# privefl/bigsnpr

Measured on AMD Instinct MI355X. Metric: SNP-cols/sec for bed_randomSVD k=20 (m*passes/wall), higher is better.
Workload: dtype i8 (2-bit codes x 24-bit (early block steps) / 16-bit (late block steps) fixed-point image of the fp64 basis in int8 slices, exact int32 MFMA accumulation; fp64 panel algebra and Rayleigh-Ritz)

## Files before the change

bigsnpr_amd/_lib.py:

```python
import ctypes as C
import os
import threading

import numpy as np

_HERE = os.path.dirname(os.path.abspath(__file__))
LIB_PATH = os.path.join(_HERE, "libbigsnpr_hip.so")

u8p = C.POINTER(C.c_uint8)
i32p = C.POINTER(C.c_int32)
i64p = C.POINTER(C.c_int64)
u64p = C.POINTER(C.c_uint64)
f64p = C.POINTER(C.c_double)
vp = C.c_void_p
i64 = C.c_int64

ALLREDUCE_FN = C.CFUNCTYPE(None, C.c_void_p, C.c_int64, C.c_void_p)


class SvdOptions(C.Structure):
    _fields_ = [("k", C.c_int32), ("tol", C.c_double), ("block", C.c_int32),
                ("slices", C.c_int32), ("max_basis", C.c_int32), ("seed", C.c_uint32),
                ("verbose", C.c_int32), ("m_total", C.c_int64), ("allreduce", ALLREDUCE_FN),
                ("allreduce_ctx", C.c_void_p), ("hook_rank", C.c_int32), ("hook_world", C.c_int32),
                ("comm", C.c_void_p), ("binom_scaling", C.c_int32),
                ("center_out", C.POINTER(C.c_double)), ("scale_out", C.POINTER(C.c_double)),
                ("warm_start", C.c_int32), ("warm_denominator", C.c_int32), ("max_restarts", C.c_int32),
                ("vec_floor", C.c_double), ("exchange_timing", C.c_int32), ("exchange_timeout_ms", C.c_int32)]


class SvdInfo(C.Structure):
    _fields_ = [("niter", C.c_int32), ("nops", C.c_int32), ("basis", C.c_int32),
                ("converged", C.c_int32), ("max_rel_resid", C.c_double), ("gpu_ms", C.c_double),
                ("cprod_ms", C.c_double), ("prod_ms", C.c_double), ("n_cprod", C.c_int32),
                ("n_prod", C.c_int32), ("block", C.c_int32), ("slices", C.c_int32),
                ("n_bad", C.c_int32), ("fused_stats", C.c_int32), ("cprod_stats_ms", C.c_double),
                ("n_cprod_stats", C.c_int32), ("warm_launches", C.c_int32), ("warm_fraction", C.c_double),
                ("warm_ms", C.c_double), ("tiled", C.c_int32), ("segmented_passes", C.c_int32), ("compact_gathers", C.c_int32),
                ("slices_max", C.c_int32), ("wide_steps", C.c_int32), ("wide_cprod_ms", C.c_double),
                ("wide_prod_ms", C.c_double), ("n_wide_cprod", C.c_int32), ("n_wide_prod", C.c_int32),
                ("lead_rel_resid", C.c_double), ("exchange_mode", C.c_int32), ("n_exchange", C.c_int32 * 4),
                ("exchange_ms", C.c_double * 4), ("compacted", C.c_int32), ("compact_ms", C.c_double),
                ("out_of_core", C.c_int32), ("na_free_steps", C.c_double * 2), ("na_skip", C.c_int32),
                ("early_ritz", C.c_int32 * 2)]


class PlrOptions(C.Structure):
    _fields_ = [("family", C.c_int32), ("nlambda", C.c_int32), ("nlam_min", C.c_int32), ("n_abort", C.c_int32),
                ("dfmax", C.c_int32), ("max_iter", C.c_int32), ("eps", C.c_double), ("lambda_min_ratio", C.c_double)]


_PLR_TAIL = [f64p, f64p, i64, f64p, i32p, C.c_int32, f64p, C.c_int32, C.POINTER(PlrOptions), f64p, f64p, f64p, f64p, f64p,
             i32p, i32p, i32p, i32p, i32p]

SIGNATURES = {
    "bsn_last_error": (C.c_char_p, []),
    "bsn_version": (C.c_int, []),
    "bsn_device_count": (C.c_int, [C.POINTER(C.c_int)]),
    "bsn_set_device": (C.c_int, [C.c_int]),
    "bsn_selftest": (C.c_int, []),
    "bsn_comm_unique_id": (C.c_int, [u8p]),
    "bsn_comm_init": (C.c_int, [u8p, C.c_int, C.c_int, C.POINTER(vp)]),
    "bsn_comm_rank": (C.c_int, [vp]),
    "bsn_comm_world": (C.c_int, [vp]),
    "bsn_comm_allreduce": (C.c_int, [vp, vp, i64]),
    "bsn_comm_abort": (C.c_int, [vp]),
    "bsn_comm_destroy": (C.c_int, [vp]),
    "bsn_ld_last_stats": (C.c_int, [f64p]),
    "bsn_robust_scale_tau2": (C.c_int, [vp, i64, i64, C.c_int32, C.c_double, C.c_double, f64p, f64p]),
    "bsn_robust_medians": (C.c_int, [vp, i64, i64, C.c_int32, f64p, f64p]),
    "bsn_robust_pair_scales": (C.c_int, [vp, i64, i64, C.c_int32, C.c_double, C.c_double, f64p, f64p]),
    "bsn_robust_mc_count": (C.c_int, [vp, i64, vp, i64, C.c_double, C.POINTER(C.c_int64)]),
    "bsn_robust_scale_cols": (C.c_int, [vp, i64, i64, C.c_int32, f64p]),
    "bsn_robust_rotate": (C.c_int, [vp, i64, i64, C.c_int32, f64p]),
    "bsn_robust_wdist": (C.c_int, [vp, i64, i64, C.c_int32, f64p, f64p, f64p]),
    "bsn_robust_dist_ogk": (C.c_int, [vp, i64, i64, C.c_int32, C.c_int32, C.c_double, C.c_double, C.c_double, f64p, C.POINTER(C.c_int64)]),
    "bsn_robust_rollmean": (C.c_int, [f64p, i64, f64p, C.c_int32, C.POINTER(C.c_int64), C.c_int32, f64p]),
    "bsn_robust_sort": (C.c_int, [f64p, i64]),
    "bsn_order_decreasing": (C.c_int, [f64p, i64, C.POINTER(C.c_int64), C.c_int32, i32p, i32p]),
    "bsn_robust_mc_window": (C.c_int, [vp, i64, vp, i64, C.c_double, C.c_double, i64, f64p, C.POINTER(C.c_int64)]),
    "bsn_bed_open": (C.c_int, [C.c_char_p, i64, i64, C.POINTER(vp)]),
    "bsn_bed_from_host": (C.c_int, [u8p, i64, i64, i64, C.POINTER(vp)]),
    "bsn_bed_from_fbm": (C.c_int, [u8p, i64, i64, i64, C.POINTER(vp)]),
    "bsn_fbm_open": (C.c_int, [u8p, i64, i64, i64, f64p, C.POINTER(vp)]),
    "bsn_bed_bits": (C.c_int, [vp]),
    "bsn_bed_tile": (C.c_int, [vp, C.POINTER(C.c_int)]),
    "bsn_bed_sample_major": (C.c_int, [vp, C.POINTER(C.c_int)]),
    "bsn_bed_na_known": (i64, [vp]),
    "bsn_bed_synthetic": (C.c_int, [i64, i64, C.c_uint32, C.c_uint32, C.c_uint32, i64, C.POINTER(vp)]),
    "bsn_bed_close": (C.c_int, [vp]),
    "bsn_bed_release_workspace": (C.c_int, [vp]),
    "bsn_bed_nrow": (i64, [vp]),
    "bsn_bed_ncol": (i64, [vp]),
    "bsn_bed_bytes": (i64, [vp]),
    "bsn_bed_download": (C.c_int, [vp, u8p]),
    "bsn_bed_prodvec": (C.c_int, [vp, i64p, i64, i64p, i64, f64p, f64p, f64p, f64p]),
    "bsn_bed_cprodvec": (C.c_int, [vp, i64p, i64, i64p, i64, f64p, f64p, f64p, f64p]),
    "bsn_bed_prodvec_sharded": (C.c_int, [vp, i64p, i64, i64p, i64, f64p, f64p, f64p, vp, f64p]),
    "bsn_bed_col_counts": (C.c_int, [vp, i64p, i64, i64p, i64, i32p]),
    "bsn_bed_row_counts": (C.c_int, [vp, i64p, i64, i64p, i64, i32p]),
    "bsn_bed_colstats": (C.c_int, [vp, i64p, i64, i64p, i64, f64p, f64p, i32p, i32p]),
    "bsn_snp_colstats": (C.c_int, [vp, i64p, i64, i64p, i64, f64p, f64p]),
    "bsn_bed_read": (C.c_int, [vp, i64p, i64, i64p, i64, C.c_int32, i32p]),
    "bsn_bed_read_scaled": (C.c_int, [vp, i64p, i64, i64p, i64, f64p, f64p, f64p]),
    "bsn_bed_cprod_planes": (C.c_int, [vp, i64p, i64, i64p, i64, f64p, i64, f64p, f64p]),
    "bsn_bed_prod_and_rowsumssq": (C.c_int, [vp, i64p, i64, i64p, i64, f64p, f64p, f64p, i64, f64p, f64p]),
    "bsn_snp_prod_and_rowsumssq2": (C.c_int, [vp, i64p, i64, i64p, i64, f64p, f64p, f64p, i64, f64p, f64p]),
    "bsn_mult_lin_reg": (C.c_int, [vp, i64p, i64, i64p, i64, f64p, i64, f64p]),
    "bsn_univ_linreg": (C.c_int, [vp, i64p, i64, i64p, i64, f64p, f64p, i64, f64p, f64p]),
    "bsn_univ_logreg": (C.c_int, [vp, i64p, i64, i64p, i64, f64p, f64p, i64, C.c_double, C.c_int32, f64p, f64p, i32p]),
    "bsn_bed_sp_reg": (C.c_int, [vp, i64p, i64, i64p, i64] + _PLR_TAIL),
    "bsn_dense_sp_reg": (C.c_int, [vp, C.c_int, i64, i64, i64] + _PLR_TAIL),
    "bsn_plr_last_stats": (C.c_int, [f64p]),
    "bsn_impute_simple": (C.c_int, [vp, C.c_int, C.c_uint64, C.POINTER(vp), u8p, i64p]),
    "bsn_impute_last_ms": (C.c_int, [f64p]),
    "bsn_bed_group_counts": (C.c_int, [vp, i64p, i64, i32p, C.c_int32, i64p, i64, i32p]),
    "bsn_fst": (C.c_int, [f64p, f64p, i64, i64, C.c_double, f64p, f64p]),
    "bsn_bed_fst": (C.c_int, [vp, i64p, i64, i32p, C.c_int32, i64p, i64, C.c_double, f64p, f64p]),
    "bsn_snp_max3": (C.c_int, [vp, i64p, i64, i32p, i64p, i64, f64p, C.c_int32, f64p]),
    "bsn_popstat_last_ms": (C.c_int, [f64p]),
    "bsn_bed_to_fbm": (C.c_int, [vp, i64p, i64, i64p, i64, u8p]),
    "bsn_bed_readbina": (C.c_int, [vp, u8p, u8p]),
    "bsn_bed_is_streamed": (C.c_int, [vp]),
    "bsn_bed_streaming_kernels": (C.c_int, [vp, C.c_char_p, i64]),
    "bsn_bed_subset_payload": (C.c_int, [vp, i64p, i64, i64p, i64, u8p]),
    "bsn_op_create": (C.c_int, [vp, i64p, i64, i64p, i64, f64p, f64p, C.POINTER(vp)]),
    "bsn_op_destroy": (C.c_int, [vp]),
    "bsn_op_set_slices": (C.c_int, [vp, C.c_int]),
    "bsn_op_prod": (C.c_int, [vp, vp, i64, C.c_int, vp, i64]),
    "bsn_op_cprod": (C.c_int, [vp, vp, i64, C.c_int, vp, i64]),
    "bsn_op_sync": (C.c_int, [vp]),
    "bsn_op_last_kernel": (C.c_int, [vp, C.c_char_p, i64]),
    "bsn_bed_randomsvd": (C.c_int, [vp, i64p, i64, i64p, i64, f64p, f64p, C.POINTER(SvdOptions),
                                    f64p, f64p, f64p, C.POINTER(SvdInfo)]),
    "bsn_bed_tcrossprod": (C.c_int, [vp, i64p, i64, i64p, i64, f64p, f64p, i64, f64p]),
    "bsn_cormat": (C.c_int, [vp, i64p, i64, i64p, i64, C.c_double, f64p, f64p, C.c_int, i32p,
                             C.POINTER(C.c_int64), C.POINTER(vp)]),
    "bsn_cormat_fetch": (C.c_int, [vp, i32p, f64p]),
    "bsn_cormat_has_nan": (C.c_int, [vp, C.POINTER(C.c_int)]),
    "bsn_cormat_free": (C.c_int, [vp]),
    "bsn_ld_scores": (C.c_int, [vp, i64p, i64, i64p, i64, C.c_double, f64p, f64p]),
    "bsn_clumping_chr": (C.c_int, [vp, i64p, i64, i64p, i64, C.c_int, f64p, f64p, i32p, i32p, f64p,
                                   C.c_double, C.c_double, i32p]),
    "bsn_clumping_chr_cached": (C.c_int, [vp, i64p, i64, i64p, i64, C.c_int, f64p, f64p, i32p, i32p, f64p,
                                          i64, f64p, f64p, i32p]),
    "bsn_snp_grid_prs": (C.c_int, [vp, i64p, i64, i64p, i64, f64p, i32p, C.POINTER(C.c_uint8), i64, i64,
                                   C.c_int, f64p]),
    "bsn_sfbm_from_csc": (C.c_int, [i64p, i32p, f64p, i64, C.c_int, C.POINTER(vp)]),
    "bsn_sfbm_ncol": (C.c_int, [vp, i64p, i64p, i64p]),
    "bsn_sfbm_free": (C.c_int, [vp]),
    "bsn_lassosum2": (C.c_int, [vp, f64p, i64, f64p, f64p, f64p, i64, i64p, C.c_double, C.c_int32, C.c_double,
                                f64p, i32p, f64p]),
    "bsn_ldpred2_gibbs": (C.c_int, [vp, f64p, f64p, i64, i64p, f64p, f64p, i32p, u64p, i64, C.c_int, C.c_int, C.c_uint64,
                                    f64p, f64p]),
    "bsn_ldpred2_gibbs_sampling": (C.c_int, [vp, f64p, f64p, i64, i64p, C.c_double, C.c_double, C.c_int32, C.c_uint64,
                                             C.c_int, C.c_int, C.c_uint64, f64p, f64p]),
    "bsn_ldpred2_auto": (C.c_int, [vp, f64p, f64p, f64p, i64, i64p, f64p, u64p, i64, C.c_double, C.c_int, C.c_int, C.c_int,
                                   C.c_int, C.c_double, C.c_int, C.c_double, C.c_double, C.c_double, C.c_double,
                                   C.c_double, C.c_uint64, f64p, f64p, f64p, f64p, f64p, f64p, f64p, f64p]),
    "bsn_sfbm_prodvec": (C.c_int, [vp, f64p, i64p, i64, f64p]),
    "bsn_sfbm_ld_scores": (C.c_int, [vp, i64p, i64, f64p]),
    "bsn_sfbm_solve_sym": (C.c_int, [vp, f64p, f64p, i64p, i64, C.c_double, C.c_int32, f64p, i32p, f64p]),
    "bsn_sfbm_last_ms": (C.c_int, [vp, f64p]),
    "bsn_sfbm_ldsplit": (C.c_int, [vp, C.c_double, C.c_double, C.c_int32, C.c_int32, C.c_int32, C.c_double, f64p, f64p, i32p,
                                   f64p, f64p, f64p, i32p, i32p, i32p, f64p]),
    "bsn_malloc": (C.c_int, [C.POINTER(vp), i64]),
    "bsn_free": (C.c_int, [vp]),
    "bsn_host_alloc": (C.c_int, [C.POINTER(vp), i64]),
    "bsn_host_free": (C.c_int, [vp]),
    "bsn_memcpy_h2d": (C.c_int, [vp, vp, i64]),
    "bsn_memcpy_d2h": (C.c_int, [vp, vp, i64]),
    "bsn_device_sync": (C.c_int, []),
    "bsn_timer_start": (C.c_int, [vp]),
    "bsn_timer_stop": (C.c_int, [vp, f64p]),
}

_lib = None


class BsnError(RuntimeError):
    pass


def load():
    global _lib
    if _lib is None:
        LIB_PATH = os.environ.get("BSN_LIB_PATH") or globals()["LIB_PATH"]
        if not os.path.exists(LIB_PATH):
            raise ImportError(
                "%s not found: build it with `python -m bigsnpr_amd.build` "
                "(there is no CPU fallback)" % LIB_PATH)
        lib = C.CDLL(LIB_PATH)
        for name, (res, args) in SIGNATURES.items():
            fn = getattr(lib, name)
            fn.restype = res
            fn.argtypes = args
        _lib = lib
    return _lib


def check(rc):
    if rc != 0:
        raise BsnError(load().bsn_last_error().decode("utf-8", "replace"))


def ptr(a, t):
    return None if a is None else a.ctypes.data_as(t)


def as_i64(a):
    return None if a is None else np.ascontiguousarray(a, dtype=np.int64)


def as_f64(a):
    return None if a is None else np.ascontiguousarray(a, dtype=np.float64)


class DeviceArray:

    def __init__(self, rows, cols=1):
        self.rows, self.cols = int(rows), int(cols)
        p = vp()
        check(load().bsn_malloc(C.byref(p), self.rows * self.cols * 8))
        self.ptr = p

    @classmethod
    def from_numpy(cls, a):
        a = np.asarray(a, dtype=np.float64)
        if a.ndim == 1:
            a = a[:, None]
        d = cls(a.shape[0], a.shape[1])
        h = np.asfortranarray(a)
        check(load().bsn_memcpy_h2d(d.ptr, h.ctypes.data_as(vp), h.nbytes))
        return d

    def to_numpy(self):
        h = np.empty((self.rows, self.cols), dtype=np.float64, order="F")
        check(load().bsn_memcpy_d2h(h.ctypes.data_as(vp), self.ptr, h.nbytes))
        return h

    def col_ptr(self, j):
        return vp(self.ptr.value + 8 * self.rows * j)

    def free(self):
        if self.ptr is not None and self.ptr.value:
            load().bsn_free(self.ptr)
            self.ptr = None

    def __del__(self):
        try:
            self.free()
        except Exception:
            pass


class _PinnedBlock:

    def __init__(self, pool, addr, size):
        self.pool, self.addr, self.size = pool, addr, size
        self.__array_interface__ = {"data": (addr, False), "shape": (size,), "typestr": "|u1", "version": 3}

    def __del__(self):
        try:
            self.pool._give_back(self.addr, self.size)
        except Exception:
            pass


class PinnedPool:

    def __init__(self, keep=None):
        self.free = []
        self.keep = int(os.environ.get("BSN_RESULT_POOL_KEEP", 1 << 30)) if keep is None else keep
        self.keep_max = int(os.environ.get("BSN_RESULT_POOL_MAX", 8 << 30))
        self.live = 0
        self.peak_live = 0
        self.lazy = not os.environ.get("BSN_RESULT_POOL_EAGER")
        self.pending = set()
        self.wanted = []
        self.prefetched = 0
        self.lock = threading.RLock()

    def empty(self, shape, dtype=np.float64):
# ... 70 lines not shown
```

bigsnpr_amd/csrc/api.hip:

```cpp
#include <dlfcn.h>
#include <fcntl.h>
#include <pthread.h>
#include <sys/mman.h>
#include <sys/stat.h>
#include <unistd.h>

#include <algorithm>
#include <cerrno>
#include <cmath>
#include <condition_variable>
#include <chrono>
#include <cstring>
#include <limits>
#include <map>
#include <memory>
#include <mutex>
#include <sched.h>
#include <atomic>
#include <thread>

#include <cstdlib>

#include "bsn_internal.hpp"
#include <cxxabi.h>
// ... 972 lines not shown
int bsn_bed_close(bsn_bed *bed) {
  return guarded([&] {
    if (bed) {
      (void)hipSetDevice(bed->device);
      free_bed(bed);
    }
  });
}

int bsn_bed_tile(bsn_bed *bed, int *built) {
  return guarded([&] {
    BSN_HIP(hipSetDevice(bed->device));
    const bool ok = image_tile(bed);
    if (built) *built = ok ? 1 : 0;
  });
}

int bsn_bed_streaming_kernels(bsn_bed *bed, char *buf, int64_t len) {
  return guarded([&] {
    if (!buf || len < 1) fail("bsn_bed_streaming_kernels: no buffer");
    buf[0] = 0;
    if (bed->last_solve_on_sub && bed->sub) bed = bed->sub;
    if (!bed->svd_op) return;
    static const char *kinds[kProfKinds] = {"cprod", "prod", "cprod_stats", "warm", "cprod_wide", "prod_wide"};
    std::string out;
    for (int k = 0; k < kProfKinds; k++) {
      const void *fn = bed->svd_op->prof_kernel[k];
      if (!fn) continue;
      const char *mangled = hipKernelNameRefByPtr(fn, bed->stream);
      if (!mangled) continue;
      int status = 1;
      char *dem = abi::__cxa_demangle(mangled, nullptr, nullptr, &status);
      std::string name = (status == 0 && dem) ? dem : mangled;
      free(dem);
      const size_t par = name.find('(');
      if (par != std::string::npos) name.resize(par);
      out += std::string(kinds[k]) + "=" + name + "\n";
    }
    snprintf(buf, (size_t)len, "%s", out.c_str());
  });
}

int bsn_op_last_kernel(bsn_op *op, char *buf, int64_t len) {
  return guarded([&] {
    if (!buf || len < 1) fail("bsn_op_last_kernel: no buffer");
    buf[0] = 0;
    if (!op->last_kernel) return;
    const char *mangled = hipKernelNameRefByPtr(op->last_kernel, op->bed->stream);
    if (!mangled) return;
    int status = 1;
    char *dem = abi::__cxa_demangle(mangled, nullptr, nullptr, &status);
    std::string name = (status == 0 && dem) ? dem : mangled;
    free(dem);
    const size_t par = name.find('(');
    if (par != std::string::npos) name.resize(par);
    snprintf(buf, (size_t)len, "%s", name.c_str());
  });
}

int bsn_bed_sample_major(bsn_bed *bed, int *built) {
  return guarded([&] {
    BSN_HIP(hipSetDevice(bed->device));
    const bool ok = image_smaj(bed);
    if (built) *built = ok ? 1 : 0;
  });
}

int bsn_bed_release_workspace(bsn_bed *bed) {
  return guarded([&] {
    BSN_HIP(hipSetDevice(bed->device));
    BSN_HIP(hipStreamSynchronize(bed->stream));
    bed->svd_op.reset();
    bed->svd_ws.reset();
    if (bed->d_tiled) {
      BSN_HIP(hipFree(bed->d_tiled));
      bed->d_tiled = nullptr;
    }
    bed->tiled_tried = false;
    image_smaj_wait(bed);
    if (bed->d_smaj) {
      BSN_HIP(hipFree(bed->d_smaj));
      bed->d_smaj = nullptr;
    }
    bed->smaj_tried = false;
    bed->smaj_cap = 0;
    if (bed->sub) {
      bed_free(bed->sub);
      bed->sub = nullptr;
      bed->sub_key = 0;
      bed->sub_cols.clear();
      bed->sub_rows.clear();
      bed->last_solve_on_sub = false;
    }
    bed->stats_cache.release();
    if (bed->slab_img) {
      bed_free(bed->slab_img);
      bed->slab_img = nullptr;
    }
    if (bed->slab_stage) {
      delete (bsn::FileStage *)bed->slab_stage;
      bed->slab_stage = nullptr;
    }
    dev_cache_flush();
  });
}

int64_t bsn_bed_nrow(const bsn_bed *bed) { return bed->n; }
int64_t bsn_bed_ncol(const bsn_bed *bed) { return bed->m; }
int64_t bsn_bed_bytes(const bsn_bed *bed) { return bed->pitch * bed->m; }

int bsn_bed_download(bsn_bed *bed, uint8_t *payload_out) {
  return guarded([&] {
    BSN_HIP(hipSetDevice(bed->device));
    if (bed->streamed()) {
      std::memcpy(payload_out, bed->h_map, (size_t)bed->n_byte * (size_t)bed->m);
      return;
    }
    image_download(bed, payload_out);
  });
}

int bsn_op_create(bsn_bed *bed, const int64_t *ind_row, int64_t n, const int64_t *ind_col,
                  int64_t m, const double *center, const double *scale, bsn_op **out) {
  return guarded([&] {
    std::unique_ptr<bsn_op> op(new bsn_op());
    fill_op(op.get(), bed, ind_row, n, ind_col, m, center, scale);
    *out = op.release();
  });
}

int bsn_op_destroy(bsn_op *op) {
  return guarded([&] {
    if (op) {
      (void)hipSetDevice(op->bed->device);
      delete op;
    }
  });
}

int bsn_op_set_slices(bsn_op *op, int slices) {
  return guarded([&] {
    if (slices < 1 || slices > 7) fail("slices must be in 1..7");
    op->slices = slices;
  });
}

int bsn_op_prod(bsn_op *op, const double *d_X, int64_t ldx, int nvec, double *d_Y, int64_t ldy) {
  return guarded([&] {
    BSN_HIP(hipSetDevice(op->bed->device));
    op_prod(op, d_X, ldx, nvec, d_Y, ldy);
  });
}

int bsn_op_cprod(bsn_op *op, const double *d_X, int64_t ldx, int nvec, double *d_Z, int64_t ldz) {
  return guarded([&] {
    BSN_HIP(hipSetDevice(op->bed->device));
    op_cprod(op, d_X, ldx, nvec, d_Z, ldz);
  });
}

int bsn_op_sync(bsn_op *op) {
  return guarded([&] { BSN_HIP(hipStreamSynchronize(op->bed->stream)); });
}

static void matvec_host(bsn_bed *bed, const int64_t *ind_row, int64_t n, const int64_t *ind_col,
                        int64_t m, const double *center, const double *scale, const double *x,
                        double *out, bool transpose, bsn_comm *comm = nullptr) {
  if (bed->streamed()) {
    if (comm) fail("sharded products are not available for an out-of-core handle");
    SlabWalk W(bed);
    std::vector<double> ce, sc, xs, part;
    if (!transpose) std::fill(out, out + n, 0.0);
    W.run(ind_col, m, [&](bsn_bed *sb, const std::vector<int64_t> &P, const std::vector<int64_t> &local) {
      const int64_t k = (int64_t)P.size();
      if (center) { ce.resize((size_t)k); for (int64_t t = 0; t < k; t++) ce[(size_t)t] = center[P[(size_t)t]]; }
      if (scale) { sc.resize((size_t)k); for (int64_t t = 0; t < k; t++) sc[(size_t)t] = scale[P[(size_t)t]]; }
      if (transpose) {
        part.resize((size_t)k);
        matvec_host(sb, ind_row, n, local.data(), k, center ? ce.data() : nullptr, scale ? sc.data() : nullptr, x,
                    part.data(), true);
        BSN_HIP(hipStreamSynchronize(sb->stream));
        for (int64_t t = 0; t < k; t++) out[P[(size_t)t]] = part[(size_t)t];
      } else {
        xs.resize((size_t)k);
        for (int64_t t = 0; t < k; t++) xs[(size_t)t] = x[P[(size_t)t]];
        part.resize((size_t)n);
        matvec_host(sb, ind_row, n, local.data(), k, center ? ce.data() : nullptr, scale ? sc.data() : nullptr, xs.data(),
                    part.data(), false);
        BSN_HIP(hipStreamSynchronize(sb->stream));
        for (int64_t i = 0; i < n; i++) out[i] += part[(size_t)i];
      }
    });
    return;
  }
  bsn_op op;
  const bool late = transpose && bed->bits == 2 && !bed->generic && (center || scale);
  fill_op(&op, bed, ind_row, n, ind_col, m, center, scale, late);
  if (late) {
    op.late_center = center;
    op.late_scale = scale;
    if (!center) BSN_HIP(hipMemsetAsync(op.d_center.p, 0, (size_t)m * 8, bed->stream));
    if (!scale) {
      hipLaunchKernelGGL(k_fill_f64, dim3((unsigned)((m + 255) / 256)), dim3(256), 0, bed->stream, op.d_scale.p, m, 1.0);
      BSN_HIP(hipGetLastError());
    }
  }
  op.slices = 7;
  int64_t nin = transpose ? n : m, nout = transpose ? m : n;
  DevBuf<double> d_in, d_out;
  copy_h2d(bed, d_in.ensure((size_t)nin), x, (size_t)nin * 8);
  d_out.ensure((size_t)nout);
  if (bed->generic) {
    const int32_t *rows = op.rows_identity ? nullptr : op.d_rows.p, *cols = op.cols_contig ? nullptr : op.d_cols.p;
    if (comm) fail("sharded products are not available for a generic decode table");
    if (transpose)
      lut_cprod(bed, rows, n, cols, op.col0, m, center ? op.d_center.p : nullptr, scale ? op.d_scale.p : nullptr,
                d_in.p, d_out.p);
    else
      lut_prod(bed, rows, n, cols, op.col0, m, center ? op.d_center.p : nullptr, scale ? op.d_scale.p : nullptr,
               d_in.p, d_out.p);
    copy_d2h(bed, out, d_out.p, (size_t)nout * 8);
    return;
  }
  if (transpose)
    op_cprod(&op, d_in.p, nin, 1, d_out.p, nout);
  else
    op_prod(&op, d_in.p, nin, 1, d_out.p, nout);
  if (comm) {
    if (transpose) fail("internal: the crossproduct of a column shard needs no exchange");
    if (comm->device != bed->device) fail("the communicator was created on another device");
    comm_allreduce_sum(comm, d_out.p, nout, bed->stream);
  }
  copy_d2h(bed, out, d_out.p, (size_t)nout * 8);
}

int bsn_bed_prodvec(bsn_bed *bed, const int64_t *ind_row, int64_t n, const int64_t *ind_col,
                    int64_t m, const double *center, const double *scale, const double *x,
                    double *y) {
  return guarded([&] { matvec_host(bed, ind_row, n, ind_col, m, center, scale, x, y, false); });
}

int bsn_bed_prodvec_sharded(bsn_bed *bed, const int64_t *ind_row, int64_t n, const int64_t *ind_col,
                            int64_t m, const double *center, const double *scale, const double *x,
                            bsn_comm *comm, double *y) {
  return guarded([&] { matvec_host(bed, ind_row, n, ind_col, m, center, scale, x, y, false, comm); });
}

int bsn_bed_cprodvec(bsn_bed *bed, const int64_t *ind_row, int64_t n, const int64_t *ind_col,
                     int64_t m, const double *center, const double *scale, const double *x,
                     double *z) {
  return guarded([&] { matvec_host(bed, ind_row, n, ind_col, m, center, scale, x, z, true); });
}

int bsn_bed_col_counts(bsn_bed *bed, const int64_t *ind_row, int64_t n, const int64_t *ind_col,
                       int64_t m, int32_t *res) {
  return guarded([&] { counts_host(bed, ind_row, n, ind_col, m, res); });
}

int bsn_bed_row_counts(bsn_bed *bed, const int64_t *ind_row, int64_t n, const int64_t *ind_col, int64_t m,
                       int32_t *res) {
  return guarded([&] {
    bsn_op op;
    fill_op(&op, bed, ind_row, n, ind_col, m, nullptr, nullptr);
    DevBuf<double> d_c;
    d_c.ensure((size_t)3 * n);
    op_row_counts(&op, d_c.p);
    std::vector<double> c((size_t)3 * n);
    copy_d2h(bed, c.data(), d_c.p, (size_t)3 * n * 8);
    for (int64_t i = 0; i < n; i++) {
      const int64_t n2 = (int64_t)c[(size_t)i], n1 = (int64_t)c[(size_t)(n + i)], na = (int64_t)c[(size_t)(2 * n + i)];
      res[4 * i + 0] = (int32_t)(m - n1 - n2 - na);
      res[4 * i + 1] = (int32_t)n1;
      res[4 * i + 2] = (int32_t)n2;
      res[4 * i + 3] = (int32_t)na;
    }
  });
}

int bsn_bed_colstats(bsn_bed *bed, const int64_t *ind_row, int64_t n, const int64_t *ind_col,
                     int64_t m, double *sumX, double *denoX, int32_t *nb_nona_col,
                     int32_t *n_bad) {
  return guarded([&] {
    std::vector<int32_t> cnt((size_t)4 * m);
    counts_host(bed, ind_row, n, ind_col, m, cnt.data());
    int32_t bad = 0;
    for (int64_t j = 0; j < m; j++) {
      const int32_t *c = &cnt[(size_t)4 * j];
      double xSum = (double)c[1] + 2.0 * c[2], xxSum = (double)c[1] + 4.0 * c[2];
      int32_t nona = (int32_t)(n - c[3]);
      sumX[j] = xSum;
      denoX[j] = xxSum - xSum * xSum / nona;
      nb_nona_col[j] = nona;
      if (2 * (int64_t)nona < n) bad++;
    }
    if (n_bad) *n_bad = bad;
  });
}

int bsn_snp_colstats(bsn_bed *bed, const int64_t *ind_row, int64_t n, const int64_t *ind_col,
                     int64_t m, double *sumX, double *denoX) {
  return guarded([&] {
    const double qnan = std::numeric_limits<double>::quiet_NaN();
    if (bed->generic) {
      bsn_op op;
      fill_op(&op, bed, ind_row, n, ind_col, m, nullptr, nullptr);
      DevBuf<double> d_st;
// ... 364 lines not shown
```

bigsnpr_amd/csrc/bsn_internal.hpp:

```cpp
#pragma once
#include <hip/hip_runtime.h>
#include <stdint.h>

#include <atomic>
#include <cstdarg>
#include <cstdio>
#include <functional>
#include <cstdlib>
#include <memory>
#include <stdexcept>
#include <string>
#include <vector>

#include "bigsnpr_hip.h"

namespace bsn {
inline const char *abl_getenv(const char *name) {
#ifdef BSN_ABLATION
  return getenv(name);
#else
  (void)name;
  return nullptr;
#endif
}

struct Error : std::runtime_error {
  using std::runtime_error::runtime_error;
};
void set_error(const char *msg);
[[noreturn]] void fail(const char *fmt, ...);
void require_gpu();

#define BSN_HIP(expr)                                                             \
  do {                                                                            \
    hipError_t e__ = (expr);                                                      \
    if (e__ != hipSuccess)                                                        \
      ::bsn::fail("HIP error %s at %s:%d (%s)", hipGetErrorString(e__), __FILE__, \
                  __LINE__, #expr);                                               \
  } while (0)

template <class F>
int guarded(F &&f) {
  try {
    f();
    return 0;
  } catch (const std::exception &ex) {
    set_error(ex.what());
    (void)hipGetLastError();
    return 1;
  } catch (...) {
    set_error("unknown C++ exception");
    (void)hipGetLastError();
    return 1;
  }
}

constexpr size_t kDevCacheMaxBlock = (size_t)256 << 20;
constexpr size_t kDevCacheMaxTotal = (size_t)2 << 30;
void *dev_alloc(size_t bytes, size_t *granted, int *device);
void dev_release(void *p, size_t granted, int device);
void dev_cache_flush();
size_t dev_cache_held();

template <class T>
struct DevBuf {
  T *p = nullptr;
  size_t n = 0;
  size_t granted = 0;
  int device = 0;
  DevBuf() = default;
  DevBuf(const DevBuf &) = delete;
  DevBuf &operator=(const DevBuf &) = delete;
  ~DevBuf() { release(); }
  void release() {
    if (p) dev_release(p, granted, device);
    p = nullptr;
    n = 0;
    granted = 0;
  }
  T *ensure(size_t count) {
    if (count > n) {
      release();
      p = (T *)dev_alloc(count * sizeof(T), &granted, &device);
      n = count;
    }
    return p;
  }
};

constexpr int64_t kPitchAlign = 256;

inline int64_t round_up(int64_t a, int64_t b) { return (a + b - 1) / b * b; }

__host__ __device__ inline uint32_t dev_from_plink(uint32_t w) {
  return (~w & 0xAAAAAAAAu) | ((w ^ (w >> 1)) & 0x55555555u);
}
__host__ __device__ inline uint32_t plink_from_dev(uint32_t w) {
  return (~w & 0xAAAAAAAAu) | (~(w ^ (w >> 1)) & 0x55555555u);
}

}

struct bsn_bed;
namespace bsn {
struct SvdWorkspace;
}

constexpr int kCommClasses = 4;
struct bsn_comm {
  void *comm = nullptr;
  int rank = 0, world = 1, device = 0;
  hipStream_t stream = nullptr;
  std::atomic<int> aborted{0};
  bool timing = false;
  struct Timed { hipEvent_t a, b; int cls; };
  std::vector<Timed> timed;
  std::vector<hipEvent_t> ev_pool;
  ~bsn_comm() {
    for (auto &t : timed) { (void)hipEventDestroy(t.a); (void)hipEventDestroy(t.b); }
    for (auto e : ev_pool) (void)hipEventDestroy(e);
  }
};

constexpr int kProfKinds = 6;
struct bsn_op {
  bsn_bed *bed = nullptr;
  int64_t n = 0, m = 0;
  bool rows_identity = true;
  bool cols_contig = true;
  bool no_na = false;
  bool na_skip_c = false, na_skip_p = false;
  bool stats_pending = false;
  bsn::DevBuf<int32_t> d_counts;
  bsn::DevBuf<int32_t> d_na;
  long long *h_na_total = nullptr;
  bool na_poll = false;
  int64_t col0 = 0;
  int slices = 4;
  int64_t passes = 0;
  const double *late_center = nullptr, *late_scale = nullptr;
  const double *preq_X = nullptr;
  int64_t preq_ldx = 0;
  int preq_nvec = 0, preq_S = 0;
  bool profile = false;
  int prof_kind_override = -1;
  std::vector<hipEvent_t> ev_begin, ev_end;
  std::vector<int> ev_kind;
  std::vector<char> ev_more;
  const void *prof_kernel[kProfKinds] = {};
  const void *last_kernel = nullptr;
  ~bsn_op() {
    for (auto e : ev_begin) (void)hipEventDestroy(e);
    for (auto e : ev_end) (void)hipEventDestroy(e);
    if (h_na_total) (void)hipHostFree(h_na_total);
  }
  bsn::DevBuf<int32_t> d_rows;
  bsn::DevBuf<int32_t> d_cols;
  bsn::DevBuf<double> d_center, d_scale;
  bsn::DevBuf<double> d_xfull;
  bsn::DevBuf<int8_t> d_q;
  bsn::DevBuf<int32_t> d_acc;
  bsn::DevBuf<double> d_meta;
  bsn::DevBuf<double> d_yfull;
};

struct bsn_bed {
  int64_t n = 0, m = 0, n_byte = 0, pitch = 0;
  int bits = 2;
  double v_off = 0.0, v_step = 1.0;
  bool generic = false;
  double *d_lut = nullptr;
  uint8_t *d_img = nullptr;
  uint8_t *d_tiled = nullptr;
  bool tiled_tried = false;
  size_t tiled_cap = 0;
  const uint8_t *h_map = nullptr;
  void *map_base = nullptr;
  size_t map_len = 0;
  int64_t slab_cols = 0;
  int fd_file = -1;
  bsn_bed *slab_img = nullptr;
  void *slab_stage = nullptr;
  bool streamed() const { return d_img == nullptr && h_map != nullptr; }
  uint8_t *d_smaj = nullptr;
  int64_t pitch_smaj = 0, rows_smaj = 0;
  bool smaj_tried = false;
  size_t smaj_cap = 0;
  void *smaj_job = nullptr;
  int64_t cap_m = 0;
  bsn_bed *sub = nullptr;
  uint64_t sub_key = 0;
  std::vector<int64_t> sub_cols, sub_rows;
  bool last_solve_on_sub = false;
  int device = 0;
  bool stream_borrowed = false;
  hipStream_t stream = nullptr;
  hipStream_t stream_up = nullptr;
  hipEvent_t ev_up = nullptr;
  hipEvent_t ev0 = nullptr, ev1 = nullptr;
  std::vector<int32_t> na_cnt;
  struct CountsCache {
    std::vector<int64_t> rows;
    std::vector<int32_t> cnt;
    void clear() {
      rows.clear();
      cnt.clear();
    }
  } counts_cache;
  struct StatsCache {
    bsn::DevBuf<int32_t> d_cnt;
    std::vector<uint8_t> known;
    int64_t n_known = 0;
    bsn::DevBuf<int32_t> d_cols;
    uint64_t cols_key = 0;
    void clear() {
      known.clear();
      n_known = 0;
    }
    void release() {
      clear();
      d_cnt.release();
      d_cols.release();
      cols_key = 0;
    }
  } stats_cache;
  void forget_counts() {
    counts_cache.clear();
    stats_cache.clear();
  }
  int na_blocks_state = 0;
  long long *h_na_blocks = nullptr;
  long long *d_na_blocks = nullptr;
  double na_free[2] = {0.0, 0.0};
  std::unique_ptr<bsn_op> svd_op;
  std::shared_ptr<bsn::SvdWorkspace> svd_ws;
  uint8_t *h_stage[2] = {nullptr, nullptr};
  hipEvent_t ev_stage[2] = {nullptr, nullptr};
  bool stage_busy[2] = {false, false};
  unsigned stage_next = 0;
};

struct bsn_sfbm {
  int64_t m2 = 0, nnz = 0;
  bsn::DevBuf<int64_t> p;
  bsn::DevBuf<int32_t> i;
  bsn::DevBuf<double> x;
  std::vector<int32_t> lo, hi;
  int64_t bandwidth = 0;
  std::vector<int64_t> hp;
  double last_ms = 0;
};

namespace bsn {

void image_alloc(bsn_bed *b, int64_t n, int64_t m, int bits = 2);
void stage_init(bsn_bed *b);
void bed_free(bsn_bed *b);
bsn_bed *image_gather(bsn_bed *src, const int64_t *ind_row, int64_t n, const int64_t *ind_col, int64_t m,
                      bsn_bed *reuse = nullptr);
bool image_tile(bsn_bed *b);
bool image_smaj(bsn_bed *b);
bool image_smaj_start(bsn_bed *b);
bool image_smaj_poll(bsn_bed *b);
void image_smaj_wait(bsn_bed *b);
void image_from_host(bsn_bed *b, const uint8_t *payload, int64_t n_byte_src);
struct FileStage {
  uint8_t *pin[2] = {nullptr, nullptr};
  hipEvent_t done[2] = {nullptr, nullptr};
  size_t bytes = 0;
  ~FileStage();
  FileStage() = default;
  FileStage(const FileStage &) = delete;
  FileStage &operator=(const FileStage &) = delete;
};
void image_from_file(bsn_bed *b, int fd, int64_t offset, int64_t n_byte_src, FileStage *stage = nullptr);
void image_from_fbm(bsn_bed *b, const uint8_t *bytes, int64_t ld, const uint8_t *lut);
void stats8(bsn_bed *b, const int32_t *d_rows, int64_t n, const int32_t *d_cols, int64_t col0, int64_t m,
            long long *d_out);
void lut_colstats(bsn_bed *b, const int32_t *d_rows, int64_t n, const int32_t *d_cols, int64_t col0, int64_t m,
                  double *d_out);
void lut_cprod(bsn_bed *b, const int32_t *d_rows, int64_t n, const int32_t *d_cols, int64_t col0, int64_t m,
               const double *d_center, const double *d_scale, const double *d_x, double *d_z);
void lut_prod(bsn_bed *b, const int32_t *d_rows, int64_t n, const int32_t *d_cols, int64_t col0, int64_t m,
              const double *d_center, const double *d_scale, const double *d_x, double *d_y);
void refuse_generic(const bsn_bed *b, const char *what);
void image_generate(bsn_bed *b, uint32_t seed, uint32_t npop, uint32_t na16, int64_t j_begin);
void image_download(bsn_bed *b, uint8_t *payload_out);
void counts_all_rows(bsn_bed *b, const int32_t *d_cols, int64_t col0, int64_t m, int32_t *d_counts);
void counts_host(bsn_bed *bed, const int64_t *ind_row, int64_t n, const int64_t *ind_col, int64_t m,
                 int32_t *res);
void counts_device(bsn_op *op, const int64_t *ind_row, int64_t n, int32_t *d_counts);
struct StatsCols {
  const int64_t *ind_col;
  const int32_t *d_cols;
  int64_t col0, m;
};
bool stats_cache_enabled(const bsn_bed *b);
bool stats_cache_known(const bsn_bed *b, const StatsCols &c);
void stats_cache_store(bsn_bed *b, const StatsCols &c, const int32_t *d_counts, hipStream_t st);
void stats_cache_load(bsn_bed *b, const StatsCols &c, int32_t *d_counts, hipStream_t st);
void read_dense(bsn_bed *b, const int32_t *d_rows, int64_t n, const int32_t *d_cols, int64_t m,
                const double *d_center, const double *d_scale, int32_t na_val, int32_t *d_out_i,
                double *d_out_d);

void to_bytes(bsn_bed *b, const int32_t *d_rows, int64_t n, const int32_t *d_cols, int64_t m,
              uint8_t *d_out);
void readbina_bytes(bsn_bed *b, const uint8_t *d_tab, uint8_t *d_out);
void subset_pack(bsn_bed *b, const int32_t *d_rows, int64_t n, const int32_t *d_cols, int64_t m,
                 uint8_t *d_out);

void copy_h2d(bsn_bed *b, void *d_dst, const void *src, size_t bytes, hipStream_t stream = nullptr);
hipStream_t upload_stream(bsn_bed *b);
void copy_d2h(bsn_bed *b, void *dst, const void *d_src, size_t bytes);
bool host_is_pinned(const void *p);
// ... 57 lines not shown
```

bigsnpr_amd/csrc/matvec.hip:

```cpp
#include <cmath>
#include <cstdlib>

#include "bsn_internal.hpp"
#include "byte_plan.hpp"
#include "prod_plan.hpp"
#include "prodt_sparse.hpp"
#include <type_traits>

namespace bsn {

typedef int v4i __attribute__((ext_vector_type(4)));
typedef int v8i __attribute__((ext_vector_type(8)));

static thread_local const void *g_last_kernel = nullptr;
#define BSN_KLAUNCH(kern, ...)                 \
  do {                                         \
    g_last_kernel = (const void *)(kern);      \
    hipLaunchKernelGGL(kern, __VA_ARGS__);     \
  } while (0)

__device__ __forceinline__ uint32_t lut4(uint32_t lut, uint32_t sel) {
  return __builtin_amdgcn_perm(lut, lut, sel);
}
__device__ __forceinline__ uint32_t perm8(uint32_t hi, uint32_t lo, uint32_t sel) {
// ... 49 lines not shown
      const double b3 = fabs(b - 3.0 * a);
      if (!(fabs(b) <= 1.79e308)) bad++; else mx = fmax(mx, fabs(b));
      if (raw3 && b3 <= 1.79e308) mx = fmax(mx, b3);
    } else if (mode == 2) {
      double b = center ? fabs(center[k + v * ldx]) : 0.0;
      if (!(b <= 1.79e308)) bad++; else mx = fmax(mx, b);
    }
    a = fabs(a);
    if (!(a <= 1.79e308)) bad++; else mx = fmax(mx, a);
  }
  for (int off = 32; off > 0; off >>= 1) {
    mx = fmax(mx, __shfl_down(mx, off));
    bad += __shfl_down(bad, off);
  }
  __shared__ double smx[16];
  __shared__ unsigned long long sbad[16];
  const int wave = threadIdx.x >> 6, nw = blockDim.x >> 6;
  if ((threadIdx.x & 63) == 0) {
    smx[wave] = mx;
    sbad[wave] = bad;
  }
  __syncthreads();
  if (threadIdx.x == 0) {
    for (int w = 1; w < nw; w++) {
      mx = fmax(mx, smx[w]);
      bad += sbad[w];
    }
    double *pp = part + ((int64_t)v * gridDim.x + blockIdx.x) * 2;
    pp[0] = mx;
    pp[1] = (double)bad;
    if (blockIdx.x == 0) meta[v].sum_hi = meta[v].sum_lo = meta[v].sum2_hi = meta[v].sum2_lo = 0;
  }
}

template <int S, int PERM>
__global__ __launch_bounds__(64) void k_quant(const double *__restrict__ X, int64_t ldx, int64_t len,
                                              int64_t len_pad, const double *__restrict__ center,
                                              const double *__restrict__ scale, int mode, int ncol,
                                              VecMeta *meta, int8_t *__restrict__ q, double vstep, double voff,
                                              int raw3, const double *__restrict__ part, int gx) {
  __shared__ double sa[64 * 17], sb[64 * 17];
  const int tid = threadIdx.x, v = blockIdx.y;
  const int64_t kb = (int64_t)blockIdx.x * 64 + tid;
  const int nplanes = mode >= 1 ? 2 : 1;
  double qs = 1.0;
  if (gx > 0) {
    double mx = 0, bad = 0;
    for (int t = tid; t < gx; t += 64) {
      mx = fmax(mx, part[((int64_t)v * gx + t) * 2]);
      bad += part[((int64_t)v * gx + t) * 2 + 1];
    }
    for (int off = 32; off > 0; off >>= 1) {
      mx = fmax(mx, __shfl_xor(mx, off));
      bad += __shfl_xor(bad, off);
    }
    qs = 0.0;
    if (mx > 0) {
      int e;
      frexp(ldexp(0.99, 8 * S - 1) / mx, &e);
      qs = ldexp(1.0, e - 1);
    }
    if (blockIdx.x == 0 && tid == 0) {
      meta[v].absmax_bits = (unsigned long long)__double_as_longlong(mx);
      meta[v].nonfinite = (unsigned long long)bad;
    }
  }
  if (blockIdx.x == 0 && tid == 0) meta[v].qscale = qs;
  double xa[16], xc[16], xs[16];
#pragma unroll
  for (int it = 0; it < 16; it++) {
    const int64_t k = (int64_t)blockIdx.x * 1024 + it * 64 + tid;
    const bool in = k < len;
    xa[it] = in ? X[k + v * ldx] : 0.0;
    xc[it] = 0.0;
    xs[it] = 1.0;
    if (mode == 1) {
      if (in && scale) xs[it] = scale[k];
      if (in && center) xc[it] = center[k];
    } else if (mode == 2) {
      if (in && center) xc[it] = center[k + v * ldx];
    }
  }
#pragma unroll
  for (int it = 0; it < 16; it++) {
    const int t = it * 64 + tid;
    double a = xa[it], b = 0;
    if (mode == 1) {
      a = a / xs[it];
      b = (xc[it] - voff) * a;
      a *= vstep;
    } else if (mode == 2) {
      b = xc[it];
    }
    if (!(fabs(a) <= 1.79e308)) a = 0;
    if (!(fabs(b) <= 1.79e308)) b = 0;
    sa[t + (t >> 4)] = a * qs;
    sb[t + (t >> 4)] = b * qs;
  }
  __syncthreads();
  long long shi = 0, slo = 0, shi2 = 0, slo2 = 0;
  if (kb * 16 < len_pad) {
    uint32_t pk[2][S][4];
#pragma unroll
    for (int p = 0; p < 2; p++)
#pragma unroll
      for (int s = 0; s < S; s++)
#pragma unroll
        for (int w = 0; w < 4; w++) pk[p][s][w] = 0;
#pragma unroll
    for (int e = 0; e < 16; e++) {
      long long A = llrint(sa[tid * 17 + e]), B = llrint(sb[tid * 17 + e]);
      shi += A >> 24; slo += A & 0xFFFFFF;
      shi2 += B >> 24; slo2 += B & 0xFFFFFF;
      if ((raw3 & 1) && PERM != 2) B -= 3 * A;
      const int pos = PERM == 1 ? ((e & 3) * 4 + (e >> 2)) : e;
#pragma unroll
      for (int s = 0; s < S; s++) {
        const int8_t da = (int8_t)(A & 0xFF), db = (int8_t)(B & 0xFF);
        A = (A - da) >> 8;
        B = (B - db) >> 8;
        if constexpr (PERM == 2) {
          const int r = prodt_sparse_row(e), ba = prodt_sparse_byte(e, 0), bb = prodt_sparse_byte(e, 1);
          pk[r][s][ba >> 2] |= (uint32_t)(uint8_t)da << (8 * (ba & 3));
          pk[r][s][bb >> 2] |= (uint32_t)(uint8_t)db << (8 * (bb & 3));
        } else {
          pk[0][s][pos >> 2] |= (uint32_t)(uint8_t)da << (8 * (pos & 3));
          pk[1][s][pos >> 2] |= (uint32_t)(uint8_t)db << (8 * (pos & 3));
        }
      }
    }
    for (int p = 0; p < nplanes; p++)
#pragma unroll
      for (int s = 0; s < S; s++) {
        const int col = v * S + s;
        int8_t *dst = q + ((kb * nplanes + p) * ncol + col) * 16;
        *(uint4 *)dst = p == 0 ? uint4{pk[0][s][0], pk[0][s][1], pk[0][s][2], pk[0][s][3]}
                               : uint4{pk[1][s][0], pk[1][s][1], pk[1][s][2], pk[1][s][3]};
      }
  }
  for (int off = 32; off > 0; off >>= 1) {
    shi += __shfl_down(shi, off); slo += __shfl_down(slo, off);
    shi2 += __shfl_down(shi2, off); slo2 += __shfl_down(slo2, off);
  }
  if (tid == 0) {
    atomicAdd((unsigned long long *)&meta[v].sum_hi, (unsigned long long)shi);
    atomicAdd((unsigned long long *)&meta[v].sum_lo, (unsigned long long)slo);
    if (mode >= 1) {
      atomicAdd((unsigned long long *)&meta[v].sum2_hi, (unsigned long long)shi2);
      atomicAdd((unsigned long long *)&meta[v].sum2_lo, (unsigned long long)slo2);
    }
  }
}

template <int NB, int NPLANE, int KC, bool RAW0, bool STATS, bool CONTIG, int TILES = 2, int WAVES = 8, int MINW = 1,
          int TAG = 0, bool TILED = false, int SGB = 0, bool NASKIP = false>
__global__ __launch_bounds__(64 * WAVES, MINW) void k_cprod(const uint8_t *__restrict__ img, int64_t pitch,
                                               const int32_t *__restrict__ cols, int64_t col0,
                                               int64_t m, const int8_t *__restrict__ xq,
                                               int32_t *__restrict__ acc_out, int64_t m_out,
                                               uint32_t lutA, uint32_t lutB, uint32_t lutC,
                                               int32_t *__restrict__ counts, int32_t n_pad_samples) {
  constexpr int NCOL = 16 * NB;
  constexpr int LD = KC / 256;
  constexpr int XS = KC / 16 * NCOL;
  __shared__ uint4 xs[2][XS];
  const int tid = threadIdx.x, wave = tid >> 6, lane = tid & 63;
  const int c = lane & 15, g = lane >> 4;
  constexpr int NT = 64 * WAVES;
  const int64_t wg_base = (int64_t)blockIdx.x * (WAVES * 16 * TILES);
  const int64_t snp_base = wg_base + wave * (16 * TILES);
  const uint8_t *rowp[TILES];
  uint32_t voff[TILES];
#pragma unroll
  for (int t = 0; t < TILES; t++) {
    int64_t j = snp_base + t * 16 + c;
    if (j > m - 1) j = m - 1;
    int64_t col = CONTIG ? col0 + j : (int64_t)cols[j];
    rowp[t] = img + col * pitch + g * 16;
    voff[t] = TILED ? (uint32_t)((((j - wg_base) >> 6) * (pitch >> 8)) * 16384 + (j & 63) * 256 + g * 16)
                    : (uint32_t)((j - wg_base) * pitch + g * 16);
  }
  static_assert(!TILED || (CONTIG && (WAVES * 16 * TILES) % 64 == 0), "streaming layout: whole 64-variant blocks");
  const __amdgpu_buffer_rsrc_t rs = __builtin_amdgcn_make_buffer_rsrc(
      (void *)(TILED ? img + (((col0 + wg_base) >> 6) * (pitch >> 8)) * 16384
                     : img + (col0 + (CONTIG ? wg_base : 0)) * pitch),
      0, 0x7fffffff, 0x00020000);
  typedef unsigned int v4u __attribute__((ext_vector_type(4)));
  auto gload = [&](const int t, const int off) -> uint4 {
    if constexpr (CONTIG) {
      const int soff = TILED ? ((off >> 8) << 14) + (off & 255) : off;
      const v4u r = __builtin_amdgcn_raw_buffer_load_b128(rs, (int)voff[t], soff, 0);
      return uint4{r.x, r.y, r.z, r.w};
    } else {
      return *(const uint4 *)(rowp[t] + off);
    }
  };
  const int nchunks = (int)(pitch * 4 / KC);
  const uint4 *xq4 = (const uint4 *)xq;

  v4i acc[TILES][NPLANE][NB];
#pragma unroll
  for (int t = 0; t < TILES; t++)
#pragma unroll
    for (int p = 0; p < NPLANE; p++)
#pragma unroll
      for (int nb = 0; nb < NB; nb++) acc[t][p][nb] = v4i{0, 0, 0, 0};
  uint32_t st_lo[TILES], st_hi[TILES], st_na[TILES];
#pragma unroll
  for (int t = 0; t < TILES; t++) st_lo[t] = st_hi[t] = st_na[t] = 0;

  constexpr int NX = (XS + NT - 1) / NT;
  static_assert(NX <= 4, "staging registers");
  constexpr bool XFULL = (XS % NT == 0);
  uint4 ga[2][TILES][LD];
  uint4 xr0 = {0, 0, 0, 0}, xr1 = {0, 0, 0, 0}, xr2 = {0, 0, 0, 0}, xr3 = {0, 0, 0, 0};
#pragma unroll
  for (int t = 0; t < TILES; t++)
#pragma unroll
    for (int it = 0; it < LD; it++) ga[0][t][it] = gload(t, it * 64);
  auto staged = [&](const int x) -> bool { return XFULL || tid + x * NT < XS; };
  if (staged(0)) xs[0][tid] = xq4[tid];
  if constexpr (NX > 1) if (staged(1)) xs[0][tid + NT] = xq4[tid + NT];
  if constexpr (NX > 2) if (staged(2)) xs[0][tid + 2 * NT] = xq4[tid + 2 * NT];
  if constexpr (NX > 3) if (staged(3)) xs[0][tid + 3 * NT] = xq4[tid + 3 * NT];
#pragma unroll
  for (int t = 0; t < TILES; t++)
#pragma unroll
    for (int it = 0; it < LD; it++)
      ga[1][t][it] = gload(t, (nchunks > 1 ? KC / 4 : 0) + it * 64);
  __syncthreads();

  auto chunk = [&](auto SETC, const int ch) {
    constexpr int SET = decltype(SETC)::value;
    const int ch1 = ch + 1 < nchunks ? ch + 1 : nchunks - 1;
    const int ch2 = ch + 2 < nchunks ? ch + 2 : nchunks - 1;
    {
      const uint4 *src = xq4 + (int64_t)ch1 * XS;
      auto at = [&](const int x) -> int { return XFULL ? tid + x * NT : (tid + x * NT < XS ? tid + x * NT : XS - 1); };
      xr0 = src[at(0)];
      if constexpr (NX > 1) xr1 = src[at(1)];
      if constexpr (NX > 2) xr2 = src[at(2)];
      if constexpr (NX > 3) xr3 = src[at(3)];
    }
    __builtin_amdgcn_sched_barrier(0);
    if constexpr (SGB & 2) __builtin_amdgcn_s_setprio(2);
    const int off2 = ch2 * (KC / 4);
    auto kstep = [&](const int t, const uint32_t w, const uint4 (&bv)[NB]) {
      uint32_t s0 = w & 0x03030303u, s1 = (w >> 2) & 0x03030303u,
               s2 = (w >> 4) & 0x03030303u, s3 = (w >> 6) & 0x03030303u;
      if constexpr (STATS) {
        const uint32_t lo = w & 0x55555555u;
        st_lo[t] += __popc(lo);
        st_hi[t] += __popc(w);
        st_na[t] += __popc(lo & (w >> 1));
      }
      static_assert(!NASKIP || (RAW0 && NPLANE == 2 && !STATS), "the skip is for the missing-value plane of the plain pass");
      bool plane1 = true;
      if constexpr (NASKIP) plane1 = __builtin_amdgcn_ballot_w64(((w & (w >> 1)) & 0x55555555u) != 0u) != 0ull;
#pragma unroll
      for (int p = 0; p < NPLANE; p++) {
        if (NASKIP && p == 1 && !plane1) continue;
        const uint32_t lut = p == 0 ? lutA : p == 1 ? lutB : lutC;
        v4i a;
        if (RAW0 && p == 0) {
          a = v4i{(int)s0, (int)s1, (int)s2, (int)s3};
        } else {
          a = v4i{(int)lut4(lut, s0), (int)lut4(lut, s1), (int)lut4(lut, s2), (int)lut4(lut, s3)};
        }
#pragma unroll
        for (int nb = 0; nb < NB; nb++) {
          v4i b = {(int)bv[nb].x, (int)bv[nb].y, (int)bv[nb].z, (int)bv[nb].w};
          acc[t][p][nb] = __builtin_amdgcn_mfma_i32_16x16x64_i8(a, b, acc[t][p][nb], 0, 0, 0);
        }
      }
    };
    constexpr bool PFB = NB <= 2;
    uint4 bv[NB], bn[PFB ? NB : 1];
#pragma unroll
    for (int nb = 0; nb < NB; nb++) bv[nb] = xs[SET][(g * 4) * NCOL + nb * 16 + c];
#pragma unroll
    for (int it = 0; it < LD; it++) {
#pragma unroll
      for (int d = 0; d < 4; d++) {
        if constexpr (!PFB) {
          if (it * 4 + d > 0) {
#pragma unroll
            for (int nb = 0; nb < NB; nb++) bv[nb] = xs[SET][(it * 16 + g * 4 + d) * NCOL + nb * 16 + c];
          }
        } else if (it * 4 + d + 1 < LD * 4) {
          const int itn = (it * 4 + d + 1) / 4, dn = (it * 4 + d + 1) % 4;
#pragma unroll
          for (int nb = 0; nb < NB; nb++) bn[nb] = xs[SET][(itn * 16 + g * 4 + dn) * NCOL + nb * 16 + c];
        }
#pragma unroll
        for (int t = 0; t < TILES; t++) {
          const uint32_t w = d == 0 ? ga[SET][t][it].x : d == 1 ? ga[SET][t][it].y
                             : d == 2 ? ga[SET][t][it].z : ga[SET][t][it].w;
          kstep(t, w, bv);
        }
        if constexpr (PFB) {
#pragma unroll
          for (int nb = 0; nb < NB; nb++) bv[nb] = bn[nb];
        }
      }
    }
#pragma unroll
    for (int t = 0; t < TILES; t++)
#pragma unroll
      for (int it = 0; it < LD; it++) ga[SET][t][it] = gload(t, off2 + it * 64);
    if constexpr (SGB & 1) {
      constexpr int VSTEP = TILES * (7 + (NPLANE - (RAW0 ? 1 : 0)) * 4 + (STATS ? 6 : 0));
      constexpr int MSTEP = TILES * NPLANE * NB;
      __builtin_amdgcn_sched_group_barrier(0x100, NB, 0);
      __builtin_amdgcn_sched_group_barrier(0x002, 7, 0);
      auto slot = [&](auto IC) {
        constexpr int i = decltype(IC)::value;
        constexpr int nv = VSTEP * (i + 1) / MSTEP - VSTEP * i / MSTEP;
        __builtin_amdgcn_sched_group_barrier(0x008, 1, 0);
        if constexpr (nv > 0) __builtin_amdgcn_sched_group_barrier(0x002, nv, 0);
      };
      auto slots = [&](auto self, auto IC) {
        constexpr int i = decltype(IC)::value;
        if constexpr (i < MSTEP) {
          slot(IC);
          self(self, std::integral_constant<int, i + 1>{});
        }
      };
#pragma unroll
      for (int stp = 0; stp < LD * 4; stp++) {
        __builtin_amdgcn_sched_group_barrier(0x100, NB, 0);
        slots(slots, std::integral_constant<int, 0>{});
      }
      __builtin_amdgcn_sched_group_barrier(0x020, TILES * LD, 0);
    }
    __builtin_amdgcn_sched_barrier(0);
    if constexpr (SGB & 2) __builtin_amdgcn_s_setprio(0);
    {
      if (staged(0)) xs[SET ^ 1][tid] = xr0;
      if constexpr (NX > 1) if (staged(1)) xs[SET ^ 1][tid + NT] = xr1;
      if constexpr (NX > 2) if (staged(2)) xs[SET ^ 1][tid + 2 * NT] = xr2;
      if constexpr (NX > 3) if (staged(3)) xs[SET ^ 1][tid + 3 * NT] = xr3;
    }
    __syncthreads();
  };
  for (int ch = 0; ch < nchunks; ch += 2) {
    chunk(std::integral_constant<int, 0>{}, ch);
    if (ch + 1 < nchunks) chunk(std::integral_constant<int, 1>{}, ch + 1);
  }

#pragma unroll
  for (int t = 0; t < TILES; t++)
#pragma unroll
    for (int r = 0; r < 4; r++) {
      int64_t j = snp_base + t * 16 + g * 4 + r;
      if (j < m) {
#pragma unroll
        for (int p = 0; p < NPLANE; p++)
#pragma unroll
          for (int nb = 0; nb < NB; nb++)
            acc_out[((int64_t)p * m_out + j) * NCOL + nb * 16 + c] = acc[t][p][nb][r];
      }
    }
  if constexpr (STATS) {
#pragma unroll
    for (int t = 0; t < TILES; t++) {
      uint32_t lo = st_lo[t], hi = st_hi[t] - st_lo[t], na = st_na[t];
      lo += __shfl_xor(lo, 16); hi += __shfl_xor(hi, 16); na += __shfl_xor(na, 16);
      lo += __shfl_xor(lo, 32); hi += __shfl_xor(hi, 32); na += __shfl_xor(na, 32);
      const int64_t j = snp_base + t * 16 + c;
      if (g == 0 && j < m) {
        const int32_t n1 = (int32_t)(lo - na), n2 = (int32_t)(hi - na);
        *(int4 *)(counts + 4 * j) =
            int4{(int32_t)(pitch * 4) - n1 - n2 - (int32_t)na - n_pad_samples, n1, n2, (int32_t)na};
      }
    }
  }
}

__device__ __forceinline__ double horner(const int32_t *a, int S) {
  double r = 0;
  for (int s = S - 1; s >= 0; s--) r = r * 256.0 + (double)a[s];
  return r;
}
__device__ __forceinline__ double horner_sub(const int32_t *a, const int32_t *q, int k, int S) {
  double r = 0;
  for (int s = S - 1; s >= 0; s--) r = r * 256.0 + (double)((long long)a[s] - (long long)k * q[s]);
  return r;
}

template <int NCOL>
__global__ __launch_bounds__(128) void k_cprod_final(const int32_t *__restrict__ acc, int64_t m, int S, int nv,
                                                     const VecMeta *__restrict__ meta,
                                                     const double *__restrict__ center,
                                                     const double *__restrict__ scale, double *Z, int64_t ldz,
                                                     int has_q) {
  constexpr int ROW = 2 * NCOL + 1;
  __shared__ int32_t srow[128 * ROW];
  const int64_t j = (int64_t)blockIdx.x * 128 + threadIdx.x;
  if (j >= m) return;
  int32_t *my = srow + threadIdx.x * ROW;
  {
    const int4 *pa = (const int4 *)(acc + j * NCOL), *pq = (const int4 *)(acc + (m + j) * NCOL);
#pragma unroll
    for (int t = 0; t < NCOL / 4; t++) {
      const int4 x = pa[t];
      my[4 * t] = x.x; my[4 * t + 1] = x.y; my[4 * t + 2] = x.z; my[4 * t + 3] = x.w;
    }
    if (has_q) {
#pragma unroll
      for (int t = 0; t < NCOL / 4; t++) {
        const int4 x = pq[t];
        my[NCOL + 4 * t] = x.x; my[NCOL + 4 * t + 1] = x.y; my[NCOL + 4 * t + 2] = x.z; my[NCOL + 4 * t + 3] = x.w;
      }
    }
  }
  const double c = center ? center[j] : 0.0, s = scale ? scale[j] : 1.0;
  for (int v = 0; v < nv; v++) {
    const double P = has_q ? horner_sub(my + v * S, my + NCOL + v * S, 3, S) : horner(my + v * S, S);
    const double Q = has_q ? horner(my + NCOL + v * S, S) : 0.0;
    const double Sx = (double)meta[v].sum_hi * 16777216.0 + (double)meta[v].sum_lo;
    const double qs = meta[v].qscale;
    double z = qs > 0 ? (P - c * (Sx - Q)) / (s * qs) : 0.0 / s;
    if (P == 0.0 && Sx - Q == 0.0 && qs > 0) z = 0.0;
    if (meta[v].nonfinite) z = __longlong_as_double(0x7ff8000000000000LL);
    Z[j + v * ldz] = z;
  }
}

template <int NB, bool CONTIG, bool RAWP, bool HASQ = true, int TAG = 0, bool TILED = false>
__global__ __launch_bounds__(256) void k_prod(const uint8_t *__restrict__ img, int64_t pitch,
                                              const int32_t *__restrict__ cols, int64_t col0,
                                              int64_t m_pad, int64_t mc,
                                              const int8_t *__restrict__ wq,
                                              int32_t *__restrict__ acc_out, int64_t n_pad,
                                              uint32_t lutP, uint32_t lutQ) {
  constexpr int NCOL = 16 * NB, WAVES = 4;
  const int tid = threadIdx.x, wave = tid >> 6, lane = tid & 63;
  const int sg = lane & 15, g = lane >> 4;
  const unsigned bx = blockIdx.x, by = blockIdx.y;
  static_assert(!TILED || CONTIG, "streaming layout: contiguous variants");
  const int64_t wbase = ((int64_t)bx * WAVES + wave) * 256;
  const int64_t wbyte = wbase / 4 + sg * 4;
  const uint32_t lane_off = (uint32_t)(g * 16 * pitch + wbyte);
  const int64_t j0 = (int64_t)by * mc;
  int64_t j1 = j0 + mc;
  if (j1 > m_pad) j1 = m_pad;
  const uint4 *wq4 = (const uint4 *)wq;

  v4i acc[16][NB];
#pragma unroll
  for (int u = 0; u < 16; u++)
#pragma unroll
    for (int nb = 0; nb < NB; nb++) acc[u][nb] = v4i{0, 0, 0, 0};

  constexpr int WS = 8 * NCOL;
  __shared__ uint4 ws[2][WS];
  static_assert((WS & (WS - 1)) == 0 && WS <= 64 * WAVES, "digit staging");
  uint32_t X[2][16];
  uint4 wreg = {0, 0, 0, 0};
  const int wtid = tid & (WS - 1);
  auto load = [&](int64_t jb, uint32_t *dst) {
    if (CONTIG) {
      if constexpr (TILED) {
        const int64_t sbw = (int64_t)bx;
        const __amdgpu_buffer_rsrc_t rs = __builtin_amdgcn_make_buffer_rsrc(
            (void *)(img + (((col0 + jb) >> 6) * (pitch >> 8) + sbw) * 16384), 0, 0x7fffffff, 0x00020000);
        const int toff = g * 4096 + wave * 64 + sg * 4;
#pragma unroll
        for (int r = 0; r < 16; r++) dst[r] = (uint32_t)__builtin_amdgcn_raw_buffer_load_b32(rs, toff, r * 256, 0);
      } else {
        const __amdgpu_buffer_rsrc_t rs = __builtin_amdgcn_make_buffer_rsrc(
            (void *)(img + (col0 + jb) * pitch), 0, 0x7fffffff, 0x00020000);
#pragma unroll
        for (int r = 0; r < 16; r++) dst[r] = (uint32_t)__builtin_amdgcn_raw_buffer_load_b32(rs, (int)lane_off, r * (int)pitch, 0);
      }
    } else {
      const int4 *ip = (const int4 *)(cols + jb + g * 16);
#pragma unroll
      for (int r4 = 0; r4 < 4; r4++) {
        int4 id = ip[r4];
        dst[r4 * 4 + 0] = *(const uint32_t *)(img + (int64_t)id.x * pitch + wbyte);
        dst[r4 * 4 + 1] = *(const uint32_t *)(img + (int64_t)id.y * pitch + wbyte);
        dst[r4 * 4 + 2] = *(const uint32_t *)(img + (int64_t)id.z * pitch + wbyte);
        dst[r4 * 4 + 3] = *(const uint32_t *)(img + (int64_t)id.w * pitch + wbyte);
      }
    }
  };
  if (j0 >= j1) return;
  const int64_t jlast = j1 - 64;
  ws[0][wtid] = wq4[(j0 / 16) * 2 * NCOL + wtid];
  load(j0, X[0]);
  load(j0 + 64 < j1 ? j0 + 64 : jlast, X[1]);
  __syncthreads();

  auto step = [&](auto SETC, const int64_t jb) {
    constexpr int SET = decltype(SETC)::value;
    const int64_t jn1 = jb + 64 < j1 ? jb + 64 : jlast, jn2 = jb + 128 < j1 ? jb + 128 : jlast;
    wreg = wq4[(jn1 / 16) * 2 * NCOL + wtid];
    __builtin_amdgcn_sched_barrier(0);
    v4i aw[NB], awc[NB];
#pragma unroll
    for (int nb = 0; nb < NB; nb++) {
      uint4 t0 = ws[SET][(g * 2 + 0) * NCOL + nb * 16 + sg];
      uint4 t1 = ws[SET][(g * 2 + 1) * NCOL + nb * 16 + sg];
      aw[nb] = v4i{(int)t0.x, (int)t0.y, (int)t0.z, (int)t0.w};
      awc[nb] = v4i{(int)t1.x, (int)t1.y, (int)t1.z, (int)t1.w};
    }
    uint32_t T[4][4];
#pragma unroll
    for (int r4 = 0; r4 < 4; r4++) {
      const uint32_t x0 = X[SET][4 * r4], x1 = X[SET][4 * r4 + 1], x2 = X[SET][4 * r4 + 2], x3 = X[SET][4 * r4 + 3];
      const uint32_t lo01 = perm8(x1, x0, 0x05010400u);
      const uint32_t hi01 = perm8(x1, x0, 0x07030602u);
      const uint32_t lo23 = perm8(x3, x2, 0x05010400u);
      const uint32_t hi23 = perm8(x3, x2, 0x07030602u);
      T[0][r4] = perm8(lo23, lo01, 0x05040100u);
      T[1][r4] = perm8(lo23, lo01, 0x07060302u);
      T[2][r4] = perm8(hi23, hi01, 0x05040100u);
      T[3][r4] = perm8(hi23, hi01, 0x07060302u);
    }
    __builtin_amdgcn_sched_barrier(0);
    load(jn2, X[SET]);
    __builtin_amdgcn_sched_barrier(0);
#pragma unroll
    for (int q = 0; q < 4; q++)
#pragma unroll
      for (int u0 = 0; u0 < 4; u0++) {
        v4i g0, na;
#pragma unroll
        for (int r4 = 0; r4 < 4; r4++) {
          const uint32_t sel = (T[q][r4] >> (2 * u0)) & 0x03030303u;
          g0[r4] = RAWP ? (int)sel : (int)lut4(lutP, sel);
          if (HASQ) na[r4] = (int)lut4(lutQ, sel);
        }
#pragma unroll
        for (int nb = 0; nb < NB; nb++) {
          acc[q * 4 + u0][nb] = __builtin_amdgcn_mfma_i32_16x16x64_i8(aw[nb], g0, acc[q * 4 + u0][nb], 0, 0, 0);
          if (HASQ)
            acc[q * 4 + u0][nb] = __builtin_amdgcn_mfma_i32_16x16x64_i8(awc[nb], na, acc[q * 4 + u0][nb], 0, 0, 0);
        }
      }
    ws[SET ^ 1][wtid] = wreg;
    __syncthreads();
  };
  for (int64_t jb = j0; jb < j1; jb += 128) {
    step(std::integral_constant<int, 0>{}, jb);
    if (jb + 64 < j1) step(std::integral_constant<int, 1>{}, jb + 64);
  }
#pragma unroll
  for (int u = 0; u < 16; u++) {
    const int64_t i = wbase + sg * 16 + u;
#pragma unroll
    for (int nb = 0; nb < NB; nb++)
      *(v4i *)(acc_out + (((int64_t)by * n_pad + i) * NCOL + nb * 16 + 4 * g)) = acc[u][nb];
  }
}

template <int NB, bool HASQ, int TILES = 2, int WAVES = 16, int TAG = 0, int SGB = 3, bool NASKIP = false, bool SPARSE = false>
__global__ __launch_bounds__(64 * WAVES) void k_prodT(const uint8_t *__restrict__ simg, int64_t rows_t, int64_t chunk0,
                                                      int nchunks, int cps,
                                                      const int8_t *__restrict__ wq, int32_t *__restrict__ acc_out,
                                                      int64_t n_pad, uint32_t lutQ, int seg_bs, int seg_stride, int seg_off) {
  constexpr int KC = 512, NCOL = 16 * NB, LD = KC / 256;
  constexpr int XS = KC / 16 * 2 * NCOL;
  constexpr int NT = 64 * WAVES, NX = XS / NT;
  static_assert(XS % NT == 0 && NX >= 1 && NX <= 4, "digit staging");
  __shared__ uint4 xs[2][XS];
  const int tid = threadIdx.x, wave = tid >> 6, lane = tid & 63;
  const int c = lane & 15, g = lane >> 4;
  const unsigned bx = seg_bs > 0 ? (blockIdx.x / (unsigned)seg_bs) * (unsigned)seg_stride + (unsigned)seg_off + blockIdx.x % (unsigned)seg_bs
                                 : blockIdx.x;
  const int64_t wg_base = (int64_t)bx * (WAVES * 16 * TILES);
  const int64_t row_base = wg_base + wave * (16 * TILES);
  uint32_t voff[TILES];
#pragma unroll
  for (int t = 0; t < TILES; t++) {
    int64_t i = row_base + t * 16 + c;
    if (i > rows_t - 1) i = rows_t - 1;
    voff[t] = (uint32_t)((i - wg_base) * (KC / 4) + g * 16);
  }
  const int ch_begin = (int)blockIdx.y * cps;
  int ch_end = ch_begin + cps;
  if (ch_end > nchunks) ch_end = nchunks;
  if (ch_begin >= ch_end) return;
  if (wg_base >= rows_t) return;
  const int64_t chunk_stride = rows_t * (KC / 4);
  const uint8_t *const base0 = simg + ((chunk0 + ch_begin) * rows_t + wg_base) * (KC / 4);
  typedef unsigned int v4u __attribute__((ext_vector_type(4)));
  auto gload = [&](const int t, const int ch, const int off) -> uint4 {
    const __amdgpu_buffer_rsrc_t rs =
        __builtin_amdgcn_make_buffer_rsrc((void *)(base0 + (int64_t)ch * chunk_stride), 0, 0x7fffffff, 0x00020000);
    const v4u r = __builtin_amdgcn_raw_buffer_load_b128(rs, (int)voff[t], off, 0);
    return uint4{r.x, r.y, r.z, r.w};
  };
  const int nch = ch_end - ch_begin;
  const uint4 *xq4 = (const uint4 *)wq + (int64_t)ch_begin * XS;

  v4i acc[TILES][NB];
#pragma unroll
  for (int t = 0; t < TILES; t++)
#pragma unroll
    for (int nb = 0; nb < NB; nb++) acc[t][nb] = v4i{0, 0, 0, 0};
  uint4 ga[2][TILES][LD];
  uint4 xr0 = {0, 0, 0, 0}, xr1 = {0, 0, 0, 0}, xr2 = {0, 0, 0, 0}, xr3 = {0, 0, 0, 0};
#pragma unroll
  for (int t = 0; t < TILES; t++)
#pragma unroll
    for (int it = 0; it < LD; it++) ga[0][t][it] = gload(t, 0, it * 64);
#pragma unroll
  for (int x = 0; x < NX; x++) xs[0][tid + x * NT] = xq4[tid + x * NT];
#pragma unroll
  for (int t = 0; t < TILES; t++)
#pragma unroll
    for (int it = 0; it < LD; it++) ga[1][t][it] = gload(t, nch > 1 ? 1 : 0, it * 64);
  __syncthreads();

  auto chunk = [&](auto SETC, const int ch) {
    constexpr int SET = decltype(SETC)::value;
    const int ch1 = ch + 1 < nch ? ch + 1 : nch - 1;
    const int ch2 = ch + 2 < nch ? ch + 2 : nch - 1;
    xr0 = xq4[(int64_t)ch1 * XS + tid];
    if constexpr (NX > 1) xr1 = xq4[(int64_t)ch1 * XS + tid + NT];
    if constexpr (NX > 2) xr2 = xq4[(int64_t)ch1 * XS + tid + 2 * NT];
    if constexpr (NX > 3) xr3 = xq4[(int64_t)ch1 * XS + tid + 3 * NT];
    __builtin_amdgcn_sched_barrier(0);
    if constexpr (SGB & 2) __builtin_amdgcn_s_setprio(2);
    constexpr int NP = HASQ ? 2 : 1;
    static_assert(!SPARSE || (HASQ && !NASKIP), "the sparse form replaces the two planes of the plain pass");
    constexpr bool PFB = NB <= 2;
    uint4 bv[NP][NB], bn[PFB ? NP : 1][PFB ? NB : 1];
    auto xrow = [&](const int kb, const int p) -> int {
      return SPARSE ? (kb + (2 * p + (g >> 1)) * 4) * 2 + (g & 1) : (kb + g * 4) * 2 + p;
    };
#pragma unroll
    for (int p = 0; p < NP; p++)
#pragma unroll
      for (int nb = 0; nb < NB; nb++) {
        bv[p][nb] = xs[SET][xrow(0, p) * NCOL + nb * 16 + c];
        if constexpr (PFB) bn[p][nb] = bv[p][nb];
      }
#pragma unroll
    for (int it = 0; it < LD; it++) {
#pragma unroll
      for (int d = 0; d < 4; d++) {
        if constexpr (!PFB) {
          if (it * 4 + d > 0) {
#pragma unroll
            for (int p = 0; p < NP; p++)
#pragma unroll
              for (int nb = 0; nb < NB; nb++) bv[p][nb] = xs[SET][xrow(it * 16 + d, p) * NCOL + nb * 16 + c];
          }
        } else if (it * 4 + d + 1 < LD * 4) {
          const int itn = (it * 4 + d + 1) / 4, dn = (it * 4 + d + 1) % 4;
#pragma unroll
          for (int p = 0; p < NP; p++)
#pragma unroll
            for (int nb = 0; nb < NB; nb++) bn[p][nb] = xs[SET][xrow(itn * 16 + dn, p) * NCOL + nb * 16 + c];
        }
#pragma unroll
        for (int t = 0; t < TILES; t++) {
          const uint32_t w = d == 0 ? ga[SET][t][it].x : d == 1 ? ga[SET][t][it].y
                             : d == 2 ? ga[SET][t][it].z : ga[SET][t][it].w;
          if constexpr (SPARSE) {
            uint32_t av[4], idx;
            prodt_sparse_decode(w, av, idx);
            const v4i a = {(int)av[0], (int)av[1], (int)av[2], (int)av[3]};
#pragma unroll
            for (int nb = 0; nb < NB; nb++) {
              const v8i b = {(int)bv[0][nb].x, (int)bv[0][nb].y, (int)bv[0][nb].z, (int)bv[0][nb].w,
                             (int)bv[1][nb].x, (int)bv[1][nb].y, (int)bv[1][nb].z, (int)bv[1][nb].w};
              acc[t][nb] = __builtin_amdgcn_smfmac_i32_16x16x128_i8(a, b, acc[t][nb], (int)idx, 0, 0);
            }
            continue;
          }
          const uint32_t s0 = w & 0x03030303u, s1 = (w >> 2) & 0x03030303u, s2 = (w >> 4) & 0x03030303u,
                         s3 = (w >> 6) & 0x03030303u;
          const v4i a0 = {(int)s0, (int)s1, (int)s2, (int)s3};
#pragma unroll
          for (int nb = 0; nb < NB; nb++) {
            const v4i b = {(int)bv[0][nb].x, (int)bv[0][nb].y, (int)bv[0][nb].z, (int)bv[0][nb].w};
            acc[t][nb] = __builtin_amdgcn_mfma_i32_16x16x64_i8(a0, b, acc[t][nb], 0, 0, 0);
          }
          if constexpr (HASQ) {
            static_assert(!NASKIP || HASQ, "the skip is for the missing-value plane");
            bool plane1 = true;
            if constexpr (NASKIP) plane1 = __builtin_amdgcn_ballot_w64(((w & (w >> 1)) & 0x55555555u) != 0u) != 0ull;
            if (plane1) {
              const v4i a1 = {(int)lut4(lutQ, s0), (int)lut4(lutQ, s1), (int)lut4(lutQ, s2), (int)lut4(lutQ, s3)};
#pragma unroll
              for (int nb = 0; nb < NB; nb++) {
                const v4i b = {(int)bv[1][nb].x, (int)bv[1][nb].y, (int)bv[1][nb].z, (int)bv[1][nb].w};
                acc[t][nb] = __builtin_amdgcn_mfma_i32_16x16x64_i8(a1, b, acc[t][nb], 0, 0, 0);
              }
            }
          }
        }
        if constexpr (PFB) {
#pragma unroll
          for (int p = 0; p < NP; p++)
#pragma unroll
            for (int nb = 0; nb < NB; nb++) bv[p][nb] = bn[p][nb];
        }
      }
    }
#pragma unroll
    for (int t = 0; t < TILES; t++)
#pragma unroll
      for (int it = 0; it < LD; it++) ga[SET][t][it] = gload(t, ch2, it * 64);
    if constexpr (SGB & 1) {
      constexpr int VSTEP = TILES * (SPARSE ? 18 : 7 + (HASQ ? 4 : 0)), MSTEP = TILES * (SPARSE ? NB : NP * NB);
      __builtin_amdgcn_sched_group_barrier(0x100, NP * NB, 0);
      __builtin_amdgcn_sched_group_barrier(0x002, SPARSE ? 9 : 7, 0);
      auto slots = [&](auto self, auto IC) {
        constexpr int i = decltype(IC)::value;
        if constexpr (i < MSTEP) {
          constexpr int nv = VSTEP * (i + 1) / MSTEP - VSTEP * i / MSTEP;
          __builtin_amdgcn_sched_group_barrier(0x008, 1, 0);
          if constexpr (nv > 0) __builtin_amdgcn_sched_group_barrier(0x002, nv, 0);
          self(self, std::integral_constant<int, i + 1>{});
        }
      };
#pragma unroll
      for (int stp = 0; stp < LD * 4; stp++) {
        __builtin_amdgcn_sched_group_barrier(0x100, NP * NB, 0);
        slots(slots, std::integral_constant<int, 0>{});
      }
      __builtin_amdgcn_sched_group_barrier(0x020, TILES * LD, 0);
    }
    __builtin_amdgcn_sched_barrier(0);
    if constexpr (SGB & 2) __builtin_amdgcn_s_setprio(0);
    xs[SET ^ 1][tid] = xr0;
    if constexpr (NX > 1) xs[SET ^ 1][tid + NT] = xr1;
    if constexpr (NX > 2) xs[SET ^ 1][tid + 2 * NT] = xr2;
    if constexpr (NX > 3) xs[SET ^ 1][tid + 3 * NT] = xr3;
    __syncthreads();
  };
  for (int ch = 0; ch < nch; ch += 2) {
    chunk(std::integral_constant<int, 0>{}, ch);
    if (ch + 1 < nch) chunk(std::integral_constant<int, 1>{}, ch + 1);
  }
#pragma unroll
  for (int t = 0; t < TILES; t++)
#pragma unroll
    for (int r = 0; r < 4; r++) {
      const int64_t i = row_base + t * 16 + g * 4 + r;
      if (i < n_pad) {
#pragma unroll
        for (int nb = 0; nb < NB; nb++)
          acc_out[((int64_t)blockIdx.y * n_pad + i) * NCOL + nb * 16 + c] = acc[t][nb][r];
      }
    }
}

template <int NCOL>
__global__ __launch_bounds__(256) void k_prod_final(const int32_t *__restrict__ acc, int64_t n_pad, int ky, int S, int nv,
                             const VecMeta *meta, const int32_t *rows, int64_t n, double *Y,
                             int64_t ldy, int sub_const, double beta, int64_t blk_rows = 0) {
  int64_t i = (int64_t)blockIdx.x * blockDim.x + threadIdx.x;
  if (i >= n) return;
  int64_t i2 = rows ? (int64_t)rows[i] : i;
  if (i2 < 0) {
    for (int v = 0; v < nv; v++) Y[(i / blk_rows * nv + v) * blk_rows + i % blk_rows] = 0.0;
    return;
  }
  long long d[NCOL];
#pragma unroll
  for (int c = 0; c < NCOL; c++) d[c] = 0;
  for (int k = 0; k < ky; k++) {
    const int4 *a = (const int4 *)(acc + ((int64_t)k * n_pad + i2) * NCOL);
#pragma unroll
    for (int c4 = 0; c4 < NCOL / 4; c4++) {
      int4 t = a[c4];
      d[4 * c4 + 0] += t.x;
      d[4 * c4 + 1] += t.y;
      d[4 * c4 + 2] += t.z;
      d[4 * c4 + 3] += t.w;
    }
  }
  for (int v = 0; v < nv; v++) {
    double r = 0;
    for (int s = S - 1; s >= 0; s--) {
      long long dv = 0;
#pragma unroll
      for (int c = 0; c < NCOL; c++) dv = (c == v * S + s) ? d[c] : dv;
      r = r * 256.0 + (double)dv;
    }
    double C = sub_const ? (double)meta[v].sum2_hi * 16777216.0 + (double)meta[v].sum2_lo : 0.0;
    double qs = meta[v].qscale;
    double y = qs > 0 ? (r - C) / qs : 0.0;
    if (meta[v].nonfinite) y = __longlong_as_double(0x7ff8000000000000LL);
    if (blk_rows > 0)
      Y[(i / blk_rows * nv + v) * blk_rows + i % blk_rows] = y;
    else
      Y[i + v * ldy] = beta != 0.0 ? beta * Y[i + v * ldy] + y : y;
  }
}

__device__ __forceinline__ uint32_t val8m(uint32_t w, uint32_t &na) {
  const uint32_t t = w ^ 0x80808080u;
  const uint32_t y = (t & 0x7F7F7F7Fu) + 0x7F7F7F7Fu;
  const uint32_t z = ~(y | t | 0x7F7F7F7Fu);
  na = z >> 7;
  return w & ~(z | (z - na));
}

template <int NB, bool HASNA, bool CONTIG>
__global__ __launch_bounds__(512) void k_cprod8(const uint8_t *__restrict__ img, int64_t pitch,
                                                const int32_t *__restrict__ cols, int64_t col0, int64_t m,
                                                const int8_t *__restrict__ xq, int32_t *__restrict__ acc_out,
                                                int64_t m_out, int slice_chunks) {
  constexpr int KC = 256, LD = KC / 64, NCOL = 16 * NB, XS = KC / 16 * NCOL, WAVES = 8, NT = 64 * WAVES;
  constexpr int NPL = HASNA ? 2 : 1;
  __shared__ uint4 xs[2][XS];
  const int tid = threadIdx.x, wave = tid >> 6, lane = tid & 63, c = lane & 15, g = lane >> 4;
  const int64_t snp_base = ((int64_t)blockIdx.x * WAVES + wave) * 16;
  int64_t j = snp_base + c;
  if (j > m - 1) j = m - 1;
  const int64_t col = CONTIG ? col0 + j : (int64_t)cols[j];
  const int ch0 = (int)blockIdx.y * slice_chunks;
  const int nchunks = min((int)(pitch / KC) - ch0, slice_chunks);
  const uint8_t *rowp = img + col * pitch + (int64_t)ch0 * KC + g * 16;
  const uint4 *xq4 = (const uint4 *)xq + (int64_t)ch0 * XS;
  acc_out += (int64_t)blockIdx.y * NPL * m_out * NCOL;
  v4i acc[NPL][NB];
#pragma unroll
  for (int p = 0; p < NPL; p++)
#pragma unroll
    for (int nb = 0; nb < NB; nb++) acc[p][nb] = v4i{0, 0, 0, 0};
  static_assert(XS <= NT, "digit staging");
  uint4 ga[2][LD], xr = {0, 0, 0, 0};
#pragma unroll
  for (int it = 0; it < LD; it++) ga[0][it] = *(const uint4 *)(rowp + it * 64);
  if (tid < XS) xs[0][tid] = xq4[tid];
#pragma unroll
  for (int it = 0; it < LD; it++) ga[1][it] = *(const uint4 *)(rowp + (nchunks > 1 ? KC : 0) + it * 64);
  __syncthreads();
  auto chunk = [&](auto SETC, const int ch) {
    constexpr int SET = decltype(SETC)::value;
    const int ch1 = ch + 1 < nchunks ? ch + 1 : nchunks - 1, ch2 = ch + 2 < nchunks ? ch + 2 : nchunks - 1;
    if (tid < XS) xr = xq4[(int64_t)ch1 * XS + tid];
    __builtin_amdgcn_sched_barrier(0);
#pragma unroll
    for (int it = 0; it < LD; it++) {
      const uint4 w = ga[SET][it];
      v4i val, na;
      if constexpr (HASNA) {
        uint32_t n0, n1, n2, n3;
        val = v4i{(int)val8m(w.x, n0), (int)val8m(w.y, n1), (int)val8m(w.z, n2), (int)val8m(w.w, n3)};
        na = v4i{(int)n0, (int)n1, (int)n2, (int)n3};
      } else {
        val = v4i{(int)w.x, (int)w.y, (int)w.z, (int)w.w};
      }
#pragma unroll
      for (int nb = 0; nb < NB; nb++) {
        const uint4 bv = xs[SET][(it * 4 + g) * NCOL + nb * 16 + c];
        const v4i b = {(int)bv.x, (int)bv.y, (int)bv.z, (int)bv.w};
        acc[0][nb] = __builtin_amdgcn_mfma_i32_16x16x64_i8(val, b, acc[0][nb], 0, 0, 0);
        if constexpr (HASNA) acc[1][nb] = __builtin_amdgcn_mfma_i32_16x16x64_i8(na, b, acc[1][nb], 0, 0, 0);
      }
    }
#pragma unroll
    for (int it = 0; it < LD; it++) ga[SET][it] = *(const uint4 *)(rowp + (int64_t)ch2 * KC + it * 64);
    __builtin_amdgcn_sched_barrier(0);
    if (tid < XS) xs[SET ^ 1][tid] = xr;
    __syncthreads();
  };
  for (int ch = 0; ch < nchunks; ch += 2) {
    chunk(std::integral_constant<int, 0>{}, ch);
    if (ch + 1 < nchunks) chunk(std::integral_constant<int, 1>{}, ch + 1);
  }
#pragma unroll
  for (int r = 0; r < 4; r++) {
    const int64_t jo = snp_base + g * 4 + r;
    if (jo < m) {
#pragma unroll
      for (int p = 0; p < NPL; p++)
#pragma unroll
        for (int nb = 0; nb < NB; nb++) acc_out[((int64_t)p * m_out + jo) * NCOL + nb * 16 + c] = acc[p][nb][r];
    }
  }
}

__device__ __forceinline__ double horner_slices(const int32_t *a, int S, int nslice, int64_t stride) {
  double r = 0;
  for (int s = S - 1; s >= 0; s--) {
    long long d = 0;
    for (int t = 0; t < nslice; t++) d += a[t * stride + s];
    r = r * 256.0 + (double)d;
  }
  return r;
}
__global__ void k_cprod_final8(const int32_t *acc, int64_t m, int ncol, int S, const VecMeta *meta,
                               const double *center, const double *scale, double *Z, int64_t ldz, int has_q,
                               double vstep, double voff, int nslice) {
  int64_t j = (int64_t)blockIdx.x * blockDim.x + threadIdx.x;
  int v = blockIdx.y;
  if (j >= m) return;
  const int64_t stride = (has_q ? 2 : 1) * m * ncol;
  const double P = horner_slices(acc + j * ncol + v * S, S, nslice, stride);
  const double Q = has_q ? horner_slices(acc + (m + j) * ncol + v * S, S, nslice, stride) : 0.0;
  const double Sx = (double)meta[v].sum_hi * 16777216.0 + (double)meta[v].sum_lo;
  const double c = center ? center[j] : 0.0, s = scale ? scale[j] : 1.0, qs = meta[v].qscale;
  double z = qs > 0 ? (vstep * P + (voff - c) * (Sx - Q)) / (s * qs) : 0.0 / s;
  if (meta[v].nonfinite) z = __longlong_as_double(0x7ff8000000000000LL);
  Z[j + v * ldz] = z;
}

template <int NB, bool HASNA, bool CONTIG>
__global__ __launch_bounds__(256) void k_prod8(const uint8_t *__restrict__ img, int64_t pitch,
                                               const int32_t *__restrict__ cols, int64_t col0, int64_t m_pad,
                                               int64_t mc, const int8_t *__restrict__ wq,
                                               int32_t *__restrict__ acc_out, int64_t n_pad) {
  constexpr int NCOL = 16 * NB, WS = 8 * NCOL;
  const int tid = threadIdx.x, wave = tid >> 6, lane = tid & 63, sg = lane & 15, g = lane >> 4;
  const int64_t wbase = ((int64_t)blockIdx.x * 4 + wave) * 64;
  const int64_t wbyte = wbase + sg * 4;
  const int64_t j0 = (int64_t)blockIdx.y * mc;
  int64_t j1 = j0 + mc;
  if (j1 > m_pad) j1 = m_pad;
  if (j0 >= j1) return;
  const uint4 *wq4 = (const uint4 *)wq;
  v4i acc[4][NB];
#pragma unroll
  for (int u = 0; u < 4; u++)
#pragma unroll
    for (int nb = 0; nb < NB; nb++) acc[u][nb] = v4i{0, 0, 0, 0};
  __shared__ uint4 ws[2][WS];
  static_assert(WS <= 256, "digit staging");
  const int wtid = tid & (WS - 1);
  uint32_t X[2][16];
  auto load = [&](int64_t jb, uint32_t *dst) {
#pragma unroll
    for (int r = 0; r < 16; r++) {
      const int64_t jj = jb + g * 16 + r;
      const int64_t col = CONTIG ? col0 + jj : (int64_t)cols[jj];
      dst[r] = *(const uint32_t *)(img + col * pitch + wbyte);
    }
  };
  const int64_t jlast = j1 - 64;
  uint4 wreg = {0, 0, 0, 0};
  ws[0][wtid] = wq4[(j0 / 16) * 2 * NCOL + wtid];
  load(j0, X[0]);
  load(j0 + 64 < j1 ? j0 + 64 : jlast, X[1]);
  __syncthreads();
  auto step = [&](auto SETC, const int64_t jb) {
    constexpr int SET = decltype(SETC)::value;
    const int64_t jn1 = jb + 64 < j1 ? jb + 64 : jlast, jn2 = jb + 128 < j1 ? jb + 128 : jlast;
// ... 50 lines not shown
    }
  }
}

void require_bits(const bsn_bed *b, int bits, const char *what) {
  if (b->bits != bits)
    fail("%s is not available for this handle: it needs %s", what,
         bits == 2 ? "a 2-bit genotype image (.bed, or an FBM.code256 whose codes decode to 0 / 1 / 2 / NA)"
                   : "a byte (dosage) image");
}

void prof_begin(bsn_op *op, int kind, bool more) {
  if (!op->profile) return;
  if (op->prof_kind_override >= 0) kind = op->prof_kind_override;
  op->ev_more.push_back(more);
  hipEvent_t a, b;
  BSN_HIP(hipEventCreate(&a));
  BSN_HIP(hipEventCreate(&b));
  op->ev_begin.push_back(a);
  op->ev_end.push_back(b);
  op->ev_kind.push_back(kind);
  BSN_HIP(hipEventRecord(a, op->bed->stream));
}
void prof_end(bsn_op *op) {
  if (!op->profile) return;
  BSN_HIP(hipEventRecord(op->ev_end.back(), op->bed->stream));
  op->prof_kernel[op->ev_kind.back() % kProfKinds] = g_last_kernel;
}
void prof_collect(bsn_op *op, double ms[kProfKinds], int count[kProfKinds]) {
  for (int k = 0; k < kProfKinds; k++) ms[k] = 0, count[k] = 0;
  for (size_t i = 0; i < op->ev_begin.size(); i++) {
    float t = 0;
    if (hipEventSynchronize(op->ev_end[i]) == hipSuccess &&
        hipEventElapsedTime(&t, op->ev_begin[i], op->ev_end[i]) == hipSuccess) {
      ms[op->ev_kind[i]] += t;
      if (!op->ev_more[i]) count[op->ev_kind[i]]++;
    }
    (void)hipEventDestroy(op->ev_begin[i]);
    (void)hipEventDestroy(op->ev_end[i]);
  }
  (void)hipGetLastError();
  op->ev_begin.clear();
  op->ev_end.clear();
  op->ev_kind.clear();
  op->ev_more.clear();
}

static VecMeta *meta_buffer(bsn_op *op) {
  return (VecMeta *)op->d_meta.ensure((size_t)kMetaVecs * 8 + (size_t)kMetaVecs * 256 * 2);
}
static inline int64_t n_padded(const bsn_bed *b) { return b->bits == 8 ? b->pitch : b->pitch * 4; }

static void quantise(bsn_op *op, const double *d_X, int64_t ldx, int64_t len, int64_t len_pad,
                     int nvec, int mode, int S, int ncol, int permute, int exact_int,
                     VecMeta *meta, int8_t *q, const double *d_W2 = nullptr) {
  hipStream_t st = op->bed->stream;
  const bool bytes = op->bed->bits == 8;
  const double vstep = bytes ? op->bed->v_step : 1.0, voff = bytes ? op->bed->v_off : 0.0;
  const int raw3 = (!bytes && mode == 1) ? 1 : 0;
  if (bytes) permute = 0;
  if (permute == 2 && !(mode == 1 && (raw3 & 1))) fail("internal: the interleaved digit rows are the scaled product's");
  double *part = (double *)(meta + kMetaVecs);
  int gx = 0;
  if (exact_int) {
    hipLaunchKernelGGL(k_meta_clear, dim3(1), dim3(64), 0, st, meta, nvec);
  } else {
    gx = (int)((len + 1023) / 1024);
    if (gx > 256) gx = 256;
    hipLaunchKernelGGL(k_absmax, dim3(gx, nvec), dim3(1024), 0, st, d_X, ldx, len,
                       mode == 1 ? op->d_center.p : mode == 2 ? d_W2 : nullptr,
                       mode == 1 ? op->d_scale.p : nullptr, mode, meta, part, vstep, voff, raw3);
  }
  int64_t nblk = len_pad / 16;
  const double *qc = mode == 1 ? op->d_center.p : mode == 2 ? d_W2 : nullptr;
  const double *qsc = mode == 1 ? op->d_scale.p : nullptr;
  const dim3 qgrid((unsigned)((nblk + 63) / 64), nvec);
#define BSN_QUANT(SV)                                                                                  \
  case SV:                                                                                             \
    if (permute == 2)                                                                                  \
      hipLaunchKernelGGL((k_quant<SV, 2>), qgrid, dim3(64), 0, st, d_X, ldx, len, len_pad, qc, qsc, mode, \
                         ncol, meta, q, vstep, voff, raw3, part, gx);                                  \
    else if (permute)                                                                                  \
      hipLaunchKernelGGL((k_quant<SV, 1>), qgrid, dim3(64), 0, st, d_X, ldx, len, len_pad, qc, qsc, mode, \
                         ncol, meta, q, vstep, voff, raw3, part, gx);                                  \
    else                                                                                               \
      hipLaunchKernelGGL((k_quant<SV, 0>), qgrid, dim3(64), 0, st, d_X, ldx, len, len_pad, qc, qsc, mode, \
                         ncol, meta, q, vstep, voff, raw3, part, gx);                                  \
    break;
  switch (S) {
    BSN_QUANT(1) BSN_QUANT(2) BSN_QUANT(3) BSN_QUANT(4) BSN_QUANT(5) BSN_QUANT(6) BSN_QUANT(7) BSN_QUANT(8)
    default: fail("slices must be in 1..8");
  }
#undef BSN_QUANT
  BSN_HIP(hipGetLastError());
}

static const double *scatter_rows_if_needed(bsn_op *op, const double *d_X, int64_t *ldx,
                                            int nvec) {
  if (op->rows_identity) return d_X;
  bsn_bed *b = op->bed;
  double *xf = op->d_xfull.ensure((size_t)b->n * nvec);
  BSN_HIP(hipMemsetAsync(xf, 0, (size_t)b->n * nvec * sizeof(double), b->stream));
  hipLaunchKernelGGL(k_scatter_rows, dim3((unsigned)((op->n + 255) / 256), nvec), dim3(256), 0,
                     b->stream, d_X, *ldx, op->d_rows.p, op->n, xf, b->n);
  BSN_HIP(hipGetLastError());
  *ldx = b->n;
  return xf;
}

#pragma clang fp contract(off)
__global__ void k_binom_scale(const int32_t *counts, int64_t m, double *center, double *scale) {
  int64_t j = (int64_t)blockIdx.x * blockDim.x + threadIdx.x;
  if (j >= m) return;
  const int4 c = *(const int4 *)(counts + 4 * j);
  const double sumX = (double)(c.y + 2 * c.z);
  const double nona = (double)(c.x + c.y + c.z);
  const double af = sumX / (2.0 * nona);
  center[j] = 2.0 * af;
  scale[j] = sqrt(2.0 * af * (1.0 - af));
}
#pragma clang fp contract(on)

__global__ __launch_bounds__(256) void k_stats_summary(const int32_t *counts, int64_t m, int64_t n, int32_t *na,
                                                       unsigned long long *out) {
  long long s = 0, bad = 0;
  for (int64_t j = (int64_t)blockIdx.x * 256 + threadIdx.x; j < m; j += (int64_t)gridDim.x * 256) {
    const int4 c = *(const int4 *)(counts + 4 * j);
    s += c.w;
    na[j] = c.w;
    if (2 * ((int64_t)c.x + c.y + c.z) < n) bad++;
  }
  for (int off = 32; off > 0; off >>= 1) {
    s += __shfl_down(s, off);
    bad += __shfl_down(bad, off);
  }
  __shared__ long long sw[4], sb[4];
  if ((threadIdx.x & 63) == 0) {
    sw[threadIdx.x >> 6] = s;
    sb[threadIdx.x >> 6] = bad;
  }
  __syncthreads();
  if (threadIdx.x == 0) {
    s = sw[0] + sw[1] + sw[2] + sw[3];
    bad = sb[0] + sb[1] + sb[2] + sb[3];
    if (s) atomicAdd(&out[0], (unsigned long long)s);
    if (bad) atomicAdd(&out[1], (unsigned long long)bad);
  }
}

static bool use_tiled(const bsn_op *op) {
  return op->bed->d_tiled != nullptr && op->cols_contig && (op->col0 & 63) == 0;
}

template <int NPLANE, bool RAW0, bool STATS>
static void launch_cprod(bsn_op *op, int NB, const int8_t *q, int32_t *acc, uint32_t l0,
                         uint32_t l1, uint32_t l2, int32_t *counts = nullptr) {
  bsn_bed *b = op->bed;
  constexpr int KC = 512, TT = STATS ? 2 : 4;
  constexpr bool PLAIN = NPLANE == 2 && RAW0 && !STATS;
  if (b->pitch * 4 > 4000000) fail("more than 4e6 samples are not supported by the crossproduct kernel");
  const int32_t *cols = op->cols_contig ? nullptr : op->d_cols.p;
  const int32_t npad = (int32_t)(b->pitch * 4 - b->n);
  CprodFacts f;
  f.NB = NB, f.plain = PLAIN, f.stats = STATS, f.cols_contig = op->cols_contig, f.tiled = use_tiled(op);
  f.warm = op->prof_kind_override == 3, f.na_skip = op->na_skip_c;
  const CprodKernel k = choose_cprod(f);
  const uint8_t *image = k.tiled ? b->d_tiled : b->d_img;
  const int per_wg = 16 * k.tiles * k.waves;
  const dim3 grid((unsigned)((op->m + per_wg - 1) / per_wg)), block(64 * k.waves);
#define BSN_CPROD(NBV, CONTIGV, TV, WV, TAGV, TILEDV, SGBV, NASKIPV)                                                   \
  if (k == CprodKernel{NBV, CONTIGV, TV, WV, TAGV, TILEDV, SGBV, NASKIPV}) {                                           \
    BSN_KLAUNCH((k_cprod<NBV, NPLANE, KC, RAW0, STATS, CONTIGV, TV, WV, 1, TAGV, TILEDV, SGBV, NASKIPV>), grid, block, \
                0, b->stream, image, b->pitch, cols, op->col0, op->m, q, acc, op->m, l0, l1, l2, counts, npad);        \
    BSN_HIP(hipGetLastError());                                                                                        \
    return;                                                                                                            \
  }
  BSN_CPROD(1, false, 2, 8, 0, false, 0, false)
  BSN_CPROD(1, true, 2, 8, 0, false, 0, false)
  BSN_CPROD(1, true, 2, 8, 1, false, 0, false)
  BSN_CPROD(1, true, TT, 8, 0, true, 0, false)
  BSN_CPROD(1, true, TT, 8, 1, true, 0, false)
  BSN_CPROD(2, false, 2, 16, 0, false, 0, false)
  BSN_CPROD(2, true, 2, 16, 0, false, 3, false)
  BSN_CPROD(2, true, 2, 16, 0, true, 3, false)
  if constexpr (!STATS && NPLANE < 3) {
    BSN_CPROD(3, false, 2, 16, 0, false, 0, false)
    BSN_CPROD(3, true, 2, 16, 0, false, 3, false)
  }
  if constexpr (PLAIN) {
    BSN_CPROD(2, false, 2, 16, 0, false, 0, true)
    BSN_CPROD(2, true, 2, 16, 0, false, 0, true)
    BSN_CPROD(3, false, 2, 16, 0, false, 0, true)
    BSN_CPROD(3, true, 2, 16, 0, false, 0, true)
  }
#undef BSN_CPROD
  fail("internal: no crossproduct kernel with %d column blocks for this pass", NB);
}

static void launch_cprod_final(bsn_op *op, int NB, const int32_t *acc, int S, int nv, const VecMeta *meta, double *Z,
                               int64_t ldz, bool has_q) {
  auto go = [&](auto kern) {
    hipLaunchKernelGGL(kern, dim3((unsigned)((op->m + 127) / 128)), dim3(128), 0, op->bed->stream, acc, op->m, S, nv, meta,
                       op->d_center.p, op->d_scale.p, Z, ldz, has_q ? 1 : 0);
  };
  if (NB == 1) go(k_cprod_final<16>);
  else if (NB == 2) go(k_cprod_final<32>);
  else go(k_cprod_final<48>);
  BSN_HIP(hipGetLastError());
}

static void finish_fused_stats(bsn_op *op) {
  bsn_bed *b = op->bed;
  hipLaunchKernelGGL(k_binom_scale, dim3((unsigned)((op->m + 255) / 256)), dim3(256), 0, b->stream,
                     op->d_counts.p, op->m, op->d_center.p, op->d_scale.p);
  BSN_HIP(hipGetLastError());
  op->stats_pending = false;
  if (!op->h_na_total) BSN_HIP(hipHostMalloc((void **)&op->h_na_total, 2 * sizeof(long long), hipHostMallocDefault));
  op->h_na_total[0] = -1;
  op->h_na_total[1] = -1;
  unsigned long long *d_tot = (unsigned long long *)(op->d_counts.p + 4 * op->m);
  BSN_HIP(hipMemsetAsync(d_tot, 0, 16, b->stream));
  int gx = (int)((op->m + 1023) / 1024);
  if (gx > 1024) gx = 1024;
  hipLaunchKernelGGL(k_stats_summary, dim3(gx), dim3(256), 0, b->stream, op->d_counts.p, op->m, op->n,
                     op->d_na.ensure((size_t)op->m), d_tot);
  BSN_HIP(hipGetLastError());
  BSN_HIP(hipMemcpyAsync(op->h_na_total, d_tot, 16, hipMemcpyDeviceToHost, b->stream));
  op->na_poll = true;
}

void op_poll_stats(bsn_op *op) {
  if (!op->na_poll || !op->h_na_total) return;
  const long long t = *(volatile long long *)op->h_na_total;
  if (t < 0) return;
  op->na_poll = false;
  if (t == 0 && !getenv("BSN_FORCE_NA_PLANE")) op->no_na = true;
}

__device__ __forceinline__ uint32_t hash32(uint32_t x) {
  x ^= x >> 16; x *= 0x7feb352dU; x ^= x >> 15; x *= 0x846ca68bU; x ^= x >> 16;
  return x;
}
__global__ __launch_bounds__(64) void k_na_blocks(const uint8_t *__restrict__ img, int64_t pitch, int64_t m,
                                                  unsigned long long *out) {
  const int lane = threadIdx.x, c = lane & 15, g = lane >> 4;
  const uint32_t h = hash32((uint32_t)blockIdx.x * 0x9E3779B1u + 0x7F4A7C15u), h2 = hash32(h ^ 0x85EBCA6Bu);
  const int64_t nseg = pitch / 64, ngrp = m / 16, nhalf = m / 256, ndw = pitch / 4;
  int free_c = 0, free_p = 0, tot_c = 0, tot_p = 0;
  if (ngrp > 0 && nseg > 0) {
    const int64_t grp = (int64_t)(((uint64_t)h * (uint64_t)ngrp) >> 32), seg = (int64_t)(((uint64_t)h2 * (uint64_t)nseg) >> 32);
    const uint4 w = *(const uint4 *)(img + (grp * 16 + c) * pitch + seg * 64 + g * 16);
    const uint32_t ws[4] = {w.x, w.y, w.z, w.w};
#pragma unroll
    for (int d = 0; d < 4; d++)
      free_c += __builtin_amdgcn_ballot_w64(((ws[d] & (ws[d] >> 1)) & 0x55555555u) != 0u) == 0ull;
    tot_c = 4;
  }
  if (nhalf > 0 && ndw > 0) {
    const int64_t hc = (int64_t)(((uint64_t)h2 * (uint64_t)nhalf) >> 32), dw = (int64_t)(((uint64_t)h * (uint64_t)ndw) >> 32);
#pragma unroll
    for (int d = 0; d < 4; d++) {
      const uint32_t w = *(const uint32_t *)(img + (hc * 256 + 64 * g + 16 * d + c) * pitch + dw * 4);
      free_p += __builtin_amdgcn_ballot_w64(((w & (w >> 1)) & 0x55555555u) != 0u) == 0ull;
    }
    tot_p = 4;
  }
  if (lane == 0) {
    atomicAdd(&out[0], (unsigned long long)free_c);
    atomicAdd(&out[1], (unsigned long long)tot_c);
    atomicAdd(&out[2], (unsigned long long)free_p);
    atomicAdd(&out[3], (unsigned long long)tot_p);
  }
}

void op_na_blocks(bsn_op *op, int digit_cols) {
  bsn_bed *b = op->bed;
  op->na_skip_c = op->na_skip_p = false;
  if (b->bits != 2 || b->generic || op->no_na || !b->d_img || digit_cols <= 16) return;
  const char *fe = getenv("BSN_NA_SKIP");
  const int force = fe ? atoi(fe) : -1;
  if (force == 0) return;
  if (force == 1) {
    op->na_skip_c = op->na_skip_p = true;
    return;
  }
  const char *me = getenv("BSN_NA_SKIP_MIN");
  const double min_free = me ? atof(me) : 0.30;
  if (b->na_blocks_state == 0) {
    if (!b->h_na_blocks) BSN_HIP(hipHostMalloc((void **)&b->h_na_blocks, 5 * sizeof(long long), hipHostMallocDefault));
    if (!b->d_na_blocks) BSN_HIP(hipMalloc((void **)&b->d_na_blocks, 5 * sizeof(long long)));
    for (int i = 0; i < 5; i++) b->h_na_blocks[i] = -1;
    BSN_HIP(hipMemsetAsync(b->d_na_blocks, 0, 5 * sizeof(long long), b->stream));
    constexpr int kSamples = 8192;
    hipLaunchKernelGGL(k_na_blocks, dim3(kSamples), dim3(64), 0, b->stream, b->d_img, b->pitch, b->m,
                       (unsigned long long *)b->d_na_blocks);
    BSN_HIP(hipGetLastError());
    BSN_HIP(hipMemsetAsync((uint8_t *)b->d_na_blocks + 4 * sizeof(long long), 1, 1, b->stream));
    BSN_HIP(hipMemcpyAsync(b->h_na_blocks, b->d_na_blocks, 4 * sizeof(long long), hipMemcpyDeviceToHost, b->stream));
    BSN_HIP(hipMemcpyAsync(b->h_na_blocks + 4, b->d_na_blocks + 4, sizeof(long long), hipMemcpyDeviceToHost, b->stream));
    b->na_blocks_state = 1;
    return;
  }
  if (b->na_blocks_state == 1) {
    if (*(volatile long long *)(b->h_na_blocks + 4) != 1) return;
    const long long *v = b->h_na_blocks;
    b->na_free[0] = v[1] > 0 ? (double)v[0] / (double)v[1] : 0.0;
    b->na_free[1] = v[3] > 0 ? (double)v[2] / (double)v[3] : 0.0;
    b->na_blocks_state = 2;
  }
  op->na_skip_c = b->na_free[0] >= min_free;
  op->na_skip_p = b->na_free[1] >= min_free;
}

static int cprod_vmax(const bsn_op *op, int S) { return cprod_vmax(op->bed->bits, op->stats_pending, S); }

void op_cprod_prequant(bsn_op *op, const double *d_X, int64_t ldx, int nvec) {
  bsn_bed *b = op->bed;
  const int S = op->slices;
  op->preq_X = nullptr;
  if (nvec <= 0 || nvec > cprod_vmax(op, S) || !op->rows_identity) return;
  const int64_t npad = n_padded(b);
  quantise(op, d_X, ldx, b->n, npad, nvec, 0, S, 16 * pick_nb(nvec * S), 1, 0, meta_buffer(op),
           op->d_q.ensure((size_t)npad * kMaxCols * 2));
  op->preq_X = d_X;
  op->preq_ldx = ldx;
  op->preq_nvec = nvec;
  op->preq_S = S;
}

void op_cprod(bsn_op *op, const double *d_X, int64_t ldx, int nvec, double *d_Z, int64_t ldz) {
  bsn_bed *b = op->bed;
  refuse_generic(b, "this function (it needs the streaming products)");
  const int S = op->slices;
  if (nvec <= 0) return;
  if (b->bits == 8 && byte_slices(b->pitch) > kByteMaxSlices)
    fail("the crossproduct on a dosage FBM supports at most %lld samples", (long long)(kByteMaxSlices * kSliceBytes));
  op_na_blocks(op, nvec * S);
  const bool have_digits = op->preq_X == d_X && op->preq_ldx == ldx && op->preq_nvec == nvec && d_X != nullptr &&
                           op->preq_S == S && nvec <= cprod_vmax(op, S);
  op->preq_X = nullptr;
  const double *xsrc = scatter_rows_if_needed(op, d_X, &ldx, nvec);
  const int64_t npad = n_padded(b);
  VecMeta *meta = meta_buffer(op);
  for (int v0 = 0, vmax = 0; v0 < nvec; v0 += vmax) {
    vmax = cprod_vmax(op, S);
    int nv = nvec - v0 < vmax ? nvec - v0 : vmax;
    int NB = pick_nb(nv * S), ncol = 16 * NB;
    int8_t *q = op->d_q.ensure((size_t)npad * kMaxCols * 2);
    const int nslice = b->bits == 8 ? byte_slices(b->pitch) : 1;
    int32_t *acc = op->d_acc.ensure(std::max((size_t)2 * op->m * kMaxCols, (size_t)nslice * 2 * op->m * ncol));
    if (!have_digits) quantise(op, xsrc + (int64_t)v0 * ldx, ldx, b->n, npad, nv, 0, S, ncol, 1, 0, meta, q);
    prof_begin(op, op->stats_pending ? 2 : NB == 3 ? 4 : 0);
    if (b->bits == 8) {
      const dim3 grid8((unsigned)((op->m + 127) / 128), (unsigned)nslice);
      const int32_t *cols8 = op->cols_contig ? nullptr : op->d_cols.p;
#define BSN_CPROD8(NBV, NAV, CV)                                                                          \
  BSN_KLAUNCH((k_cprod8<NBV, NAV, CV>), grid8, dim3(512), 0, b->stream, b->d_img, b->pitch, cols8, \
                     op->col0, op->m, q, acc, op->m, (int)(kSliceBytes / 256))
      if (NB == 1) {
        if (op->no_na) { if (op->cols_contig) BSN_CPROD8(1, false, true); else BSN_CPROD8(1, false, false); }
        else { if (op->cols_contig) BSN_CPROD8(1, true, true); else BSN_CPROD8(1, true, false); }
      } else {
        if (op->no_na) { if (op->cols_contig) BSN_CPROD8(2, false, true); else BSN_CPROD8(2, false, false); }
        else { if (op->cols_contig) BSN_CPROD8(2, true, true); else BSN_CPROD8(2, true, false); }
      }
#undef BSN_CPROD8
      BSN_HIP(hipGetLastError());
      prof_end(op);
      op->passes++;
      hipLaunchKernelGGL(k_cprod_final8, dim3((unsigned)((op->m + 255) / 256), nv), dim3(256), 0, b->stream, acc,
                         op->m, ncol, S, meta, op->d_center.p, op->d_scale.p, d_Z + (int64_t)v0 * ldz, ldz,
                         op->no_na ? 0 : 1, b->v_step, b->v_off, nslice);
      BSN_HIP(hipGetLastError());
      continue;
    }
    if (op->stats_pending) {
      if (!op->rows_identity) fail("internal: fused scaling statistics need all samples");
      launch_cprod<2, true, true>(op, NB, q, acc, kLutRaw, kLutNA, 0, op->d_counts.ensure((size_t)4 * op->m + 8));
    } else if (op->no_na) {
      launch_cprod<1, true, false>(op, NB, q, acc, kLutRaw, 0, 0);
    } else {
      launch_cprod<2, true, false>(op, NB, q, acc, kLutRaw, kLutNA, 0);
    }
    prof_end(op);
    op->passes++;
    if (op->late_center || op->late_scale) {
      hipStream_t up = upload_stream(b);
      if (op->late_center) copy_h2d(b, op->d_center.p, op->late_center, (size_t)op->m * 8, up);
      if (op->late_scale) copy_h2d(b, op->d_scale.p, op->late_scale, (size_t)op->m * 8, up);
      BSN_HIP(hipEventRecord(b->ev_up, up));
      BSN_HIP(hipStreamWaitEvent(b->stream, b->ev_up, 0));
      op->late_center = op->late_scale = nullptr;
    }
    const bool has_q = op->stats_pending || !op->no_na;
    if (op->stats_pending) finish_fused_stats(op);
    launch_cprod_final(op, NB, acc, S, nv, meta, d_Z + (int64_t)v0 * ldz, ldz, has_q);
  }
}

static void launch_prod(bsn_op *op, int NB, dim3 grid, int64_t m_pad, int64_t mc, const int8_t *q, int32_t *acc,
                        int64_t npad, uint32_t lutP, uint32_t lutQ, bool has_q) {
  bsn_bed *b = op->bed;
  const int32_t *cols = op->d_cols.p;
  const ProdKernel k = choose_prod(NB, op->cols_contig, use_tiled(op), lutP == kLutRaw, has_q, op->prof_kind_override == 3);
  const uint8_t *image = k.tiled ? b->d_tiled : b->d_img;
#define BSN_PROD(NBV, CV, RAWP, HASQ, TAGV, TILEDV)                                                                  \
  if (k == ProdKernel{NBV, CV, RAWP, HASQ, TAGV, TILEDV}) {                                                          \
    BSN_KLAUNCH((k_prod<NBV, CV, RAWP, HASQ, TAGV, TILEDV>), grid, dim3(256), 0, b->stream, image, b->pitch, cols,   \
                op->col0, m_pad, mc, q, acc, npad, lutP, lutQ);                                                      \
    BSN_HIP(hipGetLastError());                                                                                      \
    return;                                                                                                          \
  }
#define BSN_PROD6(NBV, CV, TILEDV)                                                                \
  BSN_PROD(NBV, CV, true, true, 0, TILEDV) BSN_PROD(NBV, CV, true, true, 1, TILEDV)               \
  BSN_PROD(NBV, CV, true, false, 0, TILEDV) BSN_PROD(NBV, CV, true, false, 1, TILEDV)             \
  BSN_PROD(NBV, CV, false, true, 0, TILEDV) BSN_PROD(NBV, CV, false, false, 0, TILEDV)
  BSN_PROD6(1, true, false) BSN_PROD6(1, true, true) BSN_PROD6(1, false, false)
  BSN_PROD6(2, true, false) BSN_PROD6(2, true, true) BSN_PROD6(2, false, false)
#undef BSN_PROD6
#undef BSN_PROD
  fail("internal: no product kernel with %d column blocks", NB);
}

static void launch_prodT(bsn_op *op, const ProdTKernel &k, dim3 grid, int nchunks, int cps, const int8_t *q, int32_t *acc,
                         int64_t npad, uint32_t lutQ, int seg_bs, int seg_stride, int seg_off) {
  bsn_bed *b = op->bed;
#define BSN_PRODT(NBV, HASQV, TAGV, SGBV, NASKIPV, SPARSEV)                                                           \
  if (k == ProdTKernel{NBV, HASQV, TAGV, SGBV, NASKIPV, SPARSEV}) {                                                   \
    BSN_KLAUNCH((k_prodT<NBV, HASQV, 2, 16, TAGV, SGBV, NASKIPV, SPARSEV>), grid, dim3(1024), 0, b->stream, b->d_smaj, \
                b->rows_smaj, op->col0 / 512, nchunks, cps, q, acc, npad, lutQ, seg_bs, seg_stride, seg_off);         \
    BSN_HIP(hipGetLastError());                                                                                       \
    return;                                                                                                           \
  }
  BSN_PRODT(2, true, 0, 3, false, false) BSN_PRODT(2, true, 1, 3, false, false)
  BSN_PRODT(2, false, 0, 3, false, false) BSN_PRODT(2, false, 1, 3, false, false)
  BSN_PRODT(3, true, 0, 3, false, false) BSN_PRODT(3, false, 0, 3, false, false)
  BSN_PRODT(2, true, 0, 0, true, false) BSN_PRODT(3, true, 0, 0, true, false)
  BSN_PRODT(3, true, 0, 3, false, true) BSN_PRODT(3, true, 1, 3, false, true)
#undef BSN_PRODT
  fail("internal: no sample-major product kernel with %d column blocks", k.NB);
}

static void launch_prod_final(bsn_bed *b, int NB, const int32_t *acc, int64_t npad, int ky, int S, int nv, const VecMeta *meta,
                              const int32_t *d_rows, int64_t rows, double *Y, int64_t ldy, int sub_const, double beta,
                              int64_t blk_rows) {
  auto go = [&](auto kern) {
    hipLaunchKernelGGL(kern, dim3((unsigned)((rows + 255) / 256)), dim3(256), 0, b->stream, acc, npad, ky, S, nv, meta, d_rows,
                       rows, Y, ldy, sub_const, beta, blk_rows);
  };
  if (NB == 1) go(k_prod_final<16>);
  else if (NB == 2) go(k_prod_final<32>);
  else go(k_prod_final<48>);
  BSN_HIP(hipGetLastError());
}

static int device_cus() {
  static const int ncu = [] {
    hipDeviceProp_t pr;
    int dev = 0;
    return (hipGetDevice(&dev) == hipSuccess && hipGetDeviceProperties(&pr, dev) == hipSuccess && pr.multiProcessorCount > 0)
               ? pr.multiProcessorCount : 256;
  }();
  return ncu;
}

struct ProdSegments {
  int pieces, stride, nseg;
  const ProdSegment *segs;
  const std::function<void(int)> *after;
  bool done = false;
};
static void prod_planes(bsn_op *op, const double *d_X, const double *d_W2, int64_t ldx, int nvec,
                        double *d_Y, int64_t ldy, int mode, uint32_t lutP, uint32_t lutQ, int sub_const,
                        double beta, int S, ProdSegments *sg = nullptr) {
  bsn_bed *b = op->bed;
  refuse_generic(b, "this function (it needs the streaming products)");
  if (nvec <= 0) return;
  op->preq_X = nullptr;
  op_na_blocks(op, nvec * S);
  if (b->smaj_job) (void)image_smaj_poll(b);
  const bool has_q = lutQ != 0u && !(op->no_na && lutQ == kLutNA);
  ProdFacts f;
  f.bits = b->bits, f.n = b->n, f.m = op->m, f.pitch = b->pitch, f.col0 = op->col0, f.cols_contig = op->cols_contig;
  f.have_smaj = b->d_smaj != nullptr && !getenv("BSN_NO_SMAJ");
  f.mode = mode, f.raw_na = lutP == kLutRaw && lutQ == kLutNA, f.has_q = has_q;
  f.no_sparse = getenv("BSN_NO_SPARSE_PROD") != nullptr;
  f.nvec = nvec, f.S = S, f.segmented = sg != nullptr;
  if (f.have_smaj) f.ncu = device_cus();
#ifdef BSN_ABLATION
  if (const char *e = getenv("BSN_KY")) f.ky = std::max(1, atoi(e));
  if (const char *e = getenv("BSN_KY_T")) f.ky_t = std::max(1, atoi(e));
#endif
  const ProdPlan pl = plan_prod(f);
  if (pl.refuse == ProdRefusal::pitch_limit) fail("more than 6.7e7 samples are not supported by the product kernel");
  if (pl.refuse == ProdRefusal::nothing_queued) return;
  const bool smaj = pl.smaj;
  const int vmax = pl.vmax, ky = pl.ky, smaj_cps = pl.smaj_cps;
  const int64_t npad = n_padded(b), m_pad = pl.m_pad, mc = pl.mc;
  if (smaj && (int64_t)ky * smaj_cps < m_pad / 512) fail("internal: the slabs of k_prodT do not cover the variants");
  VecMeta *meta = meta_buffer(op);
  const bool warm = op->prof_kind_override == 3;
  for (int v0 = 0; v0 < nvec; v0 += vmax) {
    int nv = nvec - v0 < vmax ? nvec - v0 : vmax;
    int NB = pick_nb(nv * S), ncol = 16 * NB;
    const ProdTKernel kt = choose_prodT(NB, has_q, warm, op->na_skip_p, pl.sparse_ok);
    int8_t *q = op->d_q.ensure((size_t)(npad > m_pad ? npad : m_pad) * kMaxCols * 2);
    size_t acc_need = (size_t)ky * npad * ncol;
    if (acc_need < (size_t)2 * op->m * kMaxCols) acc_need = (size_t)2 * op->m * kMaxCols;
    int32_t *acc = op->d_acc.ensure(acc_need);
    quantise(op, d_X + (int64_t)v0 * ldx, ldx, op->m, m_pad, nv, mode, S, ncol, smaj && NB >= 2 ? (kt.sparse ? 2 : 1) : 0, 0, meta, q,
             d_W2 ? d_W2 + (int64_t)v0 * ldx : nullptr);
    dim3 grid((unsigned)pl.wgx, (unsigned)ky);
    prof_begin(op, NB == 3 ? 5 : 1);
    if (smaj && NB >= 2) {
      const int nchunks = (int)(m_pad / 512);
      if (sg) {
        for (int sidx = 0; sidx < sg->nseg; sidx++) {
          const ProdSegment &sgm = sg->segs[sidx];
          const dim3 gs((unsigned)(sg->pieces * sgm.bs), (unsigned)ky);
          if (sidx > 0) prof_begin(op, NB == 3 ? 5 : 1, true);
          launch_prodT(op, kt, gs, nchunks, smaj_cps, q, acc, npad, lutQ, sgm.bs, sg->stride, sgm.off);
          prof_end(op);
          const int64_t rows_s = (int64_t)sgm.bs * 512, tot = rows_s * sg->pieces;
          launch_prod_final(b, NB, acc, npad, ky, S, nv, meta, sgm.d_rows, tot, sgm.d_out, 0, sub_const, 0.0, rows_s);
          (*sg->after)(sidx);
        }
        op->passes++;
        sg->done = true;
        continue;
      }
      launch_prodT(op, kt, grid, nchunks, smaj_cps, q, acc, npad, lutQ, 0, 0, 0);
    } else if (NB > 2) {
      fail("internal: three column blocks without the sample-major copy");
    } else if (b->bits == 8) {
      if (mode != 1) fail("internal: plane products are not defined on a byte image");
      const int32_t *cols8 = op->d_cols.p;
#define BSN_PROD8(NBV, NAV, CV)                                                                          \
  BSN_KLAUNCH((k_prod8<NBV, NAV, CV>), grid, dim3(256), 0, b->stream, b->d_img, b->pitch, cols8, \
                     op->col0, m_pad, mc, q, acc, npad)
      if (NB == 1) {
        if (op->no_na) { if (op->cols_contig) BSN_PROD8(1, false, true); else BSN_PROD8(1, false, false); }
        else { if (op->cols_contig) BSN_PROD8(1, true, true); else BSN_PROD8(1, true, false); }
      } else {
        if (op->no_na) { if (op->cols_contig) BSN_PROD8(2, false, true); else BSN_PROD8(2, false, false); }
        else { if (op->cols_contig) BSN_PROD8(2, true, true); else BSN_PROD8(2, true, false); }
      }
#undef BSN_PROD8
      BSN_HIP(hipGetLastError());
    } else {
      launch_prod(op, NB, grid, m_pad, mc, q, acc, npad, lutP, lutQ, has_q);
    }
    prof_end(op);
    op->last_kernel = g_last_kernel;
    op->passes++;
    launch_prod_final(b, NB, acc, npad, ky, S, nv, meta, op->rows_identity ? nullptr : op->d_rows.p, op->n,
                      d_Y + (int64_t)v0 * ldy, ldy, sub_const, beta, 0);
  }
}

__global__ void k_cprod_raw_final(const int32_t *acc, int64_t m, int ncol, int S, const VecMeta *meta,
                                  double *P, double *Q, int64_t ld) {
  int64_t j = (int64_t)blockIdx.x * blockDim.x + threadIdx.x;
  int v = blockIdx.y;
  if (j >= m) return;
  const double qs = meta[v].qscale;
  const double inv = qs > 0 ? 1.0 / qs : 0.0;
  double p = horner_sub(acc + j * ncol + v * S, acc + (m + j) * ncol + v * S, 3, S) * inv,
         q = horner(acc + (m + j) * ncol + v * S, S) * inv;
  if (meta[v].nonfinite) p = q = __longlong_as_double(0x7ff8000000000000LL);
  P[j + v * ld] = p;
  Q[j + v * ld] = q;
}

void op_cprod_raw(bsn_op *op, const double *d_X, int64_t ldx, int nvec, double *d_P, double *d_Q,
                  int64_t ld) {
  require_bits(op->bed, 2, "the plane sums of multLinReg");
  op->preq_X = nullptr;
  bsn_bed *b = op->bed;
  const int S = op->slices;
  const int vmax = 32 / S;
  if (nvec <= 0) return;
  const double *xsrc = scatter_rows_if_needed(op, d_X, &ldx, nvec);
  const int64_t npad = n_padded(b);
  VecMeta *meta = meta_buffer(op);
  for (int v0 = 0; v0 < nvec; v0 += vmax) {
    int nv = nvec - v0 < vmax ? nvec - v0 : vmax;
    int NB = pick_nb(nv * S), ncol = 16 * NB;
    int8_t *q = op->d_q.ensure((size_t)npad * kMaxCols * 2);
    int32_t *acc = op->d_acc.ensure((size_t)2 * op->m * kMaxCols);
    quantise(op, xsrc + (int64_t)v0 * ldx, ldx, b->n, npad, nv, 0, S, ncol, 1, 0, meta, q);
    launch_cprod<2, true, false>(op, NB, q, acc, kLutRaw, kLutNA, 0);
    op->passes++;
    hipLaunchKernelGGL(k_cprod_raw_final, dim3((unsigned)((op->m + 255) / 256), nv), dim3(256), 0,
                       b->stream, acc, op->m, ncol, S, meta, d_P + (int64_t)v0 * ld,
                       d_Q + (int64_t)v0 * ld, ld);
    BSN_HIP(hipGetLastError());
  }
}

void op_prod(bsn_op *op, const double *d_X, int64_t ldx, int nvec, double *d_Y, int64_t ldy) {
  prod_planes(op, d_X, nullptr, ldx, nvec, d_Y, ldy, 1, kLutRaw, kLutNA, 1, 0.0, op->slices);
}

void op_prod_acc(bsn_op *op, const double *d_X, int64_t ldx, int nvec, double *d_Y, int64_t ldy, double beta) {
  prod_planes(op, d_X, nullptr, ldx, nvec, d_Y, ldy, 1, kLutRaw, kLutNA, 1, beta, op->slices);
}

bool op_prod_segments(bsn_op *op, const double *d_X, int64_t ldx, int nvec, int pieces, int stride, int nseg,
                      const ProdSegment *segs, const std::function<void(int)> &after) {
  if (!op->rows_identity || op->prof_kind_override == 3) return false;
  ProdSegments sg{pieces, stride, nseg, segs, &after};
  prod_planes(op, d_X, nullptr, ldx, nvec, nullptr, 0, 1, kLutRaw, kLutNA, 1, 0.0, op->slices, &sg);
  return sg.done;
}

__global__ void k_rowsq_weights(const double *center, const double *scale, int64_t m, double *a,
                                double *b, double *d) {
  int64_t j = (int64_t)blockIdx.x * blockDim.x + threadIdx.x;
  if (j >= m) return;
  const double c = center[j], s = scale[j];
  a[j] = 1.0 / (s * s);
  b[j] = -2.0 * c / (s * s);
  d[j] = c * c / (s * s);
}

void op_row_sums_sq(bsn_op *op, double *d_out) {
  require_bits(op->bed, 2, "prod_and_rowSumsSq");
  bsn_bed *bed = op->bed;
  DevBuf<double> w;
  double *a = w.ensure((size_t)3 * op->m), *b2 = a + op->m, *d = b2 + op->m;
  hipLaunchKernelGGL(k_rowsq_weights, dim3((unsigned)((op->m + 255) / 256)), dim3(256), 0, bed->stream,
                     op->d_center.p, op->d_scale.p, op->m, a, b2, d);
  BSN_HIP(hipGetLastError());
  constexpr uint32_t kLutX2 = 0x00040100u;
  constexpr uint32_t kLutM = 0x00010101u;
  prod_planes(op, a, b2, op->m, 1, d_out, op->n, 2, kLutX2, kLutG0, 0, 0.0, 7);
  prod_planes(op, d, nullptr, op->m, 1, d_out, op->n, 2, kLutM, 0u, 0, 1.0, 7);
  BSN_HIP(hipStreamSynchronize(bed->stream));
}

void op_row_counts(bsn_op *op, double *d_out) {
  require_bits(op->bed, 2, "bed_counts(byrow = TRUE)");
  bsn_bed *bed = op->bed;
  std::vector<double> ones((size_t)op->m, 1.0);
  DevBuf<double> w;
  copy_h2d(bed, w.ensure((size_t)op->m), ones.data(), (size_t)op->m * 8);
  prod_planes(op, w.p, nullptr, op->m, 1, d_out, op->n, 2, kLutHom2, 0u, 0, 0.0, 7);
  prod_planes(op, w.p, nullptr, op->m, 1, d_out + op->n, op->n, 2, kLutHet, 0u, 0, 0.0, 7);
  prod_planes(op, w.p, nullptr, op->m, 1, d_out + 2 * op->n, op->n, 2, kLutNA, 0u, 0, 0.0, 7);
  BSN_HIP(hipStreamSynchronize(bed->stream));
}

__global__ void k_counts_final(const int32_t *acc, int64_t m, int ncol, int S, int64_t n_sub,
                               int32_t *counts) {
  int64_t j = (int64_t)blockIdx.x * blockDim.x + threadIdx.x;
  if (j >= m) return;
  long long n2 = (long long)horner(acc + j * ncol, S);
  long long n1 = (long long)horner(acc + (m + j) * ncol, S);
  long long na = (long long)horner(acc + (2 * m + j) * ncol, S);
  counts[4 * j + 0] = (int32_t)(n_sub - n1 - n2 - na);
  counts[4 * j + 1] = (int32_t)n1;
  counts[4 * j + 2] = (int32_t)n2;
  counts[4 * j + 3] = (int32_t)na;
}

void counts_weighted(bsn_op *op, const double *d_w, int64_t n_sub, int32_t *d_counts) {
  require_bits(op->bed, 2, "bed_counts");
  op->preq_X = nullptr;
  bsn_bed *b = op->bed;
  const int S = 4;
  const int64_t npad = n_padded(b);
  VecMeta *meta = meta_buffer(op);
  int8_t *q = op->d_q.ensure((size_t)npad * 64);
  int32_t *acc = op->d_acc.ensure((size_t)3 * op->m * 16);
  quantise(op, d_w, b->n, b->n, npad, 1, 0, S, 16, 1, 1, meta, q);
  launch_cprod<3, false, false>(op, 1, q, acc, kLutHom2, kLutHet, kLutNA);
  hipLaunchKernelGGL(k_counts_final, dim3((unsigned)((op->m + 255) / 256)), dim3(256), 0, b->stream,
                     acc, op->m, 16, S, n_sub, d_counts);
  BSN_HIP(hipGetLastError());
}

__global__ void k_group_scatter(const int32_t *__restrict__ rows, const int32_t *__restrict__ group, int64_t n, int g0, int gb,
                                int64_t n_file, int32_t *mult) {
  const int64_t i = (int64_t)blockIdx.x * blockDim.x + threadIdx.x;
  if (i >= n) return;
  const int v = group[i] - g0;
  if (v < 0 || v >= gb) return;
  const int64_t k = rows ? (int64_t)rows[i] : i;
  if (k < 0 || k >= n_file) return;
  atomicAdd(&mult[(int64_t)v * n_file + k], 1);
}

template <int S>
__global__ __launch_bounds__(256) void k_group_digits(const int32_t *__restrict__ mult, int64_t n_file, int64_t nblk, int gb,
                                                      int ncol, int8_t *__restrict__ q) {
  const int64_t kb = (int64_t)blockIdx.x * blockDim.x + threadIdx.x;
  const int v = blockIdx.y;
  if (kb >= nblk || v >= gb) return;
  uint32_t pk[S][4];
#pragma unroll
  for (int s = 0; s < S; s++)
#pragma unroll
    for (int w = 0; w < 4; w++) pk[s][w] = 0;
#pragma unroll
  for (int e = 0; e < 16; e++) {
    const int64_t k = kb * 16 + e;
    long long A = k < n_file ? (long long)mult[(int64_t)v * n_file + k] : 0;
// ... 130 lines not shown
```

bigsnpr_amd/csrc/prod_plan.hpp:

```cpp
#pragma once
#include <algorithm>
#include <cstdint>

#include "byte_plan.hpp"

namespace bsn {
constexpr int kMaxCols = 48;
constexpr int kMetaVecs = 32;
inline int pick_nb(int ncols_needed) { return ncols_needed <= 16 ? 1 : ncols_needed <= 32 ? 2 : 3; }

inline int cprod_vmax(int bits, bool stats_pending, int S) {
  const int nbmax = (bits == 2 && !stats_pending) ? 3 : 2;
  int v = 16 * nbmax / S;
  if (v > kMetaVecs) v = kMetaVecs;
  return v < 1 ? 1 : v;
}

struct ProdFacts {
  int bits = 2;
  int64_t n = 0, m = 0;
  int64_t pitch = 0;
  int64_t col0 = 0;
  bool cols_contig = false;
  bool have_smaj = false;
  int mode = 1;
  bool raw_na = false;
  bool has_q = true;
  bool no_sparse = false;
  int nvec = 1, S = 1;
  int ncu = 256;
  bool segmented = false;
  int ky = 0, ky_t = 0;
};

enum class ProdRefusal { none, pitch_limit, nothing_queued };

struct ProdPlan {
  ProdRefusal refuse = ProdRefusal::none;
  bool smaj = false;
  int vmax = 1;
  int64_t m_pad = 0;
  int64_t wgx = 0;
  int ky = 1;
  int smaj_cps = 0;
  int64_t mc = 0;
  bool sparse_ok = false;
};

inline ProdPlan plan_prod(const ProdFacts &f) {
  ProdPlan p;
  if (f.pitch >= ((int64_t)1 << 24)) {
    p.refuse = ProdRefusal::pitch_limit;
    return p;
  }
  const int nvec = f.nvec, S = f.S;
  const int64_t npad = f.bits == 8 ? f.pitch : f.pitch * 4;
  const bool smaj_ok = f.bits == 2 && f.have_smaj && f.cols_contig && (f.col0 & 511) == 0 && f.mode == 1 && f.raw_na;
  const int vmax_smaj = std::min(kMetaVecs, (smaj_ok && nvec * S > 32 ? kMaxCols : 32) / S);
  const bool smaj = smaj_ok && nvec <= vmax_smaj && pick_nb(nvec * S) >= 2;
  const int vmax = smaj ? vmax_smaj : std::max(1, std::min(kMetaVecs, 32 / S));
  p.smaj = smaj;
  p.vmax = vmax;
  if (f.segmented && !smaj) {
    p.refuse = ProdRefusal::nothing_queued;
    return p;
  }
  const int64_t unit = smaj ? 512 : 64;
  const int64_t m_pad = (f.m + unit - 1) / unit * unit;
  int64_t wgx = f.bits == 8 ? npad / 256 : npad / 1024;
  int ky = (int)((4096 + wgx - 1) / wgx);
  const int64_t steps = m_pad / 64;
  int smaj_cps = 0;
  const int nb_max = pick_nb((nvec < vmax ? nvec : vmax) * S);
  if (smaj) {
    const int ncu = f.ncu;
    wgx = (f.n + 511) / 512;
    const int64_t nchunks = m_pad / 512;
    const double slab_cost = 0.3 * 2.0 * (double)npad * 16.0 * nb_max * 4.0 / ((double)m_pad * (double)(f.pitch));
    int best = 1;
    double best_score = -1e300;
    for (int c = 1; c <= 24 && c <= nchunks; c++) {
      if (c < 6 && c < nchunks && nchunks >= 6) continue;
      const int64_t W = wgx * c;
      const double fill = (double)W / ((double)ncu * (double)((W + ncu - 1) / ncu));
      const double score = fill - slab_cost * c;
      if (score > best_score + 1e-9) best_score = score, best = c;
    }
    ky = best;
    if (f.ky_t > 0) ky = std::max(1, std::min(f.ky_t, (int)nchunks));
    const int64_t ky_min2 = (m_pad + 2499999) / 2500000;
    if (ky < ky_min2) ky = (int)ky_min2;
    smaj_cps = (int)((nchunks + ky - 1) / ky);
    ky = (int)((nchunks + smaj_cps - 1) / smaj_cps);
  }
  if (!smaj) {
    if (ky > steps) ky = (int)steps;
    if (ky > 64) ky = 64;
  }
  if (ky < 1) ky = 1;
  if (f.bits == 2 && nb_max == 1) {
    const int ncol_max = 16 * nb_max;
    int64_t cap = (int64_t)(0.04 * (double)m_pad / (32.0 * ncol_max));
    if (cap < 1) cap = 1;
    if (ky > cap) ky = (int)cap;
    int best = ky;
    double best_fill = 0.0;
    for (int c = ky; c >= 1 && 2 * c >= ky; c--) {
      const int64_t W = wgx * c;
      const double fill = (double)W / (512.0 * (double)((W + 511) / 512));
      if (fill > best_fill + 1e-9) best_fill = fill, best = c;
    }
    ky = best;
  }
  if (!smaj && f.ky > 0) {
    ky = f.ky;
    if (ky > steps) ky = (int)steps;
    if (ky < 1) ky = 1;
  }
  const int64_t ky_min = f.bits == 8 ? byte_min_slabs(m_pad) : (m_pad + 2499999) / 2500000;
  if (ky < ky_min && !smaj) ky = (int)ky_min;
  const int64_t mc = slab_variants(steps, ky);
  if (!smaj) ky = (int)((m_pad + mc - 1) / mc);
  p.sparse_ok = smaj && f.has_q && !f.no_sparse &&
                3.0 * (double)m_pad * (double)((uint64_t)1 << (8 * S - 1)) < 9007199254740992.0;
  p.m_pad = m_pad;
  p.wgx = wgx;
  p.ky = ky;
  p.smaj_cps = smaj_cps;
  p.mc = mc;
  return p;
}

struct CprodKernel {
  int NB;
  bool contig;
  int tiles, waves, tag;
  bool tiled;
  int sgb;
  bool naskip;
};
inline bool operator==(const CprodKernel &a, const CprodKernel &b) {
  return a.NB == b.NB && a.contig == b.contig && a.tiles == b.tiles && a.waves == b.waves && a.tag == b.tag &&
         a.tiled == b.tiled && a.sgb == b.sgb && a.naskip == b.naskip;
}
struct CprodFacts {
  int NB = 1;
  bool plain = true;
  bool stats = false;
  bool cols_contig = false;
  bool tiled = false;
  bool warm = false;
  bool na_skip = false;
};
inline CprodKernel choose_cprod(const CprodFacts &f) {
  if (f.plain && f.na_skip && f.NB >= 2) return {f.NB, f.cols_contig, 2, 16, 0, false, 0, true};
  if (f.NB == 3) return {3, f.cols_contig, 2, 16, 0, false, f.cols_contig ? 3 : 0, false};
  if (f.tiled) return f.NB == 1 ? CprodKernel{1, true, f.stats ? 2 : 4, 8, f.warm ? 1 : 0, true, 0, false}
                                : CprodKernel{2, true, 2, 16, 0, true, 3, false};
  if (f.NB == 1) return {1, f.cols_contig, 2, 8, f.cols_contig && f.warm ? 1 : 0, false, 0, false};
  return {2, f.cols_contig, 2, 16, 0, false, f.cols_contig ? 3 : 0, false};
}

struct ProdKernel {
  int NB;
  bool contig, rawp, hasq;
  int tag;
  bool tiled;
};
inline bool operator==(const ProdKernel &a, const ProdKernel &b) {
  return a.NB == b.NB && a.contig == b.contig && a.rawp == b.rawp && a.hasq == b.hasq && a.tag == b.tag && a.tiled == b.tiled;
}
inline ProdKernel choose_prod(int NB, bool cols_contig, bool tiled, bool rawp, bool has_q, bool warm) {
  return {NB, cols_contig, rawp, has_q, rawp && warm ? 1 : 0, cols_contig && tiled};
}

struct ProdTKernel {
  int NB;
  bool hasq;
  int tag, sgb;
  bool naskip, sparse;
};
inline bool operator==(const ProdTKernel &a, const ProdTKernel &b) {
  return a.NB == b.NB && a.hasq == b.hasq && a.tag == b.tag && a.sgb == b.sgb && a.naskip == b.naskip && a.sparse == b.sparse;
}
inline ProdTKernel choose_prodT(int NB, bool has_q, bool warm, bool na_skip, bool sparse_ok) {
  if (has_q && sparse_ok && NB == 3 && !na_skip) return {3, true, warm ? 1 : 0, 3, false, true};
  if (has_q && na_skip) return {NB, true, 0, 0, true, false};
  return {NB, has_q, NB == 2 && warm ? 1 : 0, 3, false, false};
}

}
```

include/bigsnpr_hip.h:

```cpp
#ifndef BIGSNPR_HIP_H
#define BIGSNPR_HIP_H

#include <stdint.h>

#ifdef __cplusplus
extern "C" {
#endif

typedef struct bsn_bed bsn_bed;
typedef struct bsn_op bsn_op;

const char *bsn_last_error(void);
int bsn_version(void);
int bsn_device_count(int *count);
int bsn_set_device(int device);
int bsn_selftest(void);

int bsn_bed_open(const char *path, int64_t n, int64_t m, bsn_bed **out);
int bsn_bed_is_streamed(const bsn_bed *bed);
int bsn_bed_from_host(const uint8_t *payload, int64_t n, int64_t m, int64_t n_byte, bsn_bed **out);
int bsn_bed_from_fbm(const uint8_t *bytes, int64_t n, int64_t m, int64_t ld, bsn_bed **out);
int bsn_fbm_open(const uint8_t *bytes, int64_t n, int64_t m, int64_t ld, const double *code256, bsn_bed **out);
int bsn_bed_bits(const bsn_bed *bed);
int64_t bsn_bed_na_known(const bsn_bed *bed);
int bsn_bed_synthetic(int64_t n, int64_t m, uint32_t seed, uint32_t npop, uint32_t na16,
                      int64_t j_begin, bsn_bed **out);
int bsn_bed_close(bsn_bed *bed);
int64_t bsn_bed_nrow(const bsn_bed *bed);
int64_t bsn_bed_ncol(const bsn_bed *bed);
int64_t bsn_bed_bytes(const bsn_bed *bed);
int bsn_bed_download(bsn_bed *bed, uint8_t *payload_out);

int bsn_bed_prodvec(bsn_bed *bed, const int64_t *ind_row, int64_t n, const int64_t *ind_col,
                    int64_t m, const double *center, const double *scale, const double *x,
                    double *y);
int bsn_bed_cprodvec(bsn_bed *bed, const int64_t *ind_row, int64_t n, const int64_t *ind_col,
                     int64_t m, const double *center, const double *scale, const double *x,
                     double *z);

struct bsn_comm;
int bsn_bed_prodvec_sharded(bsn_bed *bed, const int64_t *ind_row, int64_t n, const int64_t *ind_col,
                            int64_t m, const double *center, const double *scale, const double *x,
                            struct bsn_comm *comm, double *y);
int bsn_bed_col_counts(bsn_bed *bed, const int64_t *ind_row, int64_t n, const int64_t *ind_col,
                       int64_t m, int32_t *res);
int bsn_bed_row_counts(bsn_bed *bed, const int64_t *ind_row, int64_t n, const int64_t *ind_col, int64_t m,
                       int32_t *res);
int bsn_bed_colstats(bsn_bed *bed, const int64_t *ind_row, int64_t n, const int64_t *ind_col,
                     int64_t m, double *sumX, double *denoX, int32_t *nb_nona_col, int32_t *n_bad);
int bsn_snp_colstats(bsn_bed *bed, const int64_t *ind_row, int64_t n, const int64_t *ind_col,
                     int64_t m, double *sumX, double *denoX);
int bsn_bed_read(bsn_bed *bed, const int64_t *ind_row, int64_t n, const int64_t *ind_col,
                 int64_t m, int32_t na_val, int32_t *out);
int bsn_bed_read_scaled(bsn_bed *bed, const int64_t *ind_row, int64_t n, const int64_t *ind_col,
                        int64_t m, const double *center, const double *scale, double *out);

int bsn_bed_cprod_planes(bsn_bed *bed, const int64_t *ind_row, int64_t n, const int64_t *ind_col,
                         int64_t m, const double *X, int64_t K, double *P, double *Q);

int bsn_mult_lin_reg(bsn_bed *bed, const int64_t *ind_row, int64_t n, const int64_t *ind_col, int64_t m,
                     const double *U, int64_t K, double *res);

int bsn_univ_linreg(bsn_bed *bed, const int64_t *ind_row, int64_t n, const int64_t *ind_col, int64_t m, const double *y,
                    const double *U, int64_t K, double *estim, double *std_err);
int bsn_univ_logreg(bsn_bed *bed, const int64_t *ind_row, int64_t n, const int64_t *ind_col, int64_t m, const double *y01,
                    const double *covar, int64_t q, double tol, int32_t maxiter, double *estim, double *std_err,
                    int32_t *niter);

typedef struct bsn_plr_options {
  int32_t family;
  int32_t nlambda;
  int32_t nlam_min;
  int32_t n_abort;
  int32_t dfmax;
  int32_t max_iter;
  double eps;
  double lambda_min_ratio;
} bsn_plr_options;
int bsn_bed_sp_reg(bsn_bed *bed, const int64_t *ind_row, int64_t n, const int64_t *ind_col, int64_t m, const double *y,
                   const double *covar, int64_t q, const double *pf, const int32_t *fold, int32_t K, const double *alphas,
                   int32_t n_alpha, const bsn_plr_options *opt, double *intercept, double *beta, double *lambda,
                   double *loss, double *loss_val, int32_t *iter, int32_t *nb_active, int32_t *n_done, int32_t *best,
                   int32_t *status);
int bsn_dense_sp_reg(const void *X, int type, int64_t ld, int64_t n, int64_t m, const double *y, const double *covar,
                     int64_t q, const double *pf, const int32_t *fold, int32_t K, const double *alphas, int32_t n_alpha,
                     const bsn_plr_options *opt, double *intercept, double *beta, double *lambda, double *loss,
                     double *loss_val, int32_t *iter, int32_t *nb_active, int32_t *n_done, int32_t *best, int32_t *status);
int bsn_plr_last_stats(double *out );

int bsn_impute_simple(bsn_bed *src, int method, uint64_t seed, bsn_bed **out, uint8_t *fbm_bytes_out ,
                      int64_t *n_all_missing );
int bsn_impute_last_ms(double *ms_out);

int bsn_bed_group_counts(bsn_bed *bed, const int64_t *ind_row, int64_t n, const int32_t *group , int32_t G,
                         const int64_t *ind_col, int64_t m, int32_t *res );
int bsn_fst(const double *af, const double *N, int64_t r, int64_t m, double min_maf, double *fst ,
            double *overall );
int bsn_bed_fst(bsn_bed *bed, const int64_t *ind_row, int64_t n, const int32_t *group , int32_t G,
                const int64_t *ind_col, int64_t m, double min_maf, double *fst , double *overall );
int bsn_snp_max3(bsn_bed *bed, const int64_t *ind_row, int64_t n, const int32_t *y01 , const int64_t *ind_col,
                 int64_t m, const double *val, int32_t L, double *score );
int bsn_popstat_last_ms(double *ms_out );

int bsn_bed_prod_and_rowsumssq(bsn_bed *bed, const int64_t *ind_row, int64_t n, const int64_t *ind_col,
                               int64_t m, const double *center, const double *scale, const double *V,
                               int64_t K, double *XV, double *rowSumsSq);

int bsn_snp_prod_and_rowsumssq2(bsn_bed *bed, const int64_t *ind_row, int64_t n, const int64_t *ind_col,
                                int64_t m, const double *center, const double *scale, const double *V,
                                int64_t K, double *XV, double *rowSumsSq);

int bsn_snp_grid_prs(bsn_bed *bed, const int64_t *ind_row, int64_t n, const int64_t *ind_col, int64_t m,
                     const double *betas, const int32_t *bin, const uint8_t *member, int64_t C, int64_t T,
                     int slices, double *out);

int bsn_bed_to_fbm(bsn_bed *bed, const int64_t *ind_row, int64_t n, const int64_t *ind_col, int64_t m,
                   uint8_t *out);
int bsn_bed_readbina(bsn_bed *bed, const uint8_t *tab, uint8_t *out);
int bsn_bed_subset_payload(bsn_bed *bed, const int64_t *ind_row, int64_t n, const int64_t *ind_col,
                           int64_t m, uint8_t *payload_out);

int bsn_op_create(bsn_bed *bed, const int64_t *ind_row, int64_t n, const int64_t *ind_col,
                  int64_t m, const double *center, const double *scale, bsn_op **out);
int bsn_op_destroy(bsn_op *op);
int bsn_op_set_slices(bsn_op *op, int slices);
int bsn_op_prod(bsn_op *op, const double *d_X, int64_t ldx, int nvec, double *d_Y, int64_t ldy);
int bsn_op_cprod(bsn_op *op, const double *d_X, int64_t ldx, int nvec, double *d_Z, int64_t ldz);
int bsn_op_sync(bsn_op *op);

typedef void (*bsn_allreduce_fn)(void *d_buf, int64_t count, void *ctx);

#define BSN_COMM_ID_BYTES 128
typedef struct bsn_comm bsn_comm;
int bsn_comm_unique_id(uint8_t *id_out );
int bsn_comm_init(const uint8_t *id, int rank, int world, bsn_comm **out);
int bsn_comm_rank(const bsn_comm *comm);
int bsn_comm_world(const bsn_comm *comm);
int bsn_comm_allreduce(bsn_comm *comm, double *d_buf, int64_t count);
int bsn_comm_abort(bsn_comm *comm);
int bsn_comm_destroy(bsn_comm *comm);
typedef struct bsn_svd_options {
  int32_t k;
  double tol;
  int32_t block;
  int32_t slices;
  int32_t max_basis;
  uint32_t seed;
  int32_t verbose;
  int64_t m_total;
  bsn_allreduce_fn allreduce;
  void *allreduce_ctx;
  int32_t hook_rank, hook_world;
  struct bsn_comm *comm;
  int32_t binom_scaling;
  double *center_out, *scale_out;
  int32_t warm_start;
  int32_t warm_denominator;
  int32_t max_restarts;
  double vec_floor;
  int32_t exchange_timing;
  int32_t exchange_timeout_ms;
} bsn_svd_options;
typedef struct bsn_svd_info {
  int32_t niter;
  int32_t nops;
  int32_t basis;
  int32_t converged;
  double max_rel_resid;
  double gpu_ms;
  double cprod_ms;
  double prod_ms;
  int32_t n_cprod, n_prod;
  int32_t block, slices;
  int32_t n_bad;
  int32_t fused_stats;
  double cprod_stats_ms;
  int32_t n_cprod_stats;
  int32_t warm_launches;
  double warm_fraction;
  double warm_ms;
  int32_t tiled;
  int32_t segmented_passes;
  int32_t compact_gathers;
  int32_t slices_max, wide_steps;
  double wide_cprod_ms, wide_prod_ms;
  int32_t n_wide_cprod, n_wide_prod;
  double lead_rel_resid;
  int32_t exchange_mode;
  int32_t n_exchange[4];
  double exchange_ms[4];
  int32_t compacted;
  double compact_ms;
  int32_t out_of_core;
  double na_free_steps[2];
  int32_t na_skip;
  int32_t early_ritz[2];
} bsn_svd_info;
int bsn_bed_randomsvd(bsn_bed *bed, const int64_t *ind_row, int64_t n, const int64_t *ind_col,
                      int64_t m, const double *center, const double *scale,
                      const bsn_svd_options *options, double *d, double *u, double *v,
                      bsn_svd_info *info);
int bsn_bed_streaming_kernels(bsn_bed *bed, char *buf, int64_t len);
int bsn_op_last_kernel(bsn_op *op, char *buf, int64_t len);
int bsn_bed_tile(bsn_bed *bed, int *built);
int bsn_bed_sample_major(bsn_bed *bed, int *built);

int bsn_bed_release_workspace(bsn_bed *bed);

int bsn_bed_tcrossprod(bsn_bed *bed, const int64_t *ind_row, int64_t n, const int64_t *ind_col,
                       int64_t m, const double *center, const double *scale, int64_t block_size,
                       double *K);

typedef struct bsn_cor bsn_cor;
int bsn_cormat(bsn_bed *bed, const int64_t *ind_row, int64_t n, const int64_t *ind_col, int64_t m,
               double size, const double *thr, const double *pos, int fill_diag, int32_t *p_out,
               int64_t *nnz_out, bsn_cor **out);
int bsn_cormat_fetch(bsn_cor *cor, int32_t *i_out, double *x_out);
int bsn_cormat_has_nan(const bsn_cor *cor, int *out);
int bsn_cormat_free(bsn_cor *cor);
int bsn_ld_last_stats(double *out );
int bsn_ld_scores(bsn_bed *bed, const int64_t *ind_row, int64_t n, const int64_t *ind_col, int64_t m,
                  double size, const double *pos, double *out);
int bsn_clumping_chr(bsn_bed *bed, const int64_t *ind_row, int64_t n, const int64_t *ind_col,
                     int64_t m, int mode, const double *aux1, const double *aux2,
                     const int32_t *ordInd, const int32_t *rankInd, const double *pos, double size,
                     double thr, int32_t *keep);
int bsn_clumping_chr_cached(bsn_bed *bed, const int64_t *ind_row, int64_t n, const int64_t *ind_col,
                            int64_t m, int mode, const double *aux1, const double *aux2,
                            const int32_t *ordInd, const int32_t *rankInd, const double *pos,
                            int64_t n_grid, const double *sizes, const double *thrs, int32_t *keep);

int bsn_robust_scale_tau2(const double *d_X, int64_t m, int64_t ld, int32_t ncol, double c1, double c2, double *mu_out, double *s_out);
int bsn_robust_medians(const double *d_X, int64_t m, int64_t ld, int32_t ncol, const double *centre, double *med_out);
int bsn_robust_pair_scales(const double *d_Z, int64_t m, int64_t ld, int32_t p, double c1, double c2, double *s_sum_out, double *s_diff_out);
int bsn_robust_mc_count(const double *d_up, int64_t nu, const double *d_lo, int64_t nl, double t, int64_t *count_out);
int bsn_robust_scale_cols(double *d_Z, int64_t m, int64_t ld, int32_t p, const double *div );
int bsn_robust_rotate(double *d_Z, int64_t m, int64_t ld, int32_t p, const double *E );
int bsn_robust_wdist(const double *d_Z, int64_t m, int64_t ld, int32_t p, const double *mu, const double *sig, double *out);
int bsn_robust_dist_ogk(const double *d_U, int64_t m, int64_t ld, int32_t p, int32_t niter, double cut_ratio, double c1, double c2,
                        double *dist_out, int64_t *n_kept_out);
int bsn_robust_rollmean(const double *x, int64_t m, const double *w, int32_t len, const int64_t *group_off, int32_t ngroups, double *out);
int bsn_robust_sort(double *x, int64_t m);
int bsn_robust_mc_window(const double *d_up, int64_t nu, const double *d_lo, int64_t nl, double a, double b, int64_t cap, double *out,
                         int64_t *count_out);

int bsn_order_decreasing(const double *S, int64_t m, const int64_t *group_off, int32_t ngroups, int32_t *ord, int32_t *rank);

typedef struct bsn_sfbm bsn_sfbm;
int bsn_sfbm_from_csc(const int64_t *p, const int32_t *i, const double *x, int64_t m2, int upper, bsn_sfbm **out);
int bsn_sfbm_ncol(const bsn_sfbm *s, int64_t *m2_out, int64_t *nnz_out, int64_t *bandwidth_out);
int bsn_sfbm_free(bsn_sfbm *s);
int bsn_lassosum2(const bsn_sfbm *s, const double *beta_hat, int64_t m, const double *pf, const double *lambda,
                  const double *delta, int64_t G, const int64_t *ind_sub, double dfmax, int32_t maxiter, double tol,
                  double *beta_out, int32_t *num_iter_out, double *time_out);
int bsn_ldpred2_gibbs(const bsn_sfbm *s, const double *beta_hat, const double *n_vec, int64_t m, const int64_t *ind_sub,
                      const double *h2, const double *p, const int32_t *sparse, const uint64_t *stream, int64_t G, int burn_in,
                      int num_iter, uint64_t seed, double *beta_out, double *seconds_out);
int bsn_ldpred2_gibbs_sampling(const bsn_sfbm *s, const double *beta_hat, const double *n_vec, int64_t m, const int64_t *ind_sub,
                               double h2, double p, int32_t sparse, uint64_t stream, int burn_in, int num_iter, uint64_t seed,
                               double *sample_out, double *seconds_out);
int bsn_ldpred2_auto(const bsn_sfbm *s, const double *beta_hat, const double *n_vec, const double *log_var, int64_t m,
                     const int64_t *ind_sub, const double *p_init, const uint64_t *stream, int64_t G, double h2_init,
                     int burn_in, int num_iter, int report_step, int no_jump_sign, double shrink_corr, int use_mle,
                     double p_lo, double p_hi, double alpha_lo, double alpha_hi, double mean_ld, uint64_t seed,
                     double *beta_est, double *postp_est, double *corr_est, double *sample_beta,
                     double *path_p, double *path_h2, double *path_alpha, double *seconds_out);

int bsn_sfbm_prodvec(bsn_sfbm *s, const double *x, const int64_t *ind_sub, int64_t m, double *y_out);
int bsn_sfbm_ld_scores(bsn_sfbm *s, const int64_t *ind_sub, int64_t m, double *out);
int bsn_sfbm_solve_sym(bsn_sfbm *s, const double *b, const double *add_to_diag, const int64_t *ind_sub, int64_t m, double tol,
                       int32_t maxiter, double *x_out, int32_t *iters_out, double *relres_out);
int bsn_sfbm_last_ms(const bsn_sfbm *s, double *ms_out);

int bsn_sfbm_ldsplit(const bsn_sfbm *s, double thr_r2, double max_r2, int32_t min_size, int32_t max_size, int32_t max_K,
                     double max_cost, const double *pos_scaled, double *C_out, int32_t *best_ind_out, double *cost_out,
                     double *cost2_out, double *perc_kept_out, int32_t *n_block_ok_out, int32_t *all_last_out,
                     int32_t *levels_run_out, double *seconds_out);

int bsn_malloc(void **d_ptr, int64_t bytes);
int bsn_free(void *d_ptr);
// ... 13 lines not shown
```

Measured before the change: 38.57 million.

## Fuse finalisation epilogues into cprod/prodT kernels and split tail workgroups

Folds the fixed-point-to-fp64 finalisation of the transposed product into the k_cprod kernel epilogue through LDS staging, so the separate k_cprod_final pass and its int32 accumulator round trip are skipped. The last k_prodT workgroup per row block reduces the cross-y partial sums and writes Y directly, using an atomic counter. The remainder tail of the cprod grid is also split along K into several parts so the last wave of workgroups fills the device better, with a small tail-final kernel that sums the parts. In exchange it adds atomics, a memset, extra LDS and new launch-bound constraints, and exposes a prod_acc API.

```diff
diff --git a/bigsnpr_amd/_lib.py b/bigsnpr_amd/_lib.py
--- a/bigsnpr_amd/_lib.py
+++ b/bigsnpr_amd/_lib.py
@@ -129,6 +129,7 @@
     "bsn_op_set_slices": (C.c_int, [vp, C.c_int]),
     "bsn_op_prod": (C.c_int, [vp, vp, i64, C.c_int, vp, i64]),
     "bsn_op_cprod": (C.c_int, [vp, vp, i64, C.c_int, vp, i64]),
+    "bsn_op_prod_acc": (C.c_int, [vp, vp, i64, C.c_int, vp, i64, C.c_double]),
     "bsn_op_sync": (C.c_int, [vp]),
     "bsn_op_last_kernel": (C.c_int, [vp, C.c_char_p, i64]),
     "bsn_bed_randomsvd": (C.c_int, [vp, i64p, i64, i64p, i64, f64p, f64p, C.POINTER(SvdOptions),
diff --git a/bigsnpr_amd/csrc/api.hip b/bigsnpr_amd/csrc/api.hip
--- a/bigsnpr_amd/csrc/api.hip
+++ b/bigsnpr_amd/csrc/api.hip
@@ -1148,6 +1148,13 @@
   });
 }
 
+int bsn_op_prod_acc(bsn_op *op, const double *d_X, int64_t ldx, int nvec, double *d_Y, int64_t ldy, double beta) {
+  return guarded([&] {
+    BSN_HIP(hipSetDevice(op->bed->device));
+    op_prod_acc(op, d_X, ldx, nvec, d_Y, ldy, beta);
+  });
+}
+
 int bsn_op_cprod(bsn_op *op, const double *d_X, int64_t ldx, int nvec, double *d_Z, int64_t ldz) {
   return guarded([&] {
     BSN_HIP(hipSetDevice(op->bed->device));
diff --git a/bigsnpr_amd/csrc/bsn_internal.hpp b/bigsnpr_amd/csrc/bsn_internal.hpp
--- a/bigsnpr_amd/csrc/bsn_internal.hpp
+++ b/bigsnpr_amd/csrc/bsn_internal.hpp
@@ -160,6 +160,7 @@
   bsn::DevBuf<double> d_xfull;
   bsn::DevBuf<int8_t> d_q;
   bsn::DevBuf<int32_t> d_acc;
+  bsn::DevBuf<unsigned> d_blkcnt;
   bsn::DevBuf<double> d_meta;
   bsn::DevBuf<double> d_yfull;
 };
diff --git a/bigsnpr_amd/csrc/matvec.hip b/bigsnpr_amd/csrc/matvec.hip
--- a/bigsnpr_amd/csrc/matvec.hip
+++ b/bigsnpr_amd/csrc/matvec.hip
@@ -225,22 +225,87 @@
   }
 }
 
+__device__ __forceinline__ double horner(const int32_t *a, int S) {
+  double r = 0;
+  for (int s = S - 1; s >= 0; s--) r = r * 256.0 + (double)a[s];
+  return r;
+}
+__device__ __forceinline__ double horner_sub(const int32_t *a, const int32_t *q, int k, int S) {
+  double r = 0;
+  for (int s = S - 1; s >= 0; s--) r = r * 256.0 + (double)((long long)a[s] - (long long)k * q[s]);
+  return r;
+}
+
+template <class FA, class FQ>
+__device__ __forceinline__ double cprod_finish(FA a, FQ q, int S, bool has_q, double c, double s, const VecMeta &mv) {
+  double P = 0, Q = 0;
+#pragma unroll 1
+  for (int sl = S - 1; sl >= 0; sl--) {
+    if (has_q) {
+      const long long qv = q(sl);
+      P = P * 256.0 + (double)((long long)a(sl) - 3LL * qv);
+      Q = Q * 256.0 + (double)qv;
+    } else {
+      P = P * 256.0 + (double)(long long)a(sl);
+    }
+  }
+  const double Sx = (double)mv.sum_hi * 16777216.0 + (double)mv.sum_lo;
+  const double qs = mv.qscale;
+  double z = qs > 0 ? (P - c * (Sx - Q)) / (s * qs) : 0.0 / s;
+  if (P == 0.0 && Sx - Q == 0.0 && qs > 0) z = 0.0;
+  if (mv.nonfinite) z = __longlong_as_double(0x7ff8000000000000LL);
+  return z;
+}
+
+struct CprodEpi {
+  double *Z = nullptr;
+  int64_t ldz = 0;
+  const double *center = nullptr, *scale = nullptr;
+  const VecMeta *meta = nullptr;
+  int S = 1, nv = 0;
+  unsigned whole = 0xffffffffu;
+  int parts = 1;
+  int32_t *acc_tail = nullptr;
+  int64_t m_tail = 0;
+};
+
+constexpr int cprod_min_waves(bool epi, int NPLANE, int TILES, int WAVES, int MINW) {
+  return MINW > 1 || !epi || WAVES != 8 ? MINW : TILES == 4 ? 4 : NPLANE == 1 ? 6 : 4;
+}
 template <int NB, int NPLANE, int KC, bool RAW0, bool STATS, bool CONTIG, int TILES = 2, int WAVES = 8, int MINW = 1,
           int TAG = 0, bool TILED = false, int SGB = 0, bool NASKIP = false>
-__global__ __launch_bounds__(64 * WAVES, MINW) void k_cprod(const uint8_t *__restrict__ img, int64_t pitch,
+__global__ __launch_bounds__(64 * WAVES, cprod_min_waves(CONTIG && RAW0 && !STATS && !NASKIP && NPLANE <= 2 && KC == 512, NPLANE,
+                                                         TILES, WAVES, MINW)) void k_cprod(const uint8_t *__restrict__ img, int64_t pitch,
                                                const int32_t *__restrict__ cols, int64_t col0,
                                                int64_t m, const int8_t *__restrict__ xq,
                                                int32_t *__restrict__ acc_out, int64_t m_out,
                                                uint32_t lutA, uint32_t lutB, uint32_t lutC,
-                                               int32_t *__restrict__ counts, int32_t n_pad_samples) {
+                                               int32_t *__restrict__ counts, int32_t n_pad_samples, const CprodEpi epi) {
   constexpr int NCOL = 16 * NB;
   constexpr int LD = KC / 256;
   constexpr int XS = KC / 16 * NCOL;
-  __shared__ uint4 xs[2][XS];
+  constexpr bool EPI = CONTIG && RAW0 && !STATS && !NASKIP && NPLANE <= 2 && KC == 512;
+  constexpr int EROW = NPLANE * NCOL + 1, ETS = WAVES == 8 ? TILES : 1;
+  constexpr int EWORDS = WAVES * ETS * 16 * EROW;
+  constexpr int LDS_U4 = EPI && (EWORDS + 3) / 4 > 2 * XS ? (EWORDS + 3) / 4 : 2 * XS;
+  __shared__ uint4 lds[LDS_U4];
+  uint4 (*const xs)[XS] = (uint4 (*)[XS])lds;
   const int tid = threadIdx.x, wave = tid >> 6, lane = tid & 63;
   const int c = lane & 15, g = lane >> 4;
   constexpr int NT = 64 * WAVES;
-  const int64_t wg_base = (int64_t)blockIdx.x * (WAVES * 16 * TILES);
+  unsigned vb = blockIdx.x;
+  int part = -1, cb = 0, nchunks = (int)(pitch * 4 / KC);
+  if constexpr (EPI) {
+    if (blockIdx.x >= epi.whole) {
+      const unsigned t = blockIdx.x - epi.whole;
+      vb = epi.whole + t / (unsigned)epi.parts;
+      part = (int)(t % (unsigned)epi.parts);
+      int ce;
+      cprod_part_chunks(nchunks, epi.parts, part, cb, ce);
+      nchunks = ce - cb;
+    }
+  }
+  const int64_t wg_base = (int64_t)vb * (WAVES * 16 * TILES);
   const int64_t snp_base = wg_base + wave * (16 * TILES);
   const uint8_t *rowp[TILES];
   uint32_t voff[TILES];
@@ -255,8 +320,8 @@
   }
   static_assert(!TILED || (CONTIG && (WAVES * 16 * TILES) % 64 == 0), "streaming layout: whole 64-variant blocks");
   const __amdgpu_buffer_rsrc_t rs = __builtin_amdgcn_make_buffer_rsrc(
-      (void *)(TILED ? img + (((col0 + wg_base) >> 6) * (pitch >> 8)) * 16384
-                     : img + (col0 + (CONTIG ? wg_base : 0)) * pitch),
+      (void *)(TILED ? img + (((col0 + wg_base) >> 6) * (pitch >> 8) + (((int64_t)cb * (KC / 4)) >> 8)) * 16384
+                     : img + (col0 + (CONTIG ? wg_base : 0)) * pitch + (int64_t)cb * (KC / 4)),
       0, 0x7fffffff, 0x00020000);
   typedef unsigned int v4u __attribute__((ext_vector_type(4)));
   auto gload = [&](const int t, const int off) -> uint4 {
@@ -268,8 +333,7 @@
       return *(const uint4 *)(rowp[t] + off);
     }
   };
-  const int nchunks = (int)(pitch * 4 / KC);
-  const uint4 *xq4 = (const uint4 *)xq;
+  const uint4 *xq4 = (const uint4 *)xq + (int64_t)cb * XS;
 
   v4i acc[TILES][NPLANE][NB];
 #pragma unroll
@@ -421,6 +485,46 @@
     if (ch + 1 < nchunks) chunk(std::integral_constant<int, 1>{}, ch + 1);
   }
 
+  int64_t j_out0 = 0;
+  if constexpr (EPI) {
+    if (part < 0 && epi.Z != nullptr) {
+      int32_t *const stage = (int32_t *)lds + wave * (ETS * 16 * EROW);
+#pragma unroll
+      for (int t0 = 0; t0 < TILES; t0 += ETS) {
+        __syncthreads();
+#pragma unroll
+        for (int t = t0; t < t0 + ETS; t++)
+#pragma unroll
+          for (int r = 0; r < 4; r++)
+#pragma unroll
+            for (int p = 0; p < NPLANE; p++)
+#pragma unroll
+              for (int nb = 0; nb < NB; nb++)
+                stage[((t - t0) * 16 + g * 4 + r) * EROW + p * NCOL + nb * 16 + c] = acc[t][p][nb][r];
+        __syncthreads();
+#pragma unroll 1
+        for (int t = t0; t < t0 + ETS; t++) {
+          const int64_t j = snp_base + t * 16 + c;
+          if (j >= m) continue;
+          const int32_t *const my = stage + ((t - t0) * 16 + c) * EROW;
+          const double cen = epi.center ? epi.center[j] : 0.0, sc = epi.scale ? epi.scale[j] : 1.0;
+#pragma unroll 1
+          for (int v = g; v < epi.nv; v += 4) {
+            const int32_t *const a = my + v * epi.S;
+            epi.Z[j + v * epi.ldz] =
+                cprod_finish([&](int sl) { return (long long)a[sl]; }, [&](int sl) { return (long long)a[NCOL + sl]; },
+                             epi.S, NPLANE == 2, cen, sc, epi.meta[v]);
+          }
+        }
+      }
+      return;
+    }
+    if (part >= 0) {
+      j_out0 = (int64_t)epi.whole * (WAVES * 16 * TILES);
+      acc_out = epi.acc_tail + (int64_t)part * NPLANE * epi.m_tail * NCOL;
+      m_out = epi.m_tail;
+    }
+  }
 #pragma unroll
   for (int t = 0; t < TILES; t++)
 #pragma unroll
@@ -431,7 +535,7 @@
         for (int p = 0; p < NPLANE; p++)
 #pragma unroll
           for (int nb = 0; nb < NB; nb++)
-            acc_out[((int64_t)p * m_out + j) * NCOL + nb * 16 + c] = acc[t][p][nb][r];
+            acc_out[((int64_t)p * m_out + j - j_out0) * NCOL + nb * 16 + c] = acc[t][p][nb][r];
       }
     }
   if constexpr (STATS) {
@@ -450,53 +554,50 @@
   }
 }
 
-__device__ __forceinline__ double horner(const int32_t *a, int S) {
-  double r = 0;
-  for (int s = S - 1; s >= 0; s--) r = r * 256.0 + (double)a[s];
-  return r;
-}
-__device__ __forceinline__ double horner_sub(const int32_t *a, const int32_t *q, int k, int S) {
-  double r = 0;
-  for (int s = S - 1; s >= 0; s--) r = r * 256.0 + (double)((long long)a[s] - (long long)k * q[s]);
-  return r;
-}
-
-template <int NCOL>
-__global__ __launch_bounds__(128) void k_cprod_final(const int32_t *__restrict__ acc, int64_t m, int S, int nv,
+template <int NCOL, bool PIECES = false>
+__global__ __launch_bounds__(PIECES ? 64 : 128) void k_cprod_final(const int32_t *__restrict__ acc, int64_t m, int S, int nv,
                                                      const VecMeta *__restrict__ meta,
                                                      const double *__restrict__ center,
                                                      const double *__restrict__ scale, double *Z, int64_t ldz,
-                                                     int has_q) {
-  constexpr int ROW = 2 * NCOL + 1;
-  __shared__ int32_t srow[128 * ROW];
-  const int64_t j = (int64_t)blockIdx.x * 128 + threadIdx.x;
+                                                     int has_q, int parts, int64_t j0) {
+  constexpr int ROW = 2 * NCOL + 1, TPB = PIECES ? 64 : 128;
+  typedef typename std::conditional<PIECES, long long, int32_t>::type sum_t;
+  __shared__ sum_t srow[TPB * ROW];
+  const int64_t j = (int64_t)blockIdx.x * TPB + threadIdx.x;
   if (j >= m) return;
-  int32_t *my = srow + threadIdx.x * ROW;
-  {
-    const int4 *pa = (const int4 *)(acc + j * NCOL), *pq = (const int4 *)(acc + (m + j) * NCOL);
+  sum_t *my = srow + threadIdx.x * ROW;
+  const int np = has_q ? 2 : 1;
+  if constexpr (PIECES) {
+    for (int t = 0; t < np * NCOL; t++) my[t] = 0;
+  }
+  for (int pc = 0; pc < (PIECES ? parts : 1); pc++) {
+    const int4 *pa = (const int4 *)(acc + ((int64_t)pc * np * m + j) * NCOL), *pq = (const int4 *)(acc + (((int64_t)pc * np + 1) * m + j) * NCOL);
 #pragma unroll
     for (int t = 0; t < NCOL / 4; t++) {
       const int4 x = pa[t];
-      my[4 * t] = x.x; my[4 * t + 1] = x.y; my[4 * t + 2] = x.z; my[4 * t + 3] = x.w;
+      if constexpr (PIECES) {
+        my[4 * t] += x.x; my[4 * t + 1] += x.y; my[4 * t + 2] += x.z; my[4 * t + 3] += x.w;
+      } else {
+        my[4 * t] = x.x; my[4 * t + 1] = x.y; my[4 * t + 2] = x.z; my[4 * t + 3] = x.w;
+      }
     }
     if (has_q) {
 #pragma unroll
       for (int t = 0; t < NCOL / 4; t++) {
         const int4 x = pq[t];
-        my[NCOL + 4 * t] = x.x; my[NCOL + 4 * t + 1] = x.y; my[NCOL + 4 * t + 2] = x.z; my[NCOL + 4 * t + 3] = x.w;
-      }
-    }
-  }
-  const double c = center ? center[j] : 0.0, s = scale ? scale[j] : 1.0;
+        if constexpr (PIECES) {
+          my[NCOL + 4 * t] += x.x; my[NCOL + 4 * t + 1] += x.y; my[NCOL + 4 * t + 2] += x.z; my[NCOL + 4 * t + 3] += x.w;
+        } else {
+          my[NCOL + 4 * t] = x.x; my[NCOL + 4 * t + 1] = x.y; my[NCOL + 4 * t + 2] = x.z; my[NCOL + 4 * t + 3] = x.w;
+        }
+      }
+    }
+  }
+  const double c = center ? center[j0 + j] : 0.0, s = scale ? scale[j0 + j] : 1.0;
   for (int v = 0; v < nv; v++) {
-    const double P = has_q ? horner_sub(my + v * S, my + NCOL + v * S, 3, S) : horner(my + v * S, S);
-    const double Q = has_q ? horner(my + NCOL + v * S, S) : 0.0;
-    const double Sx = (double)meta[v].sum_hi * 16777216.0 + (double)meta[v].sum_lo;
-    const double qs = meta[v].qscale;
-    double z = qs > 0 ? (P - c * (Sx - Q)) / (s * qs) : 0.0 / s;
-    if (P == 0.0 && Sx - Q == 0.0 && qs > 0) z = 0.0;
-    if (meta[v].nonfinite) z = __longlong_as_double(0x7ff8000000000000LL);
-    Z[j + v * ldz] = z;
+    const sum_t *const a = my + v * S;
+    Z[j0 + j + v * ldz] = cprod_finish([&](int sl) { return (long long)a[sl]; }, [&](int sl) { return (long long)a[NCOL + sl]; },
+                                       S, has_q != 0, c, s, meta[v]);
   }
 }
 
@@ -629,11 +730,33 @@
   }
 }
 
+template <class FD>
+__device__ __forceinline__ double prod_finish(FD d, int S, const VecMeta &mv, int sub_const) {
+  double r = 0;
+  for (int s = S - 1; s >= 0; s--) r = r * 256.0 + (double)(long long)d(s);
+  const double C = sub_const ? (double)mv.sum2_hi * 16777216.0 + (double)mv.sum2_lo : 0.0;
+  const double qs = mv.qscale;
+  double y = qs > 0 ? (r - C) / qs : 0.0;
+  if (mv.nonfinite) y = __longlong_as_double(0x7ff8000000000000LL);
+  return y;
+}
+__device__ __forceinline__ void prod_store(double *y_out, double y, double beta) { *y_out = beta != 0.0 ? beta * *y_out + y : y; }
+
+struct ProdFin {
+  double *Y = nullptr;
+  int64_t ldy = 0, n = 0;
+  const VecMeta *meta = nullptr;
+  int S = 1, nv = 0, sub_const = 0;
+  double beta = 0.0;
+  unsigned *count = nullptr;
+};
+
 template <int NB, bool HASQ, int TILES = 2, int WAVES = 16, int TAG = 0, int SGB = 3, bool NASKIP = false, bool SPARSE = false>
 __global__ __launch_bounds__(64 * WAVES) void k_prodT(const uint8_t *__restrict__ simg, int64_t rows_t, int64_t chunk0,
                                                       int nchunks, int cps,
                                                       const int8_t *__restrict__ wq, int32_t *__restrict__ acc_out,
-                                                      int64_t n_pad, uint32_t lutQ, int seg_bs, int seg_stride, int seg_off) {
+                                                      int64_t n_pad, uint32_t lutQ, int seg_bs, int seg_stride, int seg_off,
+                                                      const ProdFin fin) {
   constexpr int KC = 512, NCOL = 16 * NB, LD = KC / 256;
   constexpr int XS = KC / 16 * 2 * NCOL;
   constexpr int NT = 64 * WAVES, NX = XS / NT;
@@ -823,6 +946,54 @@
           acc_out[((int64_t)blockIdx.y * n_pad + i) * NCOL + nb * 16 + c] = acc[t][nb][r];
       }
     }
+  if (fin.Y == nullptr) return;
+  __shared__ int s_last;
+  __threadfence();
+  __syncthreads();
+  if (tid == 0) s_last = atomicAdd(&fin.count[bx], 1u) == gridDim.y - 1u ? 1 : 0;
+  __syncthreads();
+  if (!s_last) return;
+  __threadfence();
+  static_assert(2 * XS * sizeof(uint4) == 256 * NCOL * sizeof(long long), "the panels hold half a block of sums");
+  long long *const sums = (long long *)&xs[0][0];
+  constexpr int PC = NCOL / 16;
+  const int ky = (int)gridDim.y;
+#pragma unroll 1
+  for (int half = 0; half < 2; half++) {
+    const int r = tid >> 2, qd = tid & 3;
+    const int64_t i = wg_base + half * 256 + r;
+    long long d[PC * 4];
+#pragma unroll
+    for (int e = 0; e < PC * 4; e++) d[e] = 0;
+    if (i < n_pad) {
+      for (int k = 0; k < ky; k++) {
+        const int4 *a = (const int4 *)(acc_out + ((int64_t)k * n_pad + i) * NCOL);
+#pragma unroll
+        for (int u = 0; u < PC; u++) {
+          const int4 t = a[u * 4 + qd];
+          d[4 * u + 0] += t.x;
+          d[4 * u + 1] += t.y;
+          d[4 * u + 2] += t.z;
+          d[4 * u + 3] += t.w;
+        }
+      }
+    }
+    __syncthreads();
+#pragma unroll
+    for (int u = 0; u < PC; u++)
+#pragma unroll
+      for (int e = 0; e < 4; e++) sums[r * NCOL + ((u * 4 + qd) * 4 + e + r) % NCOL] = d[4 * u + e];
+    __syncthreads();
+    const int rr = tid & 255;
+    const int64_t io = wg_base + half * 256 + rr;
+    if (io < fin.n) {
+      for (int v = tid >> 8; v < fin.nv; v += 4) {
+        const double y = prod_finish([&](int sl) { return sums[rr * NCOL + (v * fin.S + sl + rr) % NCOL]; }, fin.S, fin.meta[v],
+                                     fin.sub_const);
+        prod_store(fin.Y + io + v * fin.ldy, y, fin.beta);
+      }
+    }
+  }
 }
 
 template <int NCOL>
@@ -851,21 +1022,18 @@
     }
   }
   for (int v = 0; v < nv; v++) {
-    double r = 0;
-    for (int s = S - 1; s >= 0; s--) {
-      long long dv = 0;
-#pragma unroll
-      for (int c = 0; c < NCOL; c++) dv = (c == v * S + s) ? d[c] : dv;
-      r = r * 256.0 + (double)dv;
-    }
-    double C = sub_const ? (double)meta[v].sum2_hi * 16777216.0 + (double)meta[v].sum2_lo : 0.0;
-    double qs = meta[v].qscale;
-    double y = qs > 0 ? (r - C) / qs : 0.0;
-    if (meta[v].nonfinite) y = __longlong_as_double(0x7ff8000000000000LL);
+    const double y = prod_finish(
+        [&](int s) {
+          long long dv = 0;
+#pragma unroll
+          for (int c = 0; c < NCOL; c++) dv = (c == v * S + s) ? d[c] : dv;
+          return dv;
+        },
+        S, meta[v], sub_const);
     if (blk_rows > 0)
       Y[(i / blk_rows * nv + v) * blk_rows + i % blk_rows] = y;
     else
-      Y[i + v * ldy] = beta != 0.0 ? beta * Y[i + v * ldy] + y : y;
+      prod_store(Y + i + v * ldy, y, beta);
   }
 }
 
@@ -1222,9 +1390,34 @@
   return op->bed->d_tiled != nullptr && op->cols_contig && (op->col0 & 63) == 0;
 }
 
+static int device_cus() {
+  static const int ncu = [] {
+    hipDeviceProp_t pr;
+    int dev = 0;
+    return (hipGetDevice(&dev) == hipSuccess && hipGetDeviceProperties(&pr, dev) == hipSuccess && pr.multiProcessorCount > 0)
+               ? pr.multiProcessorCount : 256;
+  }();
+  return ncu;
+}
+
+static bool pass_epilogue() {
+  const char *e = getenv("BSN_PASS_EPILOGUE");
+  return !(e && atoi(e) == 0);
+}
+
+template <class K>
+static int cprod_resident(K kern, int threads) {
+  int nb = 0;
+  if (hipOccupancyMaxActiveBlocksPerMultiprocessor(&nb, kern, threads, 0) != hipSuccess || nb < 1) {
+    (void)hipGetLastError();
+    nb = 1;
+  }
+  return nb * device_cus();
+}
+
 template <int NPLANE, bool RAW0, bool STATS>
 static void launch_cprod(bsn_op *op, int NB, const int8_t *q, int32_t *acc, uint32_t l0,
-                         uint32_t l1, uint32_t l2, int32_t *counts = nullptr) {
+                         uint32_t l1, uint32_t l2, int32_t *counts = nullptr, CprodEpi *epi = nullptr) {
   bsn_bed *b = op->bed;
   constexpr int KC = 512, TT = STATS ? 2 : 4;
   constexpr bool PLAIN = NPLANE == 2 && RAW0 && !STATS;
@@ -1237,11 +1430,35 @@
   const CprodKernel k = choose_cprod(f);
   const uint8_t *image = k.tiled ? b->d_tiled : b->d_img;
   const int per_wg = 16 * k.tiles * k.waves;
-  const dim3 grid((unsigned)((op->m + per_wg - 1) / per_wg)), block(64 * k.waves);
+  dim3 grid((unsigned)((op->m + per_wg - 1) / per_wg)), block(64 * k.waves);
+  constexpr bool EPI_OK = RAW0 && !STATS && NPLANE <= 2;
+  const bool fuse = EPI_OK && epi && epi->Z && k.contig && !k.naskip;
+  if (epi && !fuse) *epi = CprodEpi{};
+  CprodEpi ke;
+  auto plan_grid = [&](int resident) {
+    const char *re = getenv("BSN_CPROD_ROUND");
+    const int R = re && atoi(re) > 0 ? atoi(re) : resident;
+    const CprodGrid cg = plan_cprod_grid((int64_t)grid.x, R, (int)(b->pitch * 4 / KC));
+    if (cg.parts > 1) {
+      epi->whole = (unsigned)cg.whole, epi->parts = cg.parts;
+      epi->m_tail = op->m - cg.whole * per_wg;
+      const size_t need = (size_t)cg.parts * NPLANE * epi->m_tail * 16 * NB;
+      epi->acc_tail = acc = op->d_acc.ensure(need > op->d_acc.n ? need : op->d_acc.n);
+      grid.x = (unsigned)cg.grid();
+    }
+    ke = *epi;
+  };
 #define BSN_CPROD(NBV, CONTIGV, TV, WV, TAGV, TILEDV, SGBV, NASKIPV)                                                   \
   if (k == CprodKernel{NBV, CONTIGV, TV, WV, TAGV, TILEDV, SGBV, NASKIPV}) {                                           \
-    BSN_KLAUNCH((k_cprod<NBV, NPLANE, KC, RAW0, STATS, CONTIGV, TV, WV, 1, TAGV, TILEDV, SGBV, NASKIPV>), grid, block, \
-                0, b->stream, image, b->pitch, cols, op->col0, op->m, q, acc, op->m, l0, l1, l2, counts, npad);        \
+    auto kern = k_cprod<NBV, NPLANE, KC, RAW0, STATS, CONTIGV, TV, WV, 1, TAGV, TILEDV, SGBV, NASKIPV>;                \
+    if constexpr (EPI_OK && CONTIGV && !NASKIPV) {                                                                     \
+      if (fuse) {                                                                                                      \
+        static const int resident = cprod_resident(kern, 64 * WV);                                                     \
+        plan_grid(resident);                                                                                           \
+      }                                                                                                                \
+    }                                                                                                                  \
+    BSN_KLAUNCH(kern, grid, block, 0, b->stream, image, b->pitch, cols, op->col0, op->m, q, acc, op->m, l0, l1, l2,   \
+                counts, npad, ke);                                                                                     \
     BSN_HIP(hipGetLastError());                                                                                        \
     return;                                                                                                            \
   }
@@ -1271,11 +1488,21 @@
                                int64_t ldz, bool has_q) {
   auto go = [&](auto kern) {
     hipLaunchKernelGGL(kern, dim3((unsigned)((op->m + 127) / 128)), dim3(128), 0, op->bed->stream, acc, op->m, S, nv, meta,
-                       op->d_center.p, op->d_scale.p, Z, ldz, has_q ? 1 : 0);
+                       op->d_center.p, op->d_scale.p, Z, ldz, has_q ? 1 : 0, 1, (int64_t)0);
   };
   if (NB == 1) go(k_cprod_final<16>);
   else if (NB == 2) go(k_cprod_final<32>);
   else go(k_cprod_final<48>);
+  BSN_HIP(hipGetLastError());
+}
+static void launch_cprod_final_tail(bsn_op *op, int NB, const CprodEpi &e, bool has_q) {
+  auto go = [&](auto kern) {
+    hipLaunchKernelGGL(kern, dim3((unsigned)((e.m_tail + 63) / 64)), dim3(64), 0, op->bed->stream, e.acc_tail, e.m_tail, e.S, e.nv,
+                       e.meta, e.center, e.scale, e.Z, e.ldz, has_q ? 1 : 0, e.parts, op->m - e.m_tail);
+  };
+  if (NB == 1) go(k_cprod_final<16, true>);
+  else if (NB == 2) go(k_cprod_final<32, true>);
+  else go(k_cprod_final<48, true>);
   BSN_HIP(hipGetLastError());
 }
 
@@ -1444,16 +1671,25 @@
       BSN_HIP(hipGetLastError());
       continue;
     }
+    CprodEpi epi;
+    if (pass_epilogue() && !op->stats_pending && !op->late_center && !op->late_scale) {
+      epi.Z = d_Z + (int64_t)v0 * ldz, epi.ldz = ldz, epi.center = op->d_center.p, epi.scale = op->d_scale.p;
+      epi.meta = meta, epi.S = S, epi.nv = nv;
+    }
     if (op->stats_pending) {
       if (!op->rows_identity) fail("internal: fused scaling statistics need all samples");
       launch_cprod<2, true, true>(op, NB, q, acc, kLutRaw, kLutNA, 0, op->d_counts.ensure((size_t)4 * op->m + 8));
     } else if (op->no_na) {
-      launch_cprod<1, true, false>(op, NB, q, acc, kLutRaw, 0, 0);
+      launch_cprod<1, true, false>(op, NB, q, acc, kLutRaw, 0, 0, nullptr, &epi);
     } else {
-      launch_cprod<2, true, false>(op, NB, q, acc, kLutRaw, kLutNA, 0);
+      launch_cprod<2, true, false>(op, NB, q, acc, kLutRaw, kLutNA, 0, nullptr, &epi);
     }
     prof_end(op);
     op->passes++;
+    if (epi.Z) {
+      if (epi.parts > 1) launch_cprod_final_tail(op, NB, epi, !op->no_na);
+      continue;
+    }
     if (op->late_center || op->late_scale) {
       hipStream_t up = upload_stream(b);
       if (op->late_center) copy_h2d(b, op->d_center.p, op->late_center, (size_t)op->m * 8, up);
@@ -1493,12 +1729,12 @@
 }
 
 static void launch_prodT(bsn_op *op, const ProdTKernel &k, dim3 grid, int nchunks, int cps, const int8_t *q, int32_t *acc,
-                         int64_t npad, uint32_t lutQ, int seg_bs, int seg_stride, int seg_off) {
+                         int64_t npad, uint32_t lutQ, int seg_bs, int seg_stride, int seg_off, const ProdFin &fin = ProdFin{}) {
   bsn_bed *b = op->bed;
 #define BSN_PRODT(NBV, HASQV, TAGV, SGBV, NASKIPV, SPARSEV)                                                           \
   if (k == ProdTKernel{NBV, HASQV, TAGV, SGBV, NASKIPV, SPARSEV}) {                                                   \
     BSN_KLAUNCH((k_prodT<NBV, HASQV, 2, 16, TAGV, SGBV, NASKIPV, SPARSEV>), grid, dim3(1024), 0, b->stream, b->d_smaj, \
-                b->rows_smaj, op->col0 / 512, nchunks, cps, q, acc, npad, lutQ, seg_bs, seg_stride, seg_off);         \
+                b->rows_smaj, op->col0 / 512, nchunks, cps, q, acc, npad, lutQ, seg_bs, seg_stride, seg_off, fin);    \
     BSN_HIP(hipGetLastError());                                                                                       \
     return;                                                                                                           \
   }
@@ -1522,16 +1758,6 @@
   else if (NB == 2) go(k_prod_final<32>);
   else go(k_prod_final<48>);
   BSN_HIP(hipGetLastError());
-}
-
-static int device_cus() {
-  static const int ncu = [] {
-    hipDeviceProp_t pr;
-    int dev = 0;
-    return (hipGetDevice(&dev) == hipSuccess && hipGetDeviceProperties(&pr, dev) == hipSuccess && pr.multiProcessorCount > 0)
-               ? pr.multiProcessorCount : 256;
-  }();
-  return ncu;
 }
 
 struct ProdSegments {
@@ -1581,6 +1807,13 @@
     quantise(op, d_X + (int64_t)v0 * ldx, ldx, op->m, m_pad, nv, mode, S, ncol, smaj && NB >= 2 ? (kt.sparse ? 2 : 1) : 0, 0, meta, q,
              d_W2 ? d_W2 + (int64_t)v0 * ldx : nullptr);
     dim3 grid((unsigned)pl.wgx, (unsigned)ky);
+    ProdFin fin;
+    if (smaj && NB >= 2 && !sg && op->rows_identity && pass_epilogue()) {
+      fin.Y = d_Y + (int64_t)v0 * ldy, fin.ldy = ldy, fin.n = op->n, fin.meta = meta, fin.S = S, fin.nv = nv;
+      fin.sub_const = sub_const, fin.beta = beta;
+      fin.count = op->d_blkcnt.ensure((size_t)pl.wgx);
+      BSN_HIP(hipMemsetAsync(fin.count, 0, (size_t)pl.wgx * sizeof(unsigned), b->stream));
+    }
     prof_begin(op, NB == 3 ? 5 : 1);
     if (smaj && NB >= 2) {
       const int nchunks = (int)(m_pad / 512);
@@ -1599,7 +1832,7 @@
         sg->done = true;
         continue;
       }
-      launch_prodT(op, kt, grid, nchunks, smaj_cps, q, acc, npad, lutQ, 0, 0, 0);
+      launch_prodT(op, kt, grid, nchunks, smaj_cps, q, acc, npad, lutQ, 0, 0, 0, fin);
     } else if (NB > 2) {
       fail("internal: three column blocks without the sample-major copy");
     } else if (b->bits == 8) {
@@ -1623,6 +1856,7 @@
     prof_end(op);
     op->last_kernel = g_last_kernel;
     op->passes++;
+    if (fin.Y) continue;
     launch_prod_final(b, NB, acc, npad, ky, S, nv, meta, op->rows_identity ? nullptr : op->d_rows.p, op->n,
                       d_Y + (int64_t)v0 * ldy, ldy, sub_const, beta, 0);
   }
diff --git a/bigsnpr_amd/csrc/prod_plan.hpp b/bigsnpr_amd/csrc/prod_plan.hpp
--- a/bigsnpr_amd/csrc/prod_plan.hpp
+++ b/bigsnpr_amd/csrc/prod_plan.hpp
@@ -161,6 +161,42 @@
   return {2, f.cols_contig, 2, 16, 0, false, f.cols_contig ? 3 : 0, false};
 }
 
+#if defined(__HIPCC__)
+#define BSN_PLAN_HD __host__ __device__ inline
+#else
+#define BSN_PLAN_HD inline
+#endif
+struct CprodGrid {
+  int64_t whole = 0;
+  int64_t split = 0;
+  int parts = 1;
+  int64_t grid() const { return whole + split * parts; }
+};
+inline CprodGrid plan_cprod_grid(int64_t W, int64_t R, int nchunks) {
+  CprodGrid g;
+  g.whole = W;
+  if (W <= 0 || R <= 0 || W / R < 2) return g;
+  const int64_t r = W % R;
+  if (r == 0) return g;
+  const int pairs = (nchunks + 1) / 2;
+  int best = 1;
+  double best_fill = (double)r / (double)R;
+  for (int s = 2; s <= 6 && s <= pairs; s++) {
+    const int64_t wgs = r * s;
+    const double fill = (double)wgs / ((double)R * (double)((wgs + R - 1) / R));
+    if (fill > best_fill + 1e-9) best_fill = fill, best = s;
+  }
+  if (best == 1) return g;
+  g.whole = W - r, g.split = r, g.parts = best;
+  return g;
+}
+BSN_PLAN_HD void cprod_part_chunks(int nchunks, int parts, int part, int &cb, int &ce) {
+  const int pairs = (nchunks + 1) / 2;
+  cb = 2 * (part * pairs / parts);
+  ce = 2 * ((part + 1) * pairs / parts);
+  if (ce > nchunks) ce = nchunks;
+}
+
 struct ProdKernel {
   int NB;
   bool contig, rawp, hasq;
diff --git a/include/bigsnpr_hip.h b/include/bigsnpr_hip.h
--- a/include/bigsnpr_hip.h
+++ b/include/bigsnpr_hip.h
@@ -126,6 +126,7 @@
 int bsn_op_set_slices(bsn_op *op, int slices);
 int bsn_op_prod(bsn_op *op, const double *d_X, int64_t ldx, int nvec, double *d_Y, int64_t ldy);
 int bsn_op_cprod(bsn_op *op, const double *d_X, int64_t ldx, int nvec, double *d_Z, int64_t ldz);
+int bsn_op_prod_acc(bsn_op *op, const double *d_X, int64_t ldx, int nvec, double *d_Y, int64_t ldy, double beta);
 int bsn_op_sync(bsn_op *op);
 
 typedef void (*bsn_allreduce_fn)(void *d_buf, int64_t count, void *ctx);
```

Measured after the change: 34.69 million. 0.899x the previous value.
